# hhcho/sfgwas

Measured on AMD Instinct MI355X. Metric: pca_power_iter_ring_macs_per_s, higher is better.
Workload: dtype u64 ring words, exact integers: int8 digits on the matrix core for the MAC of all five moduli, fp64-held integers in the encode and key-switch kernels

## Files before the change

sfgwas_amd/csrc/ab/ab.hpp:

```cpp
#pragma once
struct MacStrides; struct PanelMap; struct I8Args;
void ab_read_config(SfgConfig &c);
const char *ab_mgpu_solo(int n_local, bool multi_process, bool &solo, int &world, int &rank0);
int ab_set_attrs(sfg_ctx *ctx);
int ab_mac_dma_set_attrs(sfg_ctx *ctx);
int ab_launch_mac_dma_tiles(sfg_ctx *ctx, const double *rotf, size_t rows_per_k, const u64 *pt, u64 *out, int K, int R, int Ncols, int L, int accumulate, const MacStrides &st);
int ab_ntt_set_attrs(sfg_ctx *ctx);
int ab_launch_ntt_half_full(sfg_ctx *ctx, const double *pc, u64 *out_half, size_t nplain, int L, const PanelMap &pm);
int launch_mac(sfg_ctx *ctx, const u64 *rot, const u64 *pt, u64 *out, int K, int R, int Ncols, int L, int accumulate);
int launch_mac_strided(sfg_ctx *ctx, const u64 *rot, const u64 *pt, u64 *out, int K, int R, int Ncols, int L, int accumulate, const MacStrides &st);
void ab_launch_mac_i8_lds(hipStream_t q, const I8Args &a, const ModConst *modc, int nl);
```

sfgwas_amd/csrc/ab/config.hip:

```cpp
#include "../common.hpp"

void ab_read_config(SfgConfig &c) {
    auto env = [](const char *n) { return getenv(n); };
    if (const char *e = env("SFG_MAC_IMPL")) { c.mac_reg = !strcmp(e, "reg"); c.mac_bc = strcmp(e, "dma") != 0 && !c.mac_reg; c.mac_i8 = !strcmp(e, "i8"); }
    if (const char *e = env("SFG_MAC_I8_BIG")) c.mac_i8_big = atoi(e) != 0;
    if (const char *e = env("SFG_MAC_I8_ROT")) { c.mac_i8_nolds = strcmp(e, "lds") != 0; c.mac_i8_ring = !strcmp(e, "ring"); }
    if (env("SFG_MAC_I8_WG")) c.mac_i8_ring = false;
    if (const char *e = env("SFG_MAC_I8_WAVES")) c.mac_i8_waves = atoi(e) == 6 ? 6 : 12;
    if (const char *e = env("SFG_MAC_I8_WG")) c.mac_i8_wg1 = atoi(e) == 1;
    if (const char *e = env("SFG_MAC_WC")) c.mac_wc = atoi(e) == 2 ? 2 : 1;
    if (const char *e = env("SFG_MM_OVERLAP")) c.no_overlap = atoi(e) == 0;
    if (env("SFG_MM_NO_OVERLAP")) c.no_overlap = true;
    if (const char *e = env("SFG_NTT_HALF_IMPL")) c.ntt_half_full = !strcmp(e, "full");
    if (const char *e = env("SFG_NTT_FWD_IMPL")) c.ntt_fwd_full = !strcmp(e, "full");
    if (const char *e = env("SFG_MAC_PT")) c.mac_plain_pt = !strcmp(e, "plain");
    if (const char *e = env("SFG_PT_RIDE")) { c.pt_ride = atoi(e); if (c.pt_ride < 0) c.pt_ride = 0; c.pt_ride = c.pt_ride / 8 * 8; }
    if (const char *e = env("SFG_PT_COMPACT")) c.pt_compact = atoi(e) != 0;
    if (const char *e = env("SFG_PT_KMAJOR")) c.pt_kmajor = atoi(e) != 0;
    if (const char *e = env("SFG_PT_RIDE_DEPTH")) { c.i8_mover_depth_ride = atoi(e); if (c.i8_mover_depth_ride < 1 || c.i8_mover_depth_ride > 3) c.i8_mover_depth_ride = 1; }
    if (const char *e = env("SFG_PT_RIDE_NT")) c.i8_mover_nt_ride = atoi(e) != 0;
    if (env("SFG_ASSOC_TRACE")) c.assoc_trace = true;
}
int ab_set_attrs(sfg_ctx *ctx) { return ab_mac_dma_set_attrs(ctx) || ab_ntt_set_attrs(ctx); }
```

sfgwas_amd/csrc/common.hpp:

```cpp
#pragma once
#include <hip/hip_runtime.h>
#include <cstdint>
#include <cstdio>
#include <cstring>
#include <string>
#include <vector>
#include <map>
#include <set>
#include <unistd.h>
#include "../../include/sfgwas_hip.h"
#include "consts.hpp"

typedef unsigned long long u64;
typedef unsigned __int128 u128;

constexpr unsigned long long SFG_I8_BIG_QMAX = 0x7F7F7F7F7F80ULL;

struct ModConst {
    double q, qinv;
    double ninv, ninv_q;
    u64 qi;
};

struct RotKey {
    u64 *key_dev = nullptr;
    uint16_t *index_dev = nullptr;
};

struct PhaseStat { double ms = 0; int launches = 0; double bytes = 0; };
struct PendingEvent { hipEvent_t e0, e1; std::string name; int launches; double bytes; };

struct sfg_geno {
    const int8_t *dev = nullptr;
    size_t nrow = 0, ncol = 0, ld = 0;
    bool owned = false;
    bool packed = false;
    struct PtcEntry { double *slot; bool transposed; };
    mutable std::map<uint64_t, PtcEntry> ptc;
    mutable size_t ptc_budget = 0, ptc_used = 0;
    mutable double *ptc_arena = nullptr;
    mutable uint32_t *ptc_perm = nullptr;
    mutable const void *ptc_owner = nullptr;
    mutable size_t ptc_hits = 0, ptc_fills = 0;
};

struct SfgConfig {
    int mm_group = 8;
    bool mm_group_auto = true;
    size_t acc_budget = 24ULL << 30;
    size_t assoc_cache_budget = 160ULL << 30;
    size_t ksw_budget = 4ULL << 30;
    int enc_batch = 2048;
    bool upload_blocking = false;
    bool test_hooks = false;
    std::string test_scratch_oom;
    double tie_band = 0x1p-50;
    bool mac_i8_big = true;
    bool mac_reg = false;
    bool mac_bc = true;
    bool mac_i8 = true;
    bool mac_i8_nolds = true;
    bool mac_i8_ring = true;
    int mac_i8_waves = 12;
    bool mac_i8_wg1 = false;
    int mac_wc = 1;
    bool no_overlap = true;
    bool ntt_fwd_full = false;
    bool ntt_half_full = false;
    bool pt_compact = true;
    bool pt_kmajor = true;
    int pt_ride = 192;
    int i8_mover_depth_ride = 1, i8_mover_nt_ride = 1;
    bool mac_plain_pt = false;
    bool assoc_trace = false;
};

struct SfgShared {
    int device = 0;
    int logN = SFG_LOGN, N = SFG_N, nq = 0, np = 0, nmod = 0, beta = 0;
    double scale = 0;
    u64 q[SFG_MAXMOD] = {0}, psi[SFG_MAXMOD] = {0};
    double *tw_fwd = nullptr;
    double *tw_inv = nullptr;
    double2 *pack_fwd = nullptr;
    double2 *pack_inv = nullptr;
    ModConst *modc = nullptr;
    ModConst modc_host[SFG_MAXMOD];
    void *enc_tables = nullptr;
    void *rvec_tables = nullptr;
    void *zeros_dev = nullptr;
    u64 *sk_dev = nullptr;
    u64 *pk_dev = nullptr;
    u64 *skqp_dev = nullptr;
    uint32_t enc_key[8] = {0, 0, 0, 0, 0, 0, 0, 0}; uint32_t *enc_key_dev = nullptr; bool enc_seeded = false;
    u64 enc_next = 0;
    std::map<u64, RotKey> rotkeys;
    SfgConfig cfg;
    int refs = 1;
};

struct sfg_ctx {
    SfgShared *sh = nullptr;
    bool is_fork = false;
    int device = 0;
    int logN = SFG_LOGN, N = SFG_N, nq = 0, np = 0, nmod = 0, beta = 0;
    double scale = 0;
    u64 q[SFG_MAXMOD] = {0}, psi[SFG_MAXMOD] = {0};
    double *tw_fwd = nullptr, *tw_inv = nullptr;
    double2 *pack_fwd = nullptr, *pack_inv = nullptr;
    ModConst *modc = nullptr;
    ModConst modc_host[SFG_MAXMOD];
    SfgConfig cfg;
    unsigned ntt_plain_seq = 0;
    struct I8Slot { const void *src = nullptr; u64 sig[8] = {0, 0, 0, 0, 0, 0, 0, 0}; u64 last_use = 0; };
    static constexpr int I8_SLOTS = 16;
    u64 i8_gen = 1, i8_clock = 0; I8Slot i8_slot[2][I8_SLOTS];
    hipStream_t own_stream = nullptr, stream = nullptr;
    hipStream_t user_stream = nullptr;
    hipStream_t aux_stream = nullptr;
    unsigned char *pin = nullptr; size_t pin_bytes = 0, pin_head = 0;
    hipStream_t coll_stream = nullptr;
    hipEvent_t ev_pipe[4] = {nullptr, nullptr, nullptr, nullptr};
    std::vector<hipEvent_t> ev_pool; size_t ev_next = 0;
    std::map<int, void *> ksw_cache;
    void *ws = nullptr; size_t ws_bytes = 0;
    std::map<std::string, std::pair<void *, size_t>> pool;
    std::map<std::string, std::pair<void *, size_t>> host_pool;
    std::map<std::string, unsigned long long> pool_epoch;
    unsigned long long api_epoch = 0; int api_depth = 0;
    int scratch_oom_seen = 0;
    std::vector<PendingEvent> pending;
    std::string err;
    std::map<std::string, PhaseStat> phases;
    std::set<const sfg_geno *> ptc_genos;
    bool test_hooks = false;
    void *tie_count_dev = nullptr;
    hipStream_t main_stream() const { return user_stream ? user_stream : own_stream; }
    std::map<u64, RotKey> &rotkeys() { return sh->rotkeys; }
    const std::map<u64, RotKey> &rotkeys() const { return sh->rotkeys; }
    void *enc_tables() const { return sh->enc_tables; }
    void *zeros_dev() const { return sh->zeros_dev; }
};

int sfg_sync_all(sfg_ctx *ctx);
int sfg_encoder_check(sfg_ctx *ctx);
void sfg_ptc_detach_all(sfg_ctx *ctx);
void sfg_ptc_invalidate_all(sfg_ctx *ctx);

int encrypt_set_attrs(sfg_ctx *ctx);
int sfg_rows_from_montgomery(sfg_ctx *ctx, unsigned long long *rows_dev, size_t nrows, int nmod);
void sfg_encrypt_destroy(SfgShared *sh);
int enc_take_indices(sfg_ctx *ctx, const char *what, int nct, unsigned long long *first);
int keygen_set_attrs(sfg_ctx *ctx);
void sfg_keygen_destroy(SfgShared *sh);
int sfg_rvec_init(sfg_ctx *ctx);
void sfg_rvec_destroy(SfgShared *sh);

extern thread_local std::string g_create_error;

#define SFG_FAIL(ctx, ...) do { char _b[512]; snprintf(_b, sizeof _b, __VA_ARGS__); (ctx)->err = _b; return 1; } while (0)
#ifdef SFG_AB
#include "ab/ab.hpp"
#endif
#define SFG_HIP(ctx, call) do { hipError_t _e = (call); if (_e != hipSuccess) { char _b[512]; \
    snprintf(_b, sizeof _b, "HIP call failed: %s (%s:%d)", hipGetErrorString(_e), __FILE__, __LINE__); (ctx)->err = _b; return 1; } } while (0)
#define SFG_TRY(expr) do { int _rc = (expr); if (_rc) return _rc; } while (0)

int sfg_ws_reserve(sfg_ctx *ctx, size_t bytes);

static inline u64 h_mulmod(u64 a, u64 b, u64 q) { return (u64)(((u128)a * b) % q); }
static inline u64 h_powmod(u64 a, u64 e, u64 q) { u64 r = 1 % q; a %= q; while (e) { if (e & 1) r = h_mulmod(r, a, q); a = h_mulmod(a, a, q); e >>= 1; } return r; }
static inline u64 h_invmod(u64 a, u64 q) { return h_powmod(a, q - 2, q); }
static inline uint32_t h_brev(uint32_t x, int bits) { uint32_t r = 0; for (int i = 0; i < bits; i++) { r = (r << 1) | (x & 1); x >>= 1; } return r; }

int sfg_upload_small(sfg_ctx *ctx, void *dst_dev, const void *src_host, size_t bytes);
struct ApiScope {
    sfg_ctx *c;
    explicit ApiScope(sfg_ctx *c_) : c(c_) { if (c->api_depth++ == 0) c->api_epoch++; }
    ~ApiScope() { c->api_depth--; }
};
struct AuxScope {
    sfg_ctx *c; hipStream_t saved;
    explicit AuxScope(sfg_ctx *c_, bool on = true) : c(c_), saved(c_->stream) { if (on) c->stream = c->aux_stream; }
    ~AuxScope() { c->stream = saved; }
};
template <class T, hipError_t (*Free)(T)> struct HipOwner {
    T h = T();
    HipOwner() {}
    HipOwner(HipOwner &&o) : h(o.release()) {}
    HipOwner(const HipOwner &) = delete; HipOwner &operator=(const HipOwner &) = delete;
    ~HipOwner() { if (h) (void)Free(h); }
    T release() { T t = h; h = T(); return t; }
};
typedef HipOwner<void *, hipFree> DevMem;
typedef HipOwner<hipEvent_t, hipEventDestroy> EventOwner;
typedef HipOwner<hipStream_t, hipStreamDestroy> StreamOwner;
struct FdOwner {
    int fd;
    explicit FdOwner(int fd_ = -1) : fd(fd_) {}
    FdOwner(FdOwner &&o) : fd(o.fd) { o.fd = -1; }
    FdOwner(const FdOwner &) = delete; FdOwner &operator=(const FdOwner &) = delete;
    ~FdOwner() { reset(); }
    void reset(int fd_ = -1) { if (fd >= 0) close(fd); fd = fd_; }
};
int sfg_stream_after(sfg_ctx *ctx, hipStream_t waiter, hipStream_t signaller);
int sfg_scratch(sfg_ctx *ctx, const char *name, size_t bytes, void **out);
int sfg_host_scratch(sfg_ctx *ctx, const char *name, size_t bytes, void **out);
void sfg_phases_resolve(sfg_ctx *ctx);

struct PhaseTimer {
    sfg_ctx *ctx; const char *name; hipEvent_t e0, e1; bool on;
    PhaseTimer(sfg_ctx *c, const char *n, bool enable = true) : ctx(c), name(n), on(enable) {
        if (on) { (void)hipEventCreate(&e0); (void)hipEventCreate(&e1); (void)hipEventRecord(e0, ctx->stream); }
    }
    void stop(int launches = 1, double bytes = 0) {
        if (!on) return;
        (void)hipEventRecord(e1, ctx->stream);
        ctx->pending.push_back(PendingEvent{e0, e1, name, launches, bytes});
        on = false;
        if (ctx->pending.size() > 4096) sfg_phases_resolve(ctx);
    }
    ~PhaseTimer() { stop(0); }
};

constexpr u64 PACKED_ZERO = 0ULL;
#ifdef __HIPCC__
__device__ __host__ __forceinline__ u64 pack_limbs(u64 w) {
    return (w & 0xFFF) | (((w >> 12) & 0xFFF) << 16) | ((w >> 24) << 32);
}

__device__ __forceinline__ double mulmod_lazy(double x, double w, double wq, double q) {
    double qh = __builtin_rint(x * wq);
    double h = x * w;
    double l = __builtin_fma(x, w, -h);
    double r = __builtin_fma(-qh, q, h);
    return r + l;
}
__device__ __forceinline__ double mulmod_lazy_q(double x, double w, double q, double qinv) {
    double h = x * w;
    double qh = __builtin_rint(h * qinv);
    double l = __builtin_fma(x, w, -h);
    double r = __builtin_fma(-qh, q, h);
    return r + l;
}
__device__ __forceinline__ double canon(double x, double q, double qinv) {
    const double r = __builtin_fma(-__builtin_floor(x * qinv), q, x);
    return r == q ? 0.0 : r;
}
__device__ __forceinline__ double canon_le(double x, double q, double qinv) {
    return __builtin_fma(-__builtin_floor(x * qinv), q, x);
}
__device__ __forceinline__ double pred(double x, double q, double qinv) {
    double qh = __builtin_rint(x * qinv);
    return __builtin_fma(-qh, q, x);
}
__device__ __forceinline__ double u64_to_f64(u64 x) {
    return __longlong_as_double((long long)(x | 0x4330000000000000ULL)) - 4503599627370496.0;
}
__device__ __forceinline__ u64 f64_to_u64(double x) {
    return (u64)__double_as_longlong(x + 4503599627370496.0) & 0x000FFFFFFFFFFFFFULL;
}
__device__ __forceinline__ void bytes_tr4(unsigned w0, unsigned w1, unsigned w2, unsigned w3, unsigned (&o)[4]) {
    const unsigned p0 = __builtin_amdgcn_perm(w1, w0, 0x05010400u), p1 = __builtin_amdgcn_perm(w1, w0, 0x07030602u);
    const unsigned q0 = __builtin_amdgcn_perm(w3, w2, 0x05010400u), q1 = __builtin_amdgcn_perm(w3, w2, 0x07030602u);
    o[0] = __builtin_amdgcn_perm(q0, p0, 0x05040100u); o[1] = __builtin_amdgcn_perm(q0, p0, 0x07060302u);
    o[2] = __builtin_amdgcn_perm(q1, p1, 0x05040100u); o[3] = __builtin_amdgcn_perm(q1, p1, 0x07060302u);
}
__device__ __forceinline__ int sq_sum4_i8(int w) {
    const int sq = __builtin_amdgcn_sdot4(w, w, 0, false);
    if (sq < 128) return sq;
    int s = 0;
#pragma unroll
    for (int k = 0; k < 4; k++) { const int x = (int)(int8_t)(w >> (8 * k)); s += (int)(int8_t)(x * x); }
    return s;
}
__device__ __forceinline__ u64 pack_limbs_f64(double x) {
    const u64 b = (u64)__double_as_longlong(x + 4503599627370496.0);
    const unsigned lo = (unsigned)b, hi = (unsigned)(b >> 32);
    const unsigned x01 = ((lo << 4) & 0x0FFF0000u) | (lo & 0xFFFu);
    const unsigned x2 = __builtin_amdgcn_alignbit(hi, lo, 24) & 0xFFFu;
    return ((u64)x2 << 32) | x01;
}
__device__ __forceinline__ u64 d_mulmod_u64(u64 a, u64 b, u64 q) {
    u64 hi = __umul64hi(a, b), lo = a * b;
    u64 r = hi % q;
    for (int i = 63; i >= 0; i--) { u64 top = r >> 63; r = (r << 1) | ((lo >> i) & 1); if (top || r >= q) r -= q; }
    return r;
}
__device__ __forceinline__ u64 splitmix_at(u64 seed, u64 idx) {
    u64 z = seed + 0x9E3779B97F4A7C15ULL * (idx + 1);
    z = (z ^ (z >> 30)) * 0xBF58476D1CE4E5B9ULL;
    z = (z ^ (z >> 27)) * 0x94D049BB133111EBULL;
    return z ^ (z >> 31);
}
#endif
```

sfgwas_amd/csrc/kernels.hpp:

```cpp
#pragma once
#include "common.hpp"
#include "mm_plan.hpp"
#include "assoc_plan.hpp"

constexpr int SFG_MAXPATTERN = 128;
struct ModPattern { int period; int8_t m[SFG_MAXPATTERN]; };
struct RowMap { int rpg; size_t gstride_in, gstride_out; };
struct PanelMap { int G, g, shift0; unsigned packed_mask = 0; int K = 0; };

int launch_ntt_fwd(sfg_ctx *ctx, const u64 *in, u64 *out, size_t nrows, const ModPattern &pat);
int launch_ntt_inv(sfg_ctx *ctx, const u64 *in, u64 *out, size_t nrows, const ModPattern &pat);
int launch_ntt_plain(sfg_ctx *ctx, const double *pc, u64 *out, size_t nplain, int L);
struct MoveJob;
struct PtRide;
int launch_ntt_plain_half(sfg_ctx *ctx, const double *pc, u64 *out_half, size_t nplain, int L, PanelMap pm, const uint32_t *perm = nullptr, const MoveJob *mv = nullptr);
int launch_expand_half(sfg_ctx *ctx, const u64 *half, u64 *full, size_t nrows);
int launch_ntt_fwd_map(sfg_ctx *ctx, const u64 *in, u64 *out, size_t nrows, const ModPattern &pat, const RowMap &rm);
int launch_ntt_inv_map(sfg_ctx *ctx, const u64 *in, u64 *out, size_t nrows, const ModPattern &pat, const RowMap &rm);
struct MacStrides { size_t rot_k, rot_r, pt_k, pt_n, out_n, out_r; bool pt_half = false; bool pt_packed = false; bool pt_digits = false; bool i8 = false; bool i8_big = false; bool pt_digits_big = false;
                    const int8_t *B_small = nullptr, *B_big = nullptr;
                    int pt_layout = 0, pt_L = 0;
                    int B_mode = 0;
                    const int8_t *A_small = nullptr, *A_big = nullptr; };
int launch_mac_i8_small(sfg_ctx *ctx, const double *rotf, size_t rotf_k_stride, size_t rotf_r_stride, int plane0, const u64 *pt, u64 *out, int K, int R, int r0, int Ncols,
                        int l0, int nl, int accumulate, const MacStrides &st);
int launch_mac_i8_big(sfg_ctx *ctx, const double *rotf, size_t rotf_k_stride, size_t rotf_r_stride, int plane0, const u64 *pt, u64 *out, int K, int R, int r0, int Ncols,
                      int l0, int accumulate, const MacStrides &st);
int launch_skew(sfg_ctx *ctx, const int8_t *blk, size_t ld, int r, int c, int transposed, int square, int8_t *D);
struct PcCache { double *slot = nullptr; int mode = 0; const uint32_t *perm = nullptr; };
int launch_encode_rows(sfg_ctx *ctx, const int8_t *D, int shift0, int nshift, int L, u64 *pt, bool half_rows = false, int G = 0, int g = 0, unsigned packed_mask = 0, const PcCache *pcache = nullptr,
                       PtRide *ride = nullptr);
int encode_rows_launches(const sfg_ctx *ctx, int nshift);
int i8_ride_prepare(sfg_ctx *ctx, const u64 *panel, int K, int Ncols, size_t pt_k, size_t pt_n, int layout, int L, int launches, PtRide &ride);
int i8_ride_finish(sfg_ctx *ctx, PtRide &ride);
int i8_ride_tiles(sfg_ctx *ctx, int K, int L, int8_t **Bs, int8_t **Bb);
struct I8Args;
void launch_i8_pack_pt_digits(hipStream_t q, const I8Args &a, unsigned items, bool big);
void launch_move_alone(hipStream_t q, const MoveJob &j);
int launch_share(sfg_ctx *ctx, const u64 *rows, size_t rows_ct_stride, const u64 *xr, size_t x_ct_stride, u64 *h, int nl, int nct);
int launch_add_rows(sfg_ctx *ctx, const u64 *a, size_t a_ct_stride, const u64 *b, size_t b_ct_stride, u64 *out, size_t out_ct_stride, int nl, int nct);
int encrypt_errors_moddown(sfg_ctx *ctx, const int32_t *e0, const int32_t *e1, int nct, int level, u64 *out);
int launch_geno_unpack(sfg_ctx *ctx, const sfg_geno *g, size_t r0, size_t c0, size_t nr, size_t nc, int8_t *out, size_t ld_out);
int launch_rotate_right(sfg_ctx *ctx, const u64 *in, u64 *out, int nct, int level, const int *nrot_host);
int launch_rotate_right_indexed(sfg_ctx *ctx, const u64 *in, int nin, u64 *out, int nct, int level, const int *nrot_host, const int *in_index);
int launch_rotate_right_indexed_f64(sfg_ctx *ctx, const u64 *in, int nin, double *outf, int nct, int level, const int *nrot_host, const int *in_index, int L,
                                    const size_t *out_slot = nullptr);
int launch_relinearize(sfg_ctx *ctx, const u64 *tmp, int nct, int level, const u64 *mid, u64 *out);
int launch_ct_add(sfg_ctx *ctx, const u64 *a, const u64 *b, u64 *out, size_t nct, int level);
int mac_dma_planes(sfg_ctx *ctx, int L, std::vector<int> &plane_of, std::vector<int> &is_big);
double mac_big_maxterm(u64 q);
int launch_rot_to_f64(sfg_ctx *ctx, const u64 *rot, size_t nrows, int nl_rot, int L, double *rotf);
int launch_mac_dma(sfg_ctx *ctx, const double *rotf, size_t rows_per_k, const u64 *pt, u64 *out, int K, int R, int Ncols, int L, int accumulate, const MacStrides &st,
                   const double *rotsum = nullptr);
int launch_rot_sum(sfg_ctx *ctx, const double *rotf, size_t rows_per_k, int K, int L, double *rotsum);
int launch_pack_pt(sfg_ctx *ctx, const u64 *in, u64 *out, size_t nrows, size_t words_per_row, int L, unsigned packed_mask);
unsigned mac_dma_packed_mask(sfg_ctx *ctx, int L);
bool mac_use_dma(const sfg_ctx *ctx);
int launch_mac_bc(sfg_ctx *ctx, const double *rotf, size_t rows_per_k, const u64 *pt, u64 *out, int K, int R, int Ncols, int L, int accumulate, const MacStrides &st,
                  const double *rotsum);
int rotcache_build_rows_tab(sfg_ctx *ctx, const u64 *A, int s, int in_level, int max_level, int nbr, int b0, int b1, const std::vector<std::vector<uint8_t>> *tabs, double *cache);
int assoc_build_rotcache(sfg_ctx *ctx, const u64 *A_dev, int s, int in_level, int max_level, size_t nr, const std::vector<size_t> &widths, double **out);
struct I8RotPre { int G = 0, nbr = 0, s = 0, L = 0; std::vector<int8_t *> As, Ab; };
int i8_rotpre_build(sfg_ctx *ctx, const u64 *A_dev, int s, int in_level, int max_level, int nbr, const std::vector<std::vector<uint8_t>> *tabs, size_t budget_bytes, const char *prefix, I8RotPre &pre);
void i8_rotpre_free(I8RotPre &pre);
struct I8RotPreScope { I8RotPre pre; ~I8RotPreScope() { i8_rotpre_free(pre); } };
int matmul_resident_range_i8pre(sfg_ctx *ctx, const I8RotPre &pre, int s, int max_level, const sfg_geno *g, unsigned flags, int blk0, int blk1, uint64_t *out);
int matmul_accumulate_i8pre(sfg_ctx *ctx, const I8RotPre &pre, int s, int max_level, const sfg_geno *g, unsigned flags, int j0, int j1, int accumulate, uint64_t *acc,
                            size_t acc_col_words = 0);
int launch_i8_pack_rot_to(sfg_ctx *ctx, const double *rotf, size_t rotf_k_stride, size_t rotf_r_stride, int plane0, int K, int R, int l0, int nl, bool big, int8_t *A_out);
struct AssocRot { double *f64 = nullptr; I8RotPre pre; };
int assoc_build_rot(sfg_ctx *ctx, const u64 *A_dev, int s, int in_level, int max_level, size_t nr, const std::vector<size_t> &widths, AssocRot &out);
void assoc_free_rot(AssocRot &r);
struct AssocRotScope { AssocRot r; ~AssocRotScope() { assoc_free_rot(r); } };
int assoc_product(sfg_ctx *ctx, const AssocRot &r, const uint64_t *A_dev, int s, int in_level, int max_level, const sfg_geno *g, unsigned flags, int nct, uint64_t *out);
int assoc_batch_tail(sfg_ctx *ctx, const u64 *tmp, const sfg_geno *g, int s, size_t nct, size_t ctw, uint64_t *out_dev, size_t out_ct_capacity, size_t out_shift,
                     double *sum_host, double *sqsum_host);

int launch_bed_decode(sfg_ctx *ctx, hipStream_t st, const uint8_t *dbed, size_t bps, size_t num_sample, size_t num_snp, const int32_t *rmap, const int32_t *cmap,
                      int8_t *out, size_t ld);
int launch_bed_decode_lut(sfg_ctx *ctx, hipStream_t st, const uint8_t *dbed, size_t bps, size_t num_sample, size_t num_snp, const int32_t *rmap, const int32_t *cmap,
                          int8_t *out, size_t ld, unsigned lut);
int upload_filter_map(sfg_ctx *ctx, const uint8_t *filt, size_t n, DevMem &map, size_t *kept);

int assoc_stream_part(sfg_ctx *ctx, int fmt, const char *path, size_t num_sample, size_t num_snp, const uint8_t *row_filter, const uint8_t *col_filter,
                      size_t batch_snps, const uint64_t *A_dev, int s, int in_level, int max_level, unsigned flags,
                      uint64_t *out_dev, size_t out_ct_capacity, size_t *out_ct, double *sum_host, double *sqsum_host,
                      int part, int nparts, std::vector<std::pair<size_t, size_t>> *ranges);
```

sfgwas_amd/csrc/ksw.hpp:

```cpp
#pragma once
#include "common.hpp"

constexpr int KSW_MAXA = 4;
constexpr int KSW_MAXDIG = 8;

struct ExtConst {
    int a;
    int src[KSW_MAXA];
    double qhat_inv[KSW_MAXA], qhat_inv_q[KSW_MAXA];
    double qhat_t[SFG_MAXMOD][KSW_MAXA], qhat_t_q[SFG_MAXMOD][KSW_MAXA];
    double D_t[SFG_MAXMOD], D_t_q[SFG_MAXMOD];
};
struct KswConst {
    int level, nl, np, nt, beta, alpha;
    int tmod[SFG_MAXMOD];
    int digit_of[SFG_MAXMOD];
    ExtConst dig[KSW_MAXDIG];
    ExtConst pq;
    double pinv[SFG_MAXMOD], pinv_q[SFG_MAXMOD];
};
int get_ksw(sfg_ctx *ctx, int level, KswConst **dev, KswConst *host);

#ifdef __HIPCC__
__device__ __forceinline__ double mulmod2(double a, double b, double q, double qinv) {
    double h = a * b;
    double l = __builtin_fma(a, b, -h);
    double qh = __builtin_rint(h * qinv);
    double r = __builtin_fma(-qh, q, h);
    return r + l;
}

__device__ __forceinline__ void ext_prepare(const ExtConst &e, const ModConst *modc, const double (&x)[KSW_MAXA], double (&y)[KSW_MAXA], double &v) {
    double vf = 0.0;
#pragma unroll
    for (int m = 0; m < KSW_MAXA; m++) {
        if (m < e.a) {
            const ModConst mc = modc[e.src[m]];
            y[m] = canon(mulmod_lazy(x[m], e.qhat_inv[m], e.qhat_inv_q[m], mc.q), mc.q, mc.qinv);
            vf += y[m] / mc.q;
        }
    }
    v = (double)(u64)vf;
}
__device__ __forceinline__ double ext_target(const ExtConst &e, int tg, double qt, double qtinv, const double (&y)[KSW_MAXA], double v) {
    double acc = -mulmod_lazy(v, e.D_t[tg], e.D_t_q[tg], qt);
#pragma unroll
    for (int m = 0; m < KSW_MAXA; m++) if (m < e.a) acc += mulmod_lazy(y[m], e.qhat_t[tg][m], e.qhat_t_q[tg][m], qt);
    return canon(acc, qt, qtinv);
}
#endif
```

sfgwas_amd/csrc/matmul.hip:

```cpp
#include "common.hpp"
#include "kernels.hpp"
#include "i8_move.hpp"
#include <algorithm>
#include <string>

static inline int ceil_div(size_t a, size_t b) { return (int)((a + b - 1) / b); }

struct Shape {
    size_t nrow, ncol;
    int nbr, m_ct;
    bool transposed;
    const int8_t *dev; size_t ld;
    const sfg_geno *g;
    int rows_of(int bi) const { return (int)(std::min((size_t)(bi + 1) * SFG_SLOTS, nrow) - (size_t)bi * SFG_SLOTS); }
    int cols_of(int bj) const { return (int)(std::min((size_t)(bj + 1) * SFG_SLOTS, ncol) - (size_t)bj * SFG_SLOTS); }
    const int8_t *block(int bi, int bj) const {
        return transposed ? dev + (size_t)bj * SFG_SLOTS * ld + (size_t)bi * SFG_SLOTS
                          : dev + (size_t)bi * SFG_SLOTS * ld + (size_t)bj * SFG_SLOTS;
    }
};
static Shape make_shape(const sfg_geno *g, unsigned flags) {
    Shape sh; sh.transposed = (flags & SFG_TRANSPOSE) != 0;
    sh.nrow = sh.transposed ? g->ncol : g->nrow; sh.ncol = sh.transposed ? g->nrow : g->ncol;
    sh.nbr = ceil_div(sh.nrow, SFG_SLOTS); sh.m_ct = ceil_div(sh.ncol, SFG_SLOTS);
    sh.dev = g->dev; sh.ld = g->ld; sh.g = g; return sh;
}

__global__ void __launch_bounds__(256) k_drop_level(const u64 *in, u64 *out, int nl_in, int nl) {
    const int N = SFG_N; const size_t row = blockIdx.x / (N / 256);
    const size_t ctp = row / nl, m = row % nl;
    const size_t x = (blockIdx.x % (N / 256)) * 256 + threadIdx.x;
    out[row * N + x] = in[(ctp * nl_in + m) * N + x];
}
__global__ void __launch_bounds__(256) k_sum_giants(const u64 *rot, int ngiant, int s, int L, u64 *out, size_t out_i_stride,
                                                    int accumulate, const ModConst *modc) {
    const int N = SFG_N; const size_t row = blockIdx.x / (N / 256);
    const int i = (int)(row / (2 * L)), pl = (int)(row % (2 * L)), l = pl % L;
    const size_t x = (blockIdx.x % (N / 256)) * 256 + threadIdx.x;
    const double q = modc[l].q, qinv = modc[l].qinv;
    double acc = accumulate ? u64_to_f64(out[(size_t)i * out_i_stride + (size_t)pl * N + x]) : 0.0;
    for (int g = 0; g < ngiant; g++) {
        acc += u64_to_f64(rot[(((size_t)g * s + i) * 2 * L + pl) * N + x]);
        if ((g & 31) == 31) acc = pred(acc, q, qinv);
    }
    out[(size_t)i * out_i_stride + (size_t)pl * N + x] = f64_to_u64(canon(acc, q, qinv));
}
__global__ void __launch_bounds__(256) k_reduce_rows(u64 *rows, int L, const ModConst *modc) {
    const int N = SFG_N; const size_t row = blockIdx.x / (N / 256); const int l = (int)(row % L);
    const size_t off = row * N + (blockIdx.x % (N / 256)) * 256 + threadIdx.x;
    rows[off] = rows[off] % modc[l].qi;
}
__global__ void __launch_bounds__(256) k_pt_zero(u64 *pt, size_t pitch_words, size_t seg_words, int L, size_t prow, unsigned packed_mask) {
    const size_t seg = blockIdx.y, x = (size_t)blockIdx.x * 256 + threadIdx.x;
    if (x >= seg_words) return;
    const int l = (int)((x / prow) % L);
    pt[seg * pitch_words + x] = ((packed_mask >> l) & 1u) ? PACKED_ZERO : 0ULL;
}
__global__ void __launch_bounds__(256) k_pt_zero_kmajor(uint8_t *pt, int K, int planes, int n0, int k0, int nk) {
    const size_t blk = ((size_t)(n0 + blockIdx.y) * planes * 64 + blockIdx.x) * (size_t)K * 128 + (size_t)k0 * 128;
    uint4 *p = reinterpret_cast<uint4 *>(pt + blk);
    for (int i = threadIdx.x; i < nk * 8; i += 256) p[i] = make_uint4(0, 0, 0, 0);
}
static int launch_pt_zero_kmajor(sfg_ctx *ctx, u64 *pt, int K, int planes, int n0, int n1, int k0, int k1) {
    if (n1 <= n0 || k1 <= k0) return 0;
    hipLaunchKernelGGL(k_pt_zero_kmajor, dim3((unsigned)(planes * 64), (unsigned)(n1 - n0)), dim3(256), 0, ctx->stream, reinterpret_cast<uint8_t *>(pt), K, planes, n0, k0, k1 - k0);
    SFG_HIP(ctx, hipGetLastError());
    return 0;
}
static int launch_pt_zero(sfg_ctx *ctx, u64 *pt, size_t pitch_words, size_t seg_words, int nseg, int L, size_t prow, unsigned packed_mask) {
    if (!packed_mask) {
        if (nseg == 1) SFG_HIP(ctx, hipMemsetAsync(pt, 0, seg_words * 8, ctx->stream));
        else SFG_HIP(ctx, hipMemset2DAsync(pt, pitch_words * 8, 0, seg_words * 8, nseg, ctx->stream));
        return 0;
    }
    hipLaunchKernelGGL(k_pt_zero, dim3((unsigned)((seg_words + 255) / 256), (unsigned)nseg), dim3(256), 0, ctx->stream, pt, pitch_words, seg_words, L, prow, packed_mask);
    SFG_HIP(ctx, hipGetLastError());
    return 0;
}
constexpr int CS_ROWS = 4096;
__global__ void __launch_bounds__(256) k_colsums(const int8_t *g, size_t nrow, size_t ncol, size_t ld, double *sum, double *sqsum) {
    __shared__ int red[2][16][256 + 1];
    const int tid = threadIdx.x, cg = tid & 15, rl = tid >> 4;
    const size_t col = (size_t)blockIdx.x * 256 + (size_t)cg * 16, r0 = (size_t)blockIdx.y * CS_ROWS, r1 = r0 + CS_ROWS < nrow ? r0 + CS_ROWS : nrow;
    int p1[16], p2[16];
#pragma unroll
    for (int k = 0; k < 16; k++) p1[k] = p2[k] = 0;
    const bool vec = col + 16 <= ncol && ((reinterpret_cast<uintptr_t>(g) | ld) & 15) == 0;
    auto load = [&](size_t i) -> uint4 {
        uint4 v = make_uint4(0, 0, 0, 0);
        if (i >= r1) return v;
        if (vec) v = *reinterpret_cast<const uint4 *>(g + i * ld + col);
        else if (col < ncol) { int8_t b[16]; for (int k = 0; k < 16; k++) b[k] = col + k < ncol ? g[i * ld + col + k] : (int8_t)0; v = *reinterpret_cast<uint4 *>(b); }
        return v;
    };
    for (size_t i = r0 + rl; i < r1; i += 64) {
        const uint4 v0 = load(i), v1 = load(i + 16), v2 = load(i + 32), v3 = load(i + 48);
        const unsigned a0[4] = {v0.x, v0.y, v0.z, v0.w}, a1[4] = {v1.x, v1.y, v1.z, v1.w}, a2[4] = {v2.x, v2.y, v2.z, v2.w}, a3[4] = {v3.x, v3.y, v3.z, v3.w};
#pragma unroll
        for (int q = 0; q < 4; q++) {
            unsigned o[4]; bytes_tr4(a0[q], a1[q], a2[q], a3[q], o);
#pragma unroll
            for (int t = 0; t < 4; t++) {
                unsigned w = o[t];
                const unsigned m = w & 0x80808080u; w &= ~((m << 1) - (m >> 7));
                p1[4 * q + t] = __builtin_amdgcn_sdot4((int)w, 0x01010101, p1[4 * q + t], false);
                p2[4 * q + t] += sq_sum4_i8((int)w);
            }
        }
    }
#pragma unroll
    for (int k = 0; k < 16; k++) { red[0][rl][cg * 16 + k] = p1[k]; red[1][rl][cg * 16 + k] = p2[k]; }
    __syncthreads();
    long long s1 = 0, s2 = 0;
#pragma unroll
    for (int r = 0; r < 16; r++) { s1 += red[0][r][tid]; s2 += red[1][r][tid]; }
    const size_t j = (size_t)blockIdx.x * 256 + tid;
    if (j < ncol) {
        if (sum) atomicAdd(&sum[j], (double)s1);
        if (sqsum) atomicAdd(&sqsum[j], (double)s2);
    }
}

extern "C" int sfg_ct_drop_level_dev(sfg_ctx *ctx, const uint64_t *in, uint64_t *out, int nct, int level_in, int level_out) {
    SFG_HIP(ctx, hipSetDevice(ctx->device));
    if (level_out > level_in) SFG_FAIL(ctx, "DropLevel: requested level %d when input is %d", level_out, level_in);
    if (level_out < 0 || level_in >= ctx->nq || nct < 0) SFG_FAIL(ctx, "DropLevel: level out of range");
    if (!nct) return 0;
    const int nl = level_out + 1, nl_in = level_in + 1;
    if (nl == nl_in) { SFG_HIP(ctx, hipMemcpyAsync(out, in, (size_t)nct * 2 * nl * SFG_N * 8, hipMemcpyDeviceToDevice, ctx->stream)); return 0; }
    hipLaunchKernelGGL(k_drop_level, dim3((unsigned)((size_t)nct * 2 * nl * (SFG_N / 256))), dim3(256), 0, ctx->stream, (const u64 *)in, (u64 *)out, nl_in, nl);
    SFG_HIP(ctx, hipGetLastError());
    return 0;
}
extern "C" int sfg_memcpy_d2d(sfg_ctx *ctx, void *dst, const void *src, size_t bytes) {
    SFG_HIP(ctx, hipSetDevice(ctx->device));
    SFG_HIP(ctx, hipMemcpyAsync(dst, src, bytes, hipMemcpyDeviceToDevice, ctx->stream));
    return 0;
}

extern "C" int sfg_geno_upload(sfg_ctx *ctx, const int8_t *host, size_t nrow, size_t ncol, size_t ld, sfg_geno **out) {
    SFG_HIP(ctx, hipSetDevice(ctx->device));
    if (!nrow || !ncol || ld < ncol) SFG_FAIL(ctx, "sfg_geno_upload: bad dimensions");
    int8_t *d = nullptr;
    SFG_HIP(ctx, hipMalloc(&d, nrow * ncol));
    SFG_HIP(ctx, hipMemcpy2DAsync(d, ncol, host, ld, ncol, nrow, hipMemcpyHostToDevice, ctx->stream));
    SFG_HIP(ctx, hipStreamSynchronize(ctx->stream));
    sfg_geno *g = new sfg_geno(); g->dev = d; g->nrow = nrow; g->ncol = ncol; g->ld = ncol; g->owned = true;
    *out = g; return 0;
}
extern "C" int sfg_geno_create(sfg_ctx *ctx, size_t nrow, size_t ncol, sfg_geno **out) {
    SFG_HIP(ctx, hipSetDevice(ctx->device));
    if (!out) SFG_FAIL(ctx, "sfg_geno_create: null result pointer");
    *out = nullptr;
    if (!nrow || !ncol) SFG_FAIL(ctx, "sfg_geno_create: bad dimensions");
    int8_t *d = nullptr;
    SFG_TRY(sfg_malloc(ctx, (void **)&d, nrow * ncol));
    sfg_geno *g = new sfg_geno(); g->dev = d; g->nrow = nrow; g->ncol = ncol; g->ld = ncol; g->owned = true;
    *out = g; return 0;
}
extern "C" int sfg_geno_write_rows(sfg_ctx *ctx, sfg_geno *g, size_t row0, size_t nrows, const int8_t *rows_host, size_t ld) {
    SFG_HIP(ctx, hipSetDevice(ctx->device));
    if (!g || !g->owned || g->packed) SFG_FAIL(ctx, "sfg_geno_write_rows: not a matrix made by sfg_geno_create");
    if (!nrows) return 0;
    if (!rows_host || ld < g->ncol || row0 > g->nrow || nrows > g->nrow - row0) SFG_FAIL(ctx, "sfg_geno_write_rows: rows [%zu, %zu) of a %zu x %zu matrix, row stride %zu", row0, row0 + nrows, g->nrow, g->ncol, ld);
    if (!g->ptc.empty()) SFG_FAIL(ctx, "sfg_geno_write_rows: the matrix has cached plaintexts (sfg_geno_set_plaintext_cache): it must not change");
    SFG_HIP(ctx, hipMemcpy2DAsync(const_cast<int8_t *>(g->dev) + row0 * g->ld, g->ld, rows_host, ld, g->ncol, nrows, hipMemcpyHostToDevice, ctx->stream));
    SFG_HIP(ctx, hipStreamSynchronize(ctx->stream));
    return 0;
}
__global__ void __launch_bounds__(256) k_geno_compare(const int8_t *chunk, const int8_t *stored, size_t ld, size_t row0, size_t nrows, size_t ncol_l, int transposed, unsigned long long *ndiff) {
    const size_t total = nrows * ncol_l;
    unsigned long long bad = 0;
    for (size_t i = (size_t)blockIdx.x * 256 + threadIdx.x; i < total; i += (size_t)gridDim.x * 256) {
        size_t r, c;
        if (transposed) { r = i % nrows; c = i / nrows; } else { r = i / ncol_l; c = i % ncol_l; }
        const int8_t want = transposed ? stored[c * ld + row0 + r] : stored[(row0 + r) * ld + c];
        bad += chunk[r * ncol_l + c] != want;
    }
    if (bad) atomicAdd(ndiff, bad);
}
extern "C" int sfg_geno_compare_rows(sfg_ctx *ctx, const sfg_geno *g, unsigned flags, size_t row0, size_t nrows, const int8_t *rows_host, size_t ld, uint64_t *ndiff) {
    SFG_HIP(ctx, hipSetDevice(ctx->device));
    if (!g || g->packed || !ndiff) SFG_FAIL(ctx, "sfg_geno_compare_rows: needs an unpacked resident matrix and a result pointer");
    const bool tr = flags & SFG_TRANSPOSE;
    const size_t nrow_l = tr ? g->ncol : g->nrow, ncol_l = tr ? g->nrow : g->ncol;
    if (!nrows) return 0;
    if (!rows_host || ld < ncol_l || row0 > nrow_l || nrows > nrow_l - row0) SFG_FAIL(ctx, "sfg_geno_compare_rows: rows [%zu, %zu) of a %zu x %zu matrix, row stride %zu", row0, row0 + nrows, nrow_l, ncol_l, ld);
    int8_t *chunk = nullptr; unsigned long long *cnt = nullptr;
    SFG_TRY(sfg_scratch(ctx, "geno.cmp", nrows * ncol_l, (void **)&chunk));
    SFG_TRY(sfg_scratch(ctx, "geno.cmpcnt", 8, (void **)&cnt));
    SFG_HIP(ctx, hipMemsetAsync(cnt, 0, 8, ctx->stream));
    SFG_HIP(ctx, hipMemcpy2DAsync(chunk, ncol_l, rows_host, ld, ncol_l, nrows, hipMemcpyHostToDevice, ctx->stream));
    const size_t total = nrows * ncol_l;
    hipLaunchKernelGGL(k_geno_compare, dim3((unsigned)std::min<size_t>((total + 255) / 256, 65536)), dim3(256), 0, ctx->stream, (const int8_t *)chunk, g->dev, g->ld, row0, nrows, ncol_l, tr ? 1 : 0, cnt);
    SFG_HIP(ctx, hipGetLastError());
    unsigned long long h = 0;
    SFG_HIP(ctx, hipMemcpyAsync(&h, cnt, 8, hipMemcpyDeviceToHost, ctx->stream));
    SFG_HIP(ctx, hipStreamSynchronize(ctx->stream));
    *ndiff += h;
    return 0;
}
extern "C" int sfg_pinned_alloc(sfg_ctx *ctx, void **host_ptr, size_t bytes) {
    SFG_HIP(ctx, hipSetDevice(ctx->device));
    if (!host_ptr || !bytes) SFG_FAIL(ctx, "sfg_pinned_alloc: bad arguments");
    SFG_HIP(ctx, hipHostMalloc(host_ptr, bytes, hipHostMallocDefault));
    return 0;
}
extern "C" int sfg_pinned_free(sfg_ctx *ctx, void *host_ptr) {
    SFG_HIP(ctx, hipSetDevice(ctx->device));
    if (host_ptr) SFG_HIP(ctx, hipHostFree(host_ptr));
    return 0;
}
extern "C" int sfg_geno_from_device(sfg_ctx *ctx, const int8_t *dev, size_t nrow, size_t ncol, size_t ld, sfg_geno **out) {
    if (!nrow || !ncol || ld < ncol) SFG_FAIL(ctx, "sfg_geno_from_device: bad dimensions");
    sfg_geno *g = new sfg_geno(); g->dev = dev; g->nrow = nrow; g->ncol = ncol; g->ld = ld; g->owned = false;
    *out = g; return 0;
}
static void ptc_drop(sfg_ctx *ctx, const sfg_geno *g) {
    sfg_ctx *own = g->ptc_owner ? (sfg_ctx *)g->ptc_owner : ctx;
    own->ptc_genos.erase(g);
    if (g->ptc.empty() && !g->ptc_perm) return;
    (void)hipSetDevice(own->device); (void)sfg_sync_all(own);
    if (own != ctx) (void)sfg_sync_all(ctx);
    g->ptc.clear(); g->ptc_used = 0;
    if (g->ptc_arena) { (void)hipFree(g->ptc_arena); g->ptc_arena = nullptr; }
    if (g->ptc_perm) { (void)hipFree(g->ptc_perm); g->ptc_perm = nullptr; }
}
void sfg_ptc_invalidate_all(sfg_ctx *ctx) {
    for (const sfg_geno *g : ctx->ptc_genos) { g->ptc.clear(); g->ptc_used = 0; }
}
void sfg_ptc_detach_all(sfg_ctx *ctx) {
    for (const sfg_geno *g : ctx->ptc_genos) {
        g->ptc.clear(); g->ptc_used = 0; g->ptc_budget = 0;
        if (g->ptc_arena) { (void)hipFree(g->ptc_arena); g->ptc_arena = nullptr; }
        if (g->ptc_perm) { (void)hipFree(g->ptc_perm); g->ptc_perm = nullptr; }
        g->ptc_owner = nullptr;
    }
    ctx->ptc_genos.clear();
}
extern "C" void sfg_geno_free(sfg_ctx *ctx, sfg_geno *g) {
    if (!g) return;
    ptc_drop(ctx, g);
    if (g->owned) { (void)hipSetDevice(ctx->device); (void)sfg_sync_all(ctx); (void)hipFree((void *)g->dev); }
    delete g;
}
extern "C" int sfg_geno_set_plaintext_cache(sfg_ctx *ctx, const sfg_geno *g, size_t max_bytes) {
    SFG_HIP(ctx, hipSetDevice(ctx->device));
    if (!g) SFG_FAIL(ctx, "sfg_geno_set_plaintext_cache: null matrix");
    if (!max_bytes) { ptc_drop(ctx, g); g->ptc_budget = 0; g->ptc_owner = nullptr; return 0; }
    if (g->ptc_owner && g->ptc_owner != (const void *)ctx) SFG_FAIL(ctx, "sfg_geno_set_plaintext_cache: the cache of this matrix belongs to another context (drop it there first)");
    if (!g->ptc_perm) {
        const int n = SFG_SLOTS, d = SFG_D; const unsigned M = 2u * SFG_N;
        std::vector<uint32_t> tab(n);
        std::vector<unsigned> pow5(n); pow5[0] = 1; for (int k = 1; k < n; k++) pow5[k] = (unsigned)(((u64)pow5[k - 1] * 5u) % M);
        for (int t = 0; t < n; t++) {
            const int u = (n - t) % n, k = ((t % d) + d * (u / d)) % n;
            tab[t] = (uint32_t)u | (uint32_t)pow5[k] << 16;
        }
        uint32_t *dv = nullptr;
        SFG_HIP(ctx, hipMalloc((void **)&dv, (size_t)n * 4));
        if (hipMemcpy(dv, tab.data(), (size_t)n * 4, hipMemcpyHostToDevice) != hipSuccess) { (void)hipFree(dv); SFG_FAIL(ctx, "sfg_geno_set_plaintext_cache: table upload failed"); }
        g->ptc_perm = dv;
    }
    const size_t slot_bytes = (size_t)SFG_SLOTS * SFG_SLOTS * 8, want = max_bytes / slot_bytes * slot_bytes;
    if (want != g->ptc_budget || !g->ptc_arena) {
        (void)hipStreamSynchronize(ctx->stream);
        g->ptc.clear(); g->ptc_used = 0;
        if (g->ptc_arena) { (void)hipFree(g->ptc_arena); g->ptc_arena = nullptr; }
        g->ptc_budget = 0;
        if (!want) SFG_FAIL(ctx, "sfg_geno_set_plaintext_cache: max_bytes is less than one block (%zu bytes)", slot_bytes);
        void *a = nullptr;
        if (hipMalloc(&a, want) != hipSuccess) { (void)hipGetLastError(); SFG_FAIL(ctx, "sfg_geno_set_plaintext_cache: cannot allocate %zu bytes", want); }
        g->ptc_arena = (double *)a; g->ptc_budget = want;
    }
    g->ptc_owner = ctx; ctx->ptc_genos.insert(g);
    return 0;
}
extern "C" int sfg_geno_plaintext_cache_stats(sfg_ctx *ctx, const sfg_geno *g, size_t *blocks, size_t *bytes, size_t *hits, size_t *fills) {
    if (!g) SFG_FAIL(ctx, "sfg_geno_plaintext_cache_stats: null matrix");
    if (blocks) *blocks = g->ptc.size();
    if (bytes) *bytes = g->ptc_used;
    if (hits) *hits = g->ptc_hits;
    if (fills) *fills = g->ptc_fills;
    return 0;
}
extern "C" int sfg_geno_colsums(sfg_ctx *ctx, const sfg_geno *g, double *sum_host, double *sqsum_host) {
    SFG_HIP(ctx, hipSetDevice(ctx->device));
    if (g->packed) {
        sfg_geno *u = nullptr; SFG_TRY(sfg_geno_unpack(ctx, g, &u));
        const int rc = sfg_geno_colsums(ctx, u, sum_host, sqsum_host); sfg_geno_free(ctx, u); return rc;
    }
    SFG_TRY(sfg_ws_reserve(ctx, g->ncol * 16));
    double *ds = (double *)ctx->ws, *dq = ds + g->ncol;
    SFG_HIP(ctx, hipMemsetAsync(ds, 0, g->ncol * 16, ctx->stream));
    hipLaunchKernelGGL(k_colsums, dim3((unsigned)((g->ncol + 255) / 256), (unsigned)((g->nrow + CS_ROWS - 1) / CS_ROWS)), dim3(256), 0, ctx->stream, g->dev, g->nrow, g->ncol, g->ld, ds, dq);
    SFG_HIP(ctx, hipGetLastError());
    if (sum_host) SFG_HIP(ctx, hipMemcpyAsync(sum_host, ds, g->ncol * 8, hipMemcpyDeviceToHost, ctx->stream));
    if (sqsum_host) SFG_HIP(ctx, hipMemcpyAsync(sqsum_host, dq, g->ncol * 8, hipMemcpyDeviceToHost, ctx->stream));
    SFG_HIP(ctx, hipStreamSynchronize(ctx->stream));
    return 0;
}
extern "C" int sfg_reduce_rows_dev(sfg_ctx *ctx, uint64_t *rows, size_t nrows_of_L, int L) {
    SFG_HIP(ctx, hipSetDevice(ctx->device));
    const size_t rows_total = nrows_of_L * L;
    if (!rows_total) return 0;
    hipLaunchKernelGGL(k_reduce_rows, dim3((unsigned)(rows_total * (SFG_N / 256))), dim3(256), 0, ctx->stream, (u64 *)rows, L, ctx->modc);
    SFG_HIP(ctx, hipGetLastError());
    return 0;
}

static int build_rot_row_tab(sfg_ctx *ctx, const u64 *A, int s, int nl_in, int nl, int lev, int L, int nbr, int bi, const std::vector<uint8_t> &baby_t,
                             u64 *a_row, u64 *rotc, bool dma, double *rotf_dst);
static int build_rot_row(sfg_ctx *ctx, const u64 *A, int s, int nl_in, int nl, int lev, int L, const Shape &sh, int bi, u64 *a_row, u64 *rotc,
                         bool dma, double *rotf_dst) {
    const int d = SFG_D;
    const int nr = sh.rows_of(bi);
    std::vector<uint8_t> baby_t(d, 0);
    for (int shift = 0; shift < SFG_SLOTS; shift++) {
        if (baby_t[shift % d]) continue;
        bool any = false;
        for (int bj = 0; bj < sh.m_ct && !any; bj++) any = diag_bool(nr, sh.cols_of(bj), SFG_SLOTS, -shift);
        if (any) baby_t[shift % d] = 1;
    }
    return build_rot_row_tab(ctx, A, s, nl_in, nl, lev, L, sh.nbr, bi, baby_t, a_row, rotc, dma, rotf_dst);
}
static int build_rot_row_tab(sfg_ctx *ctx, const u64 *A, int s, int nl_in, int nl, int lev, int L, int nbr, int bi, const std::vector<uint8_t> &baby_t,
                             u64 *a_row, u64 *rotc, bool dma, double *rotf_dst) {
    const int N = SFG_N, d = SFG_D; const size_t ctw = (size_t)2 * nl * N;
    for (int i = 0; i < s; i++) {
        const u64 *src = A + ((size_t)i * nbr + bi) * 2 * nl_in * N;
        if (nl == nl_in) SFG_HIP(ctx, hipMemcpyAsync(a_row + (size_t)i * ctw, src, ctw * 8, hipMemcpyDeviceToDevice, ctx->stream));
        else hipLaunchKernelGGL(k_drop_level, dim3((unsigned)(2 * nl * (N / 256))), dim3(256), 0, ctx->stream, src, a_row + (size_t)i * ctw, nl_in, nl);
    }
    SFG_HIP(ctx, hipGetLastError());
    {
        PhaseTimer t(ctx, "rotate");
        std::vector<int> nrv((size_t)d * s, 0), inv((size_t)d * s, 0);
        for (int baby = 0; baby < d; baby++) for (int i = 0; i < s; i++) { nrv[(size_t)baby * s + i] = baby_t[baby] ? -baby : 0; inv[(size_t)baby * s + i] = i; }
        if (dma) SFG_TRY(launch_rotate_right_indexed_f64(ctx, a_row, s, rotf_dst, d * s, lev, nrv.data(), inv.data(), L));
        else SFG_TRY(launch_rotate_right_indexed(ctx, a_row, s, rotc, d * s, lev, nrv.data(), inv.data()));
        t.stop(1);
    }
    return 0;
}

static MmPlanIn plan_input(sfg_ctx *ctx, int s, int L, int nblockrows, int ncolb, RotSrc rot, int pre_G) {
    const SfgConfig &c = ctx->cfg;
    MmPlanIn in;
    in.mm_group = c.mm_group; in.mm_group_auto = c.mm_group_auto; in.mac_i8 = c.mac_i8; in.mac_i8_big = c.mac_i8_big;
    in.pt_compact = c.pt_compact; in.pt_kmajor = c.pt_kmajor; in.pt_ride = c.pt_ride; in.no_overlap = c.no_overlap;
    in.dma = mac_use_dma(ctx); in.packed_mask = in.dma ? mac_dma_packed_mask(ctx, L) : 0u; in.mods = ModSplit(ctx->q, L);
    in.s = s; in.L = L; in.nblockrows = nblockrows; in.ncolb = ncolb; in.rot = rot; in.pre_G = pre_G;
    if (mm_plan_reads_memory(in)) {
        size_t fr = 0, tot = 0;
        in.mem_failed = hipMemGetInfo(&fr, &tot) != hipSuccess;
        in.mem_search = in.mem_keep = fr;
        for (const auto &kv : ctx->pool) {
            if (kv.first == "mm.pt" || kv.first == "mm.rotf" || kv.first.rfind("mi8.", 0) == 0) in.mem_search += kv.second.second;
            if (kv.first.rfind("mi8.A", 0) == 0) in.mem_keep += kv.second.second;
        }
    }
    return in;
}
struct MmCall {
    sfg_ctx *ctx; const Shape &sh; unsigned flags; const u64 *A; const I8RotPre *pre8;
    int s, L, lev, nl, nl_in; bool dma; unsigned packed_mask; size_t ctw, accw, rowf = 0;
    MmPlan plan;
    u64 *a_row = nullptr, *rotc = nullptr; int8_t *skew = nullptr, *unpacked = nullptr; double *rotf = nullptr, *rotsum = nullptr;
    int8_t *rideBs = nullptr, *rideBb = nullptr;
};
struct MacJob { bool on = false; u64 *ptp = nullptr; int gsn = 0, gi = 0, acc_flag = 0; u64 *accj = nullptr; const double *rotf_grp = nullptr, *rotsum_grp = nullptr; };

static int build_group(const MmCall &c, int bg, int b1, int buf) {
    sfg_ctx *ctx = c.ctx; const int d = SFG_D, s = c.s, ng = std::min(c.plan.G, b1 - bg);
    ctx->i8_gen++;
    double *dst = c.rotf + (size_t)buf * c.plan.grp_slices * s * 2 * c.rowf;
    for (int g = 0; g < ng; g++) SFG_TRY(build_rot_row(ctx, c.A, s, c.nl_in, c.nl, c.lev, c.L, c.sh, bg + g, c.a_row, c.rotc, c.dma, c.dma ? dst + (size_t)g * d * s * 2 * c.rowf : nullptr));
    if (c.dma && (ng * d) % 4)
        SFG_HIP(ctx, hipMemsetAsync(dst + (size_t)ng * d * s * 2 * c.rowf, 0, (size_t)3 * s * 2 * c.rowf * 8, ctx->stream));
    if (c.packed_mask) SFG_TRY(launch_rot_sum(ctx, dst, (size_t)s * 2, ng * d, c.L, c.rotsum + (size_t)buf * s * 2 * c.rowf));
    return 0;
}
static int run_mac(const MmCall &c, const MacJob &m, int B_mode) {
    sfg_ctx *ctx = c.ctx; const MmPlan &p = c.plan; const int N = SFG_N, d = SFG_D;
    PhaseTimer t(ctx, "mac");
    MacStrides st;
    if (c.rideBs) { st.B_small = c.rideBs; st.B_big = c.rideBb; st.B_mode = B_mode; }
    if (c.pre8) { st.A_small = c.pre8->As[m.gi]; st.A_big = c.pre8->Ab[m.gi]; }
    st.rot_k = (size_t)c.s * c.ctw; st.rot_r = (size_t)c.nl * N;
    st.pt_k = p.plw; st.pt_n = (size_t)m.gsn * d * p.plw; st.pt_half = c.dma; st.pt_packed = c.packed_mask != 0; st.pt_digits = st.i8 = p.use_i8; st.i8_big = st.pt_digits_big = p.use_i8_big;
    st.pt_layout = p.pt_layout; st.pt_L = c.L;
    st.out_n = c.accw; st.out_r = (size_t)c.L * N;
    int rc;
    if (c.dma) rc = launch_mac_dma(ctx, c.pre8 ? nullptr : m.rotf_grp, (size_t)c.s * 2, m.ptp, m.accj, m.gsn * d, 2 * c.s, d, c.L, m.acc_flag, st, m.rotsum_grp);
#ifdef SFG_AB
    else rc = launch_mac_strided(ctx, c.rotc, m.ptp, m.accj, d, 2 * c.s, d, c.L, m.acc_flag, st);
#else
    else { rc = 1; ctx->err = "matmul: the register-staged MAC exists in the A/B build only (make ab)"; }
#endif
    t.stop(1);
    return rc;
}
struct PtcSlot {
    static constexpr size_t slot_bytes = (size_t)SFG_SLOTS * SFG_SLOTS * 8;
    PcCache pcc; const sfg_geno *g; uint64_t key = 0; bool fresh = false;
    PtcSlot(const MmCall &c, int bi, int bj) : g(c.sh.g) {
        if (!c.dma || !g->ptc_budget || g->ptc_owner != (const void *)c.ctx) return;
        const uint64_t sr = c.sh.transposed ? bj : bi, sc = c.sh.transposed ? bi : bj;
        key = sr << 33 | sc << 1 | ((c.flags & SFG_SQUARE) ? 1u : 0u);
        auto it = g->ptc.find(key);
        if (it != g->ptc.end()) { pcc.slot = it->second.slot; pcc.mode = it->second.transposed == c.sh.transposed ? 2 : 3; pcc.perm = g->ptc_perm; g->ptc_hits++; }
        else if (g->ptc_used + slot_bytes <= g->ptc_budget) {
            double *slot = g->ptc_arena + g->ptc_used / 8;
            g->ptc[key] = sfg_geno::PtcEntry{slot, c.sh.transposed}; g->ptc_used += slot_bytes; g->ptc_fills++;
            pcc.slot = slot; pcc.mode = 1; fresh = true;
        }
    }
    void undo() {
        if (!fresh) return;
        auto it = g->ptc.find(key);
        if (it != g->ptc.end()) { g->ptc.erase(it); g->ptc_used -= slot_bytes; }
        fresh = false;
    }
};
static int encode_block(const MmCall &c, int bi, int bj, int g, int ng, u64 *pt, PtRide *ride) {
    sfg_ctx *ctx = c.ctx; const Shape &sh = c.sh; const MmPlan &p = c.plan;
    const int d = SFG_D, L = c.L, nr = sh.rows_of(bi), nc = sh.cols_of(bj), tr = sh.transposed ? 1 : 0, sq = (c.flags & SFG_SQUARE) ? 1 : 0;
    const size_t plw = p.plw, nplain = (size_t)d * d;
    PtcSlot ptc(c, bi, bj);
    int rc = 0;
    if (ptc.pcc.mode < 2) {
        PhaseTimer t(ctx, "skew");
        if (sh.g->packed) {
            const size_t sr0 = (size_t)(tr ? bj : bi) * SFG_SLOTS, sc0 = (size_t)(tr ? bi : bj) * SFG_SLOTS;
            rc = launch_geno_unpack(ctx, sh.g, sr0, sc0, tr ? nc : nr, tr ? nr : nc, c.unpacked, SFG_SLOTS);
            if (!rc) rc = launch_skew(ctx, c.unpacked, SFG_SLOTS, nr, nc, tr, sq, c.skew);
        } else rc = launch_skew(ctx, sh.block(bi, bj), sh.ld, nr, nc, tr, sq, c.skew);
        t.stop(1);
    }
    if (rc) { ptc.undo(); return rc; }
    int runs[2][2]; int nruns = 0;
    if (nr + nc > SFG_SLOTS) { runs[0][0] = 0; runs[0][1] = SFG_SLOTS; nruns = 1; }
    else { runs[0][0] = 0; runs[0][1] = nr; runs[1][0] = SFG_SLOTS - nc + 1; runs[1][1] = SFG_SLOTS; nruns = runs[1][0] < runs[1][1] ? 2 : 1; }
    const bool full = nruns == 1 && runs[0][1] - runs[0][0] == SFG_SLOTS;
    if (p.kmajor) {
        const int kb0 = g * d;
        if (full) rc = launch_pt_zero_kmajor(ctx, pt, ng * d, p.pt_planes, d - 1, d, kb0 + (SFG_SLOTS - (d - 1) * d), kb0 + d);
        else rc = launch_pt_zero_kmajor(ctx, pt, ng * d, p.pt_planes, 0, d, kb0, kb0 + d);
    } else if (full) {
        rc = launch_pt_zero(ctx, pt + (((size_t)(d - 1) * ng + g) * d + (SFG_SLOTS - (d - 1) * d)) * plw, 0, (nplain - SFG_SLOTS) * plw, 1, L, p.prow, c.packed_mask);
    } else {
        rc = launch_pt_zero(ctx, pt + (size_t)g * d * plw, (size_t)ng * d * plw, (size_t)d * plw, d, L, p.prow, c.packed_mask);
    }
    if (rc) { ptc.undo(); return rc; }
    PhaseTimer t(ctx, "encode");
    for (int r = 0; r < nruns && !rc; r++) {
        if (c.dma) rc = launch_encode_rows(ctx, c.skew, runs[r][0], runs[r][1] - runs[r][0], L, pt, true, ng, g, p.enc_flags, ptc.pcc.mode ? &ptc.pcc : nullptr, ride);
        else rc = launch_encode_rows(ctx, c.skew, runs[r][0], runs[r][1] - runs[r][0], L, pt + (size_t)runs[r][0] * plw, false);
    }
    t.stop(nruns);
    if (rc) ptc.undo();
    return rc;
}
static int ride_launch_count(const MmCall &c, int bg, int ng, int nc) {
    int launches = 0;
    for (int g = 0; g < ng; g++) {
        const int nr = c.sh.rows_of(bg + g);
        if (nr + nc > SFG_SLOTS) launches += encode_rows_launches(c.ctx, SFG_SLOTS);
        else launches += encode_rows_launches(c.ctx, nr) + (nc > 1 ? encode_rows_launches(c.ctx, nc - 1) : 0);
    }
    return launches;
}

static int matmul_accumulate(sfg_ctx *ctx, const u64 *A, int s, int in_level, int max_level, const Shape &sh, unsigned flags,
                             int b0, int b1, int j0, int j1, int accumulate, u64 *acc, const double *rotf_pre = nullptr, const double *rotsum_pre = nullptr,
                             const I8RotPre *pre8 = nullptr, size_t acc_col_words = 0) {
    const int N = SFG_N, d = SFG_D, L = max_level;
    if (pre8 && (rotf_pre || !mac_use_dma(ctx) || b0 != 0 || b1 != pre8->nbr || sh.nbr != pre8->nbr || s != pre8->s || L != pre8->L))
        SFG_FAIL(ctx, "matmul: internal: the int8 rot tiles were built for another product (block rows %d, s = %d, level %d)", pre8->nbr, pre8->s, pre8->L);
    const int lev = in_level > max_level ? max_level : in_level, nl = lev + 1, nl_in = in_level + 1;
    if (L < 1 || L > ctx->nq) SFG_FAIL(ctx, "matmul: max_level out of range");
    if (nl < L) SFG_FAIL(ctx, "matmul: input level %d has fewer than max_level = %d moduli", in_level, max_level);
    if (b0 < 0 || b1 > sh.nbr || b0 > b1 || j0 < 0 || j1 > sh.m_ct || j0 > j1) SFG_FAIL(ctx, "matmul: block range out of bounds");
    const size_t ctw = (size_t)2 * nl * N, accw = (size_t)s * 2 * L * N;
    const int ncolb = j1 - j0;
    const size_t acc_col = acc_col_words ? acc_col_words : (size_t)d * accw;
    if (acc_col < (size_t)d * accw) SFG_FAIL(ctx, "matmul: internal: accumulator column stride below 91 giant steps");
    if (b0 == b1 || j0 == j1) {
        if (!accumulate) for (int c = 0; c < ncolb; c++) SFG_HIP(ctx, hipMemsetAsync(acc + (size_t)c * acc_col, 0, (size_t)d * accw * 8, ctx->stream));
        return 0;
    }
    const MmPlanIn in = plan_input(ctx, s, L, b1 - b0, ncolb, rotf_pre ? RotSrc::f64_cache : pre8 ? RotSrc::i8_tiles : RotSrc::own, pre8 ? pre8->G : 0);
    if (in.dma && in.mods.too_big) SFG_FAIL(ctx, "sfg_mac: modulus >= 2^47 unsupported by the fp64 limb schedule");
    MmCall c{ctx, sh, flags, A, pre8, s, L, lev, nl, nl_in, in.dma, in.packed_mask, ctw, accw};
    c.plan = mm_plan(in);
    MmPlan &plan = c.plan;
    const int G = plan.G; const bool dma = in.dma, rot_ext = in.rot != RotSrc::own;
    if (rotsum_pre && G < rotsum_group_size(in.mm_group, in.nblockrows)) SFG_FAIL(ctx, "matmul: internal: fewer rot-sum groups than MAC groups");
    u64 *pt = nullptr;
    SFG_TRY(sfg_scratch(ctx, "mm.a_row", (size_t)s * ctw * 8, (void **)&c.a_row));
    SFG_TRY(sfg_scratch(ctx, "mm.rotc", dma ? 8 : (size_t)d * s * ctw * 8, (void **)&c.rotc));
    if (plan.ride_want && sfg_scratch(ctx, "mm.pt", plan.panel_words * 8 * 2 + 65536, (void **)&pt)) { ctx->err.clear(); plan.ride_want = false; }
    if (!plan.ride_want) SFG_TRY(sfg_scratch(ctx, "mm.pt", plan.panel_words * 8 + 65536, (void **)&pt));
    u64 *const pt_base = pt;
    SFG_TRY(sfg_scratch(ctx, "mm.skew", (size_t)SFG_SLOTS * SFG_SLOTS, (void **)&c.skew));
    if (sh.g->packed) SFG_TRY(sfg_scratch(ctx, "mm.unpack", (size_t)SFG_SLOTS * SFG_SLOTS, (void **)&c.unpacked));
    if (dma) {
        c.rowf = (size_t)in.mods.fp64_planes * N;
        if (!rot_ext) SFG_TRY(sfg_scratch(ctx, "mm.rotf", plan.grp_slices * s * 2 * c.rowf * 8 * (plan.pipelined ? 2 : 1), (void **)&c.rotf));
        if (!rot_ext && in.packed_mask) SFG_TRY(sfg_scratch(ctx, "mm.rotsum", (size_t)2 * s * 2 * c.rowf * 8, (void **)&c.rotsum));
    }
    const size_t rot_half = plan.grp_slices * s * 2 * c.rowf, rotsum_half = (size_t)s * 2 * c.rowf;
    hipStream_t main_stream = ctx->stream;
    if (plan.pipelined) {
        SFG_TRY(sfg_stream_after(ctx, ctx->aux_stream, main_stream));
        { AuxScope aux(ctx); SFG_TRY(build_group(c, b0, b1, 0)); }
        SFG_HIP(ctx, hipEventRecord(ctx->ev_pipe[0], ctx->aux_stream));
    }
    int rc = 0, gi = 0, it = 0;
    MacJob held;
    for (int bg = b0; bg < b1; bg += G, gi++) {
        const int ng = std::min(G, b1 - bg);
        if (held.on && !pre8) { SFG_TRY(run_mac(c, held, 2)); held.on = false; }
        const double *rotf_grp = c.rotf, *rotsum_grp = c.rotsum;
        if (rotf_pre) { rotf_grp = rotf_pre + (size_t)(bg - b0) * d * s * 2 * c.rowf; rotsum_grp = rotsum_pre ? rotsum_pre + (size_t)gi * rotsum_half : nullptr; }
        else if (pre8) { rotf_grp = nullptr; rotsum_grp = nullptr; }
        else if (plan.pipelined) {
            if (bg + G < b1) {
                SFG_TRY(sfg_stream_after(ctx, ctx->aux_stream, main_stream));
                { AuxScope aux(ctx); SFG_TRY(build_group(c, bg + G, b1, (gi + 1) & 1)); }
                SFG_HIP(ctx, hipEventRecord(ctx->ev_pipe[(gi + 1) & 1], ctx->aux_stream));
            }
            SFG_HIP(ctx, hipStreamWaitEvent(main_stream, ctx->ev_pipe[gi & 1], 0));
            rotf_grp = c.rotf + (size_t)(gi & 1) * rot_half;
            if (c.rotsum) rotsum_grp = c.rotsum + (size_t)(gi & 1) * rotsum_half;
        } else SFG_TRY(build_group(c, bg, b1, 0));
        for (int bj = j0; bj < j1; bj++, it++) {
            pt = pt_base + (size_t)(plan.ride_want ? (it & 1) : 0) * plan.panel_words;
            PtRide ride;
            if (plan.ride_want && !c.rideBs) SFG_TRY(i8_ride_tiles(ctx, G * d, L, &c.rideBs, &c.rideBb));
            if (held.on && plan.ride_want && c.rideBs) {
                SFG_TRY(i8_ride_prepare(ctx, held.ptp, held.gsn * d, d, plan.plw, (size_t)held.gsn * d * plan.plw, plan.pt_layout, L, ride_launch_count(c, bg, ng, sh.cols_of(bj)), ride));
                if (ride.on && (ride.job.a5.B != c.rideBs || (ride.job.n6 && ride.job.a6.B != c.rideBb))) SFG_FAIL(ctx, "matmul: internal: the riding transposition's tile buffers moved");
            }
            if (held.on && !ride.on) { SFG_TRY(run_mac(c, held, c.rideBs ? 2 : 0)); held.on = false; }
            for (int g = 0; g < ng; g++) SFG_TRY(encode_block(c, bg + g, bj, g, ng, pt, ride.on ? &ride : nullptr));
            if (held.on) { SFG_TRY(i8_ride_finish(ctx, ride)); SFG_TRY(run_mac(c, held, 1)); held.on = false; }
            MacJob m; m.on = true; m.ptp = pt; m.gsn = ng; m.gi = gi;
            m.acc_flag = (accumulate || bg != b0) ? 1 : 0;
            m.accj = acc + (size_t)(bj - j0) * acc_col; m.rotf_grp = rotf_grp; m.rotsum_grp = rotsum_grp;
            if (plan.ride_want && c.rideBs) held = m;
            else SFG_TRY(run_mac(c, m, c.rideBs ? 2 : 0));
        }
    }
    if (held.on) rc = run_mac(c, held, 2);
    return rc;
}

static int matmul_finalize(sfg_ctx *ctx, const u64 *acc, int s, int max_level, int ncolb, int m_ct_out, int jout0, int g0, int g1,
                           const std::vector<uint8_t> *giant_active, int accumulate, u64 *out, int acc_giants = SFG_D, int giant_base = 0) {
    const int N = SFG_N, d = SFG_D, L = max_level;
    const size_t accw = (size_t)s * 2 * L * N, ctw = (size_t)2 * L * N;
    if (g0 < 0 || g1 > acc_giants || g0 > g1 || giant_base < 0) SFG_FAIL(ctx, "finalize: giant range out of bounds");
    u64 *rot = nullptr;
    SFG_TRY(sfg_scratch(ctx, "mm.fin_rot", (size_t)d * accw * 8, (void **)&rot));
    std::vector<int> glist;
    for (int g = g0; g < g1; g++) if (giant_base + g < d && (!giant_active || (*giant_active)[giant_base + g])) glist.push_back(g);
    const int ng = (int)glist.size();
    std::vector<int> nrv((size_t)ng * s), inv((size_t)ng * s);
    for (int k = 0; k < ng; k++) for (int i = 0; i < s; i++) { nrv[(size_t)k * s + i] = -(giant_base + glist[k]) * d; inv[(size_t)k * s + i] = glist[k] * s + i; }
    int rc = 0;
    for (int jb = 0; jb < ncolb && !rc; jb++) {
        const u64 *accj = acc + (size_t)jb * acc_giants * accw;
        u64 *o = out + (size_t)(jout0 + jb) * ctw;
        if (ng) {
            PhaseTimer t(ctx, "rotate");
            rc = launch_rotate_right_indexed(ctx, accj, acc_giants * s, rot, ng * s, L - 1, nrv.data(), inv.data());
            t.stop(1);
            if (rc) break;
        }
        hipLaunchKernelGGL(k_sum_giants, dim3((unsigned)((size_t)s * 2 * L * (N / 256))), dim3(256), 0, ctx->stream, rot, ng, s, L,
                           o, (size_t)m_ct_out * ctw, accumulate, ctx->modc);
        if (hipGetLastError() != hipSuccess) { rc = 1; ctx->err = "finalize: k_sum_giants launch failed"; }
    }
    return rc;
}

static void giant_table(const Shape &sh, std::vector<uint8_t> &giant_t) {
    giant_t.assign(SFG_D, 0);
    for (int bi = 0; bi < sh.nbr; bi++) {
        const int nr = sh.rows_of(bi);
        for (int shift = 0; shift < SFG_SLOTS; shift++) {
            if (giant_t[shift / SFG_D]) { shift = (shift / SFG_D + 1) * SFG_D - 1; continue; }
            bool any = false;
            for (int bj = 0; bj < sh.m_ct && !any; bj++) any = diag_bool(nr, sh.cols_of(bj), SFG_SLOTS, -shift);
            if (any) giant_t[shift / SFG_D] = 1;
        }
    }
}

extern "C" int sfg_matmul_accumulate_dev(sfg_ctx *ctx, const uint64_t *A, int s, int in_level, int max_level, const sfg_geno *g, unsigned flags,
                                         int b0, int b1, int j0, int j1, int accumulate, uint64_t *acc) {
    ApiScope api_scope(ctx);
    SFG_HIP(ctx, hipSetDevice(ctx->device));
    Shape sh = make_shape(g, flags);
    return matmul_accumulate(ctx, (const u64 *)A, s, in_level, max_level, sh, flags, b0, b1, j0, j1, accumulate, (u64 *)acc);
}
extern "C" int sfg_matmul_finalize_dev(sfg_ctx *ctx, const uint64_t *acc, int s, int max_level, int ncolb, int g0, int g1, int accumulate, uint64_t *out) {
    ApiScope api_scope(ctx);
    SFG_HIP(ctx, hipSetDevice(ctx->device));
    return matmul_finalize(ctx, (const u64 *)acc, s, max_level, ncolb, ncolb, 0, g0, g1, nullptr, accumulate, (u64 *)out);
}

extern "C" int sfg_matmul_finalize_slots_dev(sfg_ctx *ctx, const uint64_t *acc, int s, int max_level, int ncolb, int acc_giants, int giant_base,
                                             int g0, int g1, int accumulate, uint64_t *out) {
    ApiScope api_scope(ctx);
    SFG_HIP(ctx, hipSetDevice(ctx->device));
    if (acc_giants < 1) SFG_FAIL(ctx, "finalize: acc_giants must be positive");
    return matmul_finalize(ctx, (const u64 *)acc, s, max_level, ncolb, ncolb, 0, g0, g1, nullptr, accumulate, (u64 *)out, acc_giants, giant_base);
}

static int matmul_resident_range(sfg_ctx *ctx, const uint64_t *A, int s, int in_level, int max_level, const sfg_geno *g, unsigned flags,
                                 int blk0, int blk1, uint64_t *out, const double *rotf_ext, const I8RotPre *pre8 = nullptr) {
    SFG_HIP(ctx, hipSetDevice(ctx->device));
    ctx->phases.clear();
    if (!rotf_ext && !pre8) ctx->i8_gen++;
    Shape sh = make_shape(g, flags);
    const int d = SFG_D, L = max_level, N = SFG_N;
    const size_t accw = (size_t)s * 2 * L * N;
    std::vector<uint8_t> giant_t; giant_table(sh, giant_t);
    int b0 = 0, b1 = sh.nbr, j0 = 0, j1 = sh.m_ct;
    if (sh.transposed) { b0 = blk0; b1 = blk1; } else { j0 = blk0; j1 = blk1; }
    if (b0 < 0 || b1 > sh.nbr || j0 < 0 || j1 > sh.m_ct || b0 > b1 || j0 > j1) SFG_FAIL(ctx, "matmul: SNP-block range out of bounds");
    const int m_out = j1 - j0;
    const size_t budget = ctx->cfg.acc_budget;
    int jg = (int)(budget / ((size_t)d * accw * 8)); if (jg < 1) jg = 1;
    const double *rotf_all = rotf_ext, *rotsum_all = nullptr;
    if (rotf_ext && !mac_use_dma(ctx)) SFG_FAIL(ctx, "matmul: a prebuilt rotation cache needs the LDS-DMA MAC (the A/B build selected the register-staged kernel)");
    if (!rotf_ext && !pre8 && mac_use_dma(ctx) && j1 - j0 > jg && b1 > b0) {
        std::vector<int> plane_of, is_big; const int nplanes = mac_dma_planes(ctx, L, plane_of, is_big);
        if (nplanes < 0) return 1;
        const size_t rowf = (size_t)nplanes * N, per_row = (size_t)d * s * 2 * rowf;
        const int lev = in_level > max_level ? max_level : in_level, nl = lev + 1;
        if (nl >= L && ((size_t)(b1 - b0) * per_row + 3 * (size_t)s * 2 * rowf) * 8 <= (48ULL << 30)) {
            double *buf = nullptr; u64 *a_row = nullptr, *rotc = nullptr;
            const size_t ctw = (size_t)2 * nl * N;
            SFG_TRY(sfg_scratch(ctx, "mm.rotf", ((size_t)(b1 - b0) * per_row + 3 * (size_t)s * 2 * rowf) * 8, (void **)&buf));
            SFG_TRY(sfg_scratch(ctx, "mm.a_row", (size_t)s * ctw * 8, (void **)&a_row));
            SFG_TRY(sfg_scratch(ctx, "mm.rotc", 8, (void **)&rotc));
            for (int bi = b0; bi < b1; bi++) SFG_TRY(build_rot_row(ctx, (const u64 *)A, s, in_level + 1, nl, lev, L, sh, bi, a_row, rotc, true, buf + (size_t)(bi - b0) * per_row));
            SFG_HIP(ctx, hipMemsetAsync(buf + (size_t)(b1 - b0) * per_row, 0, 3 * (size_t)s * 2 * rowf * 8, ctx->stream));
            rotf_all = buf;
            if (mac_dma_packed_mask(ctx, L)) {
                const int G = rotsum_group_size(ctx->cfg.mm_group, b1 - b0), ngrp = (b1 - b0 + G - 1) / G;
                double *rs = nullptr;
                SFG_TRY(sfg_scratch(ctx, "mm.rotsum_all", (size_t)ngrp * s * 2 * rowf * 8, (void **)&rs));
                for (int gi = 0; gi < ngrp; gi++) {
                    const int ng = std::min(G, b1 - b0 - gi * G);
                    SFG_TRY(launch_rot_sum(ctx, buf + (size_t)gi * G * per_row, (size_t)s * 2, ng * d, L, rs + (size_t)gi * s * 2 * rowf));
                }
                rotsum_all = rs;
            }
        }
    }
    const bool overlap = (rotf_all || pre8) && !ctx->cfg.no_overlap;
    if (overlap) { jg = (jg + 1) / 2; }
    hipStream_t main_stream = ctx->stream;
    int k = 0;
    for (int ja = j0; ja < j1; ja += jg, k++) {
        const int jb = std::min(j1, ja + jg);
        u64 *acc = nullptr;
        SFG_TRY(sfg_scratch(ctx, "mm.acc", (size_t)jg * d * accw * 8 * (overlap ? 2 : 1), (void **)&acc));
        if (overlap) {
            acc += (size_t)(k & 1) * jg * d * accw;
            if (k >= 2) SFG_HIP(ctx, hipStreamWaitEvent(main_stream, ctx->ev_pipe[2 + (k & 1)], 0));
        }
        int rc = matmul_accumulate(ctx, (const u64 *)A, s, in_level, max_level, sh, flags, b0, b1, ja, jb, 0, acc, rotf_all, rotsum_all, pre8);
        if (rc) return rc;
        if (overlap) {
            SFG_TRY(sfg_stream_after(ctx, ctx->aux_stream, main_stream));
            { AuxScope aux(ctx); rc = matmul_finalize(ctx, acc, s, max_level, jb - ja, m_out, ja - j0, 0, d, &giant_t, 0, (u64 *)out); }
            if (rc) return rc;
            SFG_HIP(ctx, hipEventRecord(ctx->ev_pipe[2 + (k & 1)], ctx->aux_stream));
        } else {
            rc = matmul_finalize(ctx, acc, s, max_level, jb - ja, m_out, ja - j0, 0, d, &giant_t, 0, (u64 *)out);
            if (rc) return rc;
        }
    }
    if (overlap) SFG_TRY(sfg_stream_after(ctx, main_stream, ctx->aux_stream));
    return 0;
}
extern "C" int sfg_matmul_resident_range_dev(sfg_ctx *ctx, const uint64_t *A, int s, int in_level, int max_level, const sfg_geno *g, unsigned flags,
                                             int blk0, int blk1, uint64_t *out) {
    ApiScope api_scope(ctx);
    return matmul_resident_range(ctx, A, s, in_level, max_level, g, flags, blk0, blk1, out, nullptr);
}

static int rotcache_rowf(sfg_ctx *ctx, int L, size_t &rowf) {
    if (!mac_use_dma(ctx)) SFG_FAIL(ctx, "rotation cache objects need the LDS-DMA MAC (the A/B build selected the register-staged kernel)");
    if (L < 1 || L > ctx->nq) SFG_FAIL(ctx, "rotcache: max_level out of range");
    std::vector<int> plane_of, is_big; const int nplanes = mac_dma_planes(ctx, L, plane_of, is_big);
    if (nplanes < 0) return 1;
    rowf = (size_t)nplanes * SFG_N; return 0;
}
extern "C" int sfg_rotcache_layout(sfg_ctx *ctx, int s, int max_level, size_t *job_doubles, size_t *tail_doubles) {
    size_t rowf = 0; SFG_TRY(rotcache_rowf(ctx, max_level, rowf));
    if (job_doubles) *job_doubles = (size_t)SFG_D * 2 * rowf;
    if (tail_doubles) *tail_doubles = (size_t)3 * s * 2 * rowf;
    return 0;
}
extern "C" int sfg_rotcache_build_jobs_dev(sfg_ctx *ctx, const uint64_t *A, int s, int in_level, int max_level, int nbr, int job0, int job1, double *staged) {
    ApiScope api_scope(ctx);
    SFG_HIP(ctx, hipSetDevice(ctx->device));
    const int N = SFG_N, d = SFG_D, L = max_level;
    size_t rowf = 0; SFG_TRY(rotcache_rowf(ctx, L, rowf));
    const int lev = in_level > max_level ? max_level : in_level, nl = lev + 1, nl_in = in_level + 1;
    if (nl < L || in_level >= ctx->nq) SFG_FAIL(ctx, "rotcache: input level %d unusable with max_level = %d", in_level, max_level);
    if (s < 1 || nbr < 1 || job0 < 0 || job1 > nbr * s || job0 > job1) SFG_FAIL(ctx, "rotcache: job range out of bounds");
    const size_t ctw = (size_t)2 * nl * N;
    constexpr int CH = 64;
    u64 *a_in = nullptr;
    SFG_TRY(sfg_scratch(ctx, "rc.in", (size_t)CH * ctw * 8, (void **)&a_in));
    PhaseTimer t(ctx, "rotate");
    for (int c0 = job0; c0 < job1; c0 += CH) {
        const int nj = std::min(CH, job1 - c0);
        for (int k = 0; k < nj; k++) {
            const int job = c0 + k, bi = job / s, i = job % s;
            const u64 *src = (const u64 *)A + ((size_t)i * nbr + bi) * 2 * nl_in * N;
            if (nl == nl_in) SFG_HIP(ctx, hipMemcpyAsync(a_in + (size_t)k * ctw, src, ctw * 8, hipMemcpyDeviceToDevice, ctx->stream));
            else hipLaunchKernelGGL(k_drop_level, dim3((unsigned)(2 * nl * (N / 256))), dim3(256), 0, ctx->stream, src, a_in + (size_t)k * ctw, nl_in, nl);
        }
        SFG_HIP(ctx, hipGetLastError());
        std::vector<int> nrv((size_t)d * nj), inv((size_t)d * nj); std::vector<size_t> slot((size_t)d * nj);
        for (int baby = 0; baby < d; baby++) for (int k = 0; k < nj; k++) {
            nrv[(size_t)baby * nj + k] = -baby; inv[(size_t)baby * nj + k] = k; slot[(size_t)baby * nj + k] = (size_t)(c0 - job0 + k) * d + baby;
        }
        SFG_TRY(launch_rotate_right_indexed_f64(ctx, a_in, nj, staged, d * nj, lev, nrv.data(), inv.data(), L, slot.data()));
    }
    t.stop(1);
    return 0;
}
extern "C" int sfg_rotcache_scatter_dev(sfg_ctx *ctx, const double *staged, int s, int max_level, int job0, int job1, int row0, int nrows, double *cache) {
    ApiScope api_scope(ctx);
    SFG_HIP(ctx, hipSetDevice(ctx->device));
    ctx->i8_gen++;
    const int d = SFG_D;
    size_t rowf = 0; SFG_TRY(rotcache_rowf(ctx, max_level, rowf));
    if (s < 1 || nrows < 1 || job0 < row0 * s || job1 > (row0 + nrows) * s || job0 > job1) SFG_FAIL(ctx, "rotcache: job range outside the cache rows");
    const size_t jw = (size_t)2 * rowf;
    for (int job = job0; job < job1; job++) {
        const int bi = job / s, i = job % s;
        SFG_HIP(ctx, hipMemcpy2DAsync(cache + (((size_t)(bi - row0) * d) * s + i) * jw, (size_t)s * jw * 8, staged + (size_t)(job - job0) * d * jw, jw * 8, jw * 8, d,
                                      hipMemcpyDeviceToDevice, ctx->stream));
    }
    SFG_HIP(ctx, hipMemsetAsync(cache + (size_t)nrows * d * s * jw, 0, (size_t)3 * s * jw * 8, ctx->stream));
    return 0;
}
int rotcache_build_rows_tab(sfg_ctx *ctx, const u64 *A, int s, int in_level, int max_level, int nbr, int b0, int b1, const std::vector<std::vector<uint8_t>> *tabs, double *cache) {
    ctx->i8_gen++;
    SFG_HIP(ctx, hipSetDevice(ctx->device));
    const int N = SFG_N, d = SFG_D, L = max_level;
    size_t rowf = 0; SFG_TRY(rotcache_rowf(ctx, L, rowf));
    const int lev = in_level > max_level ? max_level : in_level, nl = lev + 1;
    if (nl < L || in_level >= ctx->nq) SFG_FAIL(ctx, "rotcache: input level %d unusable with max_level = %d", in_level, max_level);
    if (s < 1 || b0 < 0 || b1 > nbr || b0 > b1) SFG_FAIL(ctx, "rotcache: block-row range out of bounds");
    const size_t ctw = (size_t)2 * nl * N, per_row = (size_t)d * s * 2 * rowf;
    u64 *a_row = nullptr, *rotc = nullptr;
    SFG_TRY(sfg_scratch(ctx, "mm.a_row", (size_t)s * ctw * 8, (void **)&a_row));
    SFG_TRY(sfg_scratch(ctx, "mm.rotc", 8, (void **)&rotc));
    const std::vector<uint8_t> all(d, 1);
    for (int bi = b0; bi < b1; bi++)
        SFG_TRY(build_rot_row_tab(ctx, A, s, in_level + 1, nl, lev, L, nbr, bi, tabs ? (*tabs)[bi - b0] : all, a_row, rotc, true, cache + (size_t)(bi - b0) * per_row));
    SFG_HIP(ctx, hipMemsetAsync(cache + (size_t)(b1 - b0) * per_row, 0, (size_t)3 * s * 2 * rowf * 8, ctx->stream));
    return 0;
}
extern "C" int sfg_rotcache_build_rows_dev(sfg_ctx *ctx, const uint64_t *A, int s, int in_level, int max_level, int nbr, int b0, int b1, double *cache) {
    ApiScope api_scope(ctx);
    return rotcache_build_rows_tab(ctx, (const u64 *)A, s, in_level, max_level, nbr, b0, b1, nullptr, cache);
}
void i8_rotpre_free(I8RotPre &pre) { pre = I8RotPre(); }
int i8_rotpre_build(sfg_ctx *ctx, const u64 *A, int s, int in_level, int max_level, int nbr, const std::vector<std::vector<uint8_t>> *tabs, size_t budget_bytes, const char *prefix, I8RotPre &pre) {
    pre = I8RotPre();
    const int d = SFG_D, L = max_level;
    const auto &c = ctx->cfg;
    if (!mac_use_dma(ctx) || !c.mac_bc || c.mac_plain_pt || !c.mac_i8 || !c.mac_i8_big || 2 * s > 30 || L < 1 || L > ctx->nq || nbr < 1) return 0;
    if (!mac_dma_packed_mask(ctx, L)) return 0;
    const ModSplit m(ctx->q, L);
    const int l_big = m.l_big, l_s0 = m.l_small0, n_s = m.nsmall; const int *plane_of = m.plane_of;
    const size_t rowf = (size_t)m.fp64_planes * SFG_N;
    size_t have = 0, tot = 0; bool mem_failed = false;
    if (c.mm_group_auto && nbr > c.mm_group) {
        mem_failed = hipMemGetInfo(&have, &tot) != hipSuccess;
        for (const auto &kv : ctx->pool) if (kv.first.rfind(prefix, 0) == 0 || kv.first == "mm.pt" || kv.first == "mm.rotf" || kv.first.rfind("mi8.", 0) == 0) have += kv.second.second;
    }
    int G = i8pre_group_size(m, c.mm_group, c.mm_group_auto, s, nbr, mem_failed, have, budget_bytes);
    if (!G) return 0;
    double *tmp = nullptr;
    auto alloc_all = [&](int Gc) -> bool {
        const int ngc = (nbr + Gc - 1) / Gc;
        pre.As.assign(ngc, nullptr); pre.Ab.assign(ngc, nullptr);
        int arc = sfg_scratch(ctx, "mm.rotf", ((size_t)Gc * d + 3) * s * 2 * rowf * 8, (void **)&tmp);
        for (int gi = 0; gi < ngc && !arc; gi++) {
            const int ng = std::min(Gc, nbr - gi * Gc);
            char nm[48];
            snprintf(nm, sizeof nm, "%s.s%d", prefix, gi);
            arc = sfg_scratch(ctx, nm, mac_i8_rot_tile_bytes(ng * d, n_s, 5), (void **)&pre.As[gi]);
            if (!arc && l_big >= 0) { snprintf(nm, sizeof nm, "%s.b%d", prefix, gi); arc = sfg_scratch(ctx, nm, mac_i8_rot_tile_bytes(ng * d, 1, 6), (void **)&pre.Ab[gi]); }
        }
        if (arc) { ctx->err.clear(); i8_rotpre_free(pre); }
        return !arc;
    };
    if (!alloc_all(G)) {
        const int G0 = std::min(c.mm_group, nbr);
        if (G0 == G) return 0;
        G = G0;
        if (!alloc_all(G)) return 0;
    }
    const int ngrp = (nbr + G - 1) / G;
    for (int gi = 0; gi < ngrp; gi++) {
        const int bg = gi * G, ng = std::min(G, nbr - bg);
        std::vector<std::vector<uint8_t>> sub;
        if (tabs) sub.assign(tabs->begin() + bg, tabs->begin() + bg + ng);
        int rc = rotcache_build_rows_tab(ctx, A, s, in_level, max_level, nbr, bg, bg + ng, tabs ? &sub : nullptr, tmp);
        if (!rc) rc = launch_i8_pack_rot_to(ctx, tmp, (size_t)s * 2 * rowf, rowf, plane_of[l_s0], ng * d, 2 * s, l_s0, n_s, false, pre.As[gi]);
        if (!rc && l_big >= 0) rc = launch_i8_pack_rot_to(ctx, tmp, (size_t)s * 2 * rowf, rowf, plane_of[l_big], ng * d, 2 * s, l_big, 1, true, pre.Ab[gi]);
        if (rc) { i8_rotpre_free(pre); return rc; }
    }
    pre.G = G; pre.nbr = nbr; pre.s = s; pre.L = L;
    return 0;
}
int matmul_resident_range_i8pre(sfg_ctx *ctx, const I8RotPre &pre, int s, int max_level, const sfg_geno *g, unsigned flags, int blk0, int blk1, uint64_t *out) {
    ApiScope api_scope(ctx);
    if (!pre.G) SFG_FAIL(ctx, "matmul: no int8 rot tiles");
    return matmul_resident_range(ctx, nullptr, s, max_level, max_level, g, flags, blk0, blk1, out, nullptr, &pre);
}
int matmul_accumulate_i8pre(sfg_ctx *ctx, const I8RotPre &pre, int s, int max_level, const sfg_geno *g, unsigned flags, int j0, int j1, int accumulate, uint64_t *acc, size_t acc_col_words) {
    ApiScope api_scope(ctx);
    SFG_HIP(ctx, hipSetDevice(ctx->device));
    if (!pre.G) SFG_FAIL(ctx, "matmul: no int8 rot tiles");
    Shape sh = make_shape(g, flags);
    return matmul_accumulate(ctx, nullptr, s, max_level, max_level, sh, flags, 0, pre.nbr, j0, j1, accumulate, (u64 *)acc, nullptr, nullptr, &pre, acc_col_words);
}
extern "C" int sfg_matmul_resident_range_rc_dev(sfg_ctx *ctx, const double *cache, int s, int max_level, const sfg_geno *g, unsigned flags,
                                                int blk0, int blk1, uint64_t *out) {
    ApiScope api_scope(ctx);
    if (!cache) SFG_FAIL(ctx, "matmul: null rotation cache");
    return matmul_resident_range(ctx, nullptr, s, max_level, max_level, g, flags, blk0, blk1, out, cache);
}
extern "C" int sfg_matmul_accumulate_rc_dev(sfg_ctx *ctx, const double *cache, int s, int max_level, const sfg_geno *g, unsigned flags,
                                            int b0, int b1, int j0, int j1, int accumulate, uint64_t *acc) {
    ApiScope api_scope(ctx);
    SFG_HIP(ctx, hipSetDevice(ctx->device));
    if (!cache) SFG_FAIL(ctx, "matmul: null rotation cache");
    if (!mac_use_dma(ctx)) SFG_FAIL(ctx, "matmul: a prebuilt rotation cache needs the LDS-DMA MAC (the A/B build selected the register-staged kernel)");
    Shape sh = make_shape(g, flags);
    return matmul_accumulate(ctx, nullptr, s, max_level, max_level, sh, flags, b0, b1, j0, j1, accumulate, (u64 *)acc, cache, nullptr);
}

extern "C" int sfg_matmul_resident_dev(sfg_ctx *ctx, const uint64_t *A, int s, int in_level, int max_level, const sfg_geno *g, unsigned flags, uint64_t *out) {
    ApiScope api_scope(ctx);
    const size_t nb = (g->ncol + SFG_SLOTS - 1) / SFG_SLOTS;
    return sfg_matmul_resident_range_dev(ctx, A, s, in_level, max_level, g, flags, 0, (int)nb, out);
}

extern "C" int sfg_matmul_stream(sfg_ctx *ctx, const uint64_t *A_host, int s, int in_level, int max_level,
                                 const int8_t *geno_host, size_t nrow, size_t ncol, size_t ld, unsigned flags,
                                 uint64_t *out_host, double *sum_host, double *sqsum_host) {
    ApiScope api_scope(ctx);
    SFG_HIP(ctx, hipSetDevice(ctx->device));
    sfg_geno *g = nullptr;
    SFG_TRY(sfg_geno_upload(ctx, geno_host, nrow, ncol, ld, &g));
    Shape sh = make_shape(g, flags);
    const size_t a_words = (size_t)s * sh.nbr * 2 * (in_level + 1) * SFG_N, o_words = (size_t)s * sh.m_ct * 2 * max_level * SFG_N;
    u64 *dA = nullptr, *dO = nullptr; int rc = 0;
    if (hipMalloc(&dA, a_words * 8) != hipSuccess || hipMalloc(&dO, o_words * 8) != hipSuccess) { rc = 1; ctx->err = "matmul_stream: out of device memory"; }
    if (!rc && hipMemcpy(dA, A_host, a_words * 8, hipMemcpyHostToDevice) != hipSuccess) { rc = 1; ctx->err = "matmul_stream: upload failed"; }
    if (!rc && (sum_host || sqsum_host)) rc = sfg_geno_colsums(ctx, g, sum_host, sqsum_host);
    if (!rc) rc = sfg_matmul_resident_dev(ctx, (const uint64_t *)dA, s, in_level, max_level, g, flags, (uint64_t *)dO);
    if (!rc && (hipMemcpyAsync(out_host, dO, o_words * 8, hipMemcpyDeviceToHost, ctx->stream) != hipSuccess ||
                hipStreamSynchronize(ctx->stream) != hipSuccess)) { rc = 1; ctx->err = "matmul_stream: download failed"; }
    (void)hipStreamSynchronize(ctx->stream);
    (void)hipFree(dA); (void)hipFree(dO); sfg_geno_free(ctx, g);
    if (!rc) rc = sfg_encoder_check(ctx);
    return rc;
}


struct DiagCacheHdr { uint64_t vectorLen, level, n, numModuli, rowSize; double scale; std::vector<uint8_t> baby, giant; long data_pos; };
static int dc_open(sfg_ctx *ctx, const std::string &fn, FILE **fp, DiagCacheHdr &h) {
    FILE *f = fopen(fn.c_str(), "rb");
    if (!f) SFG_FAIL(ctx, "matmul_from_cache: cannot open %s", fn.c_str());
    unsigned char b[48];
    auto le = [&](int k) { uint64_t v = 0; for (int i = 0; i < 8; i++) v |= (uint64_t)b[8 * k + i] << (8 * i); return v; };
    h.baby.assign(SFG_D, 0); h.giant.assign(SFG_D, 0);
    if (fread(b, 1, 48, f) != 48 || fread(h.baby.data(), 1, SFG_D, f) != (size_t)SFG_D || fread(h.giant.data(), 1, SFG_D, f) != (size_t)SFG_D) { fclose(f); SFG_FAIL(ctx, "matmul_from_cache: short header in %s", fn.c_str()); }
    h.vectorLen = le(0); h.level = le(1); uint64_t sb = le(2); memcpy(&h.scale, &sb, 8); h.n = le(3); h.numModuli = le(4); h.rowSize = le(5);
    h.data_pos = ftell(f);
    *fp = f; return 0;
}
__global__ void __launch_bounds__(256) k_cache_to_panel(const u64 *raw, const uint8_t *present, u64 *panel, int jp, int L, unsigned packed_mask,
                                                        const u64 *r64inv, const ModConst *modc, unsigned long long *asym) {
    const int N = SFG_N, n = N / 2;
    const size_t row = blockIdx.x / (n / 256);
    const int l = (int)(row % L); const size_t bj = row / L; const int j = (int)(bj % jp), baby = (int)(bj / jp);
    const int x = (int)(blockIdx.x % (n / 256)) * 256 + threadIdx.x;
    u64 *dst = panel + (((size_t)j * SFG_D + baby) * L + l) * n;
    const bool packed = (packed_mask >> l) & 1u;
    if (!present[bj]) { dst[x] = packed ? PACKED_ZERO : 0ULL; return; }
    const u64 *src = raw + row * N;
    const u64 be = src[x], bm = src[N - 1 - x];
    if (be != bm) atomicAdd(asym, 1ULL);
    const u64 w = __builtin_bswap64(be);
    const u64 v = d_mulmod_u64(w % modc[l].qi, r64inv[l], modc[l].qi);
    dst[x] = packed ? pack_limbs(v) : v;
}

__global__ void __launch_bounds__(256) k_cache_payload(const u64 *pt, u64 *out, int LV, const u64 *r64, const ModConst *modc) {
    const int N = SFG_N; const size_t row = blockIdx.x / (N / 256); const int l = (int)(row % LV);
    const size_t x = row * N + (blockIdx.x % (N / 256)) * 256 + threadIdx.x;
    out[x] = __builtin_bswap64(d_mulmod_u64(pt[x], r64[l], modc[l].qi));
}
extern "C" int sfg_diagcache_write(sfg_ctx *ctx, const sfg_geno *g, unsigned flags, int max_level, const char *prefix, int *files_written) {
    ApiScope api_scope(ctx);
    SFG_HIP(ctx, hipSetDevice(ctx->device));
    if (files_written) *files_written = 0;
    if (!g || !prefix) SFG_FAIL(ctx, "sfg_diagcache_write: null argument");
    if (flags & ~SFG_TRANSPOSE) SFG_FAIL(ctx, "sfg_diagcache_write: only the transpose flag is meaningful here (MatMult4StreamPreprocess neither squares nor sums)");
    const int LV = max_level + 1;
    if (max_level < 1 || LV > ctx->nq) SFG_FAIL(ctx, "sfg_diagcache_write: max_level out of range");
    if (g->packed) {
        sfg_geno *u = nullptr; SFG_TRY(sfg_geno_unpack(ctx, g, &u));
        const int rc = sfg_diagcache_write(ctx, u, flags, max_level, prefix, files_written); sfg_geno_free(ctx, u); return rc;
    }
    const Shape sh = make_shape(g, flags);
    const int N = SFG_N, d = SFG_D, slots = SFG_SLOTS;
    const size_t ptw = (size_t)LV * N;
    const size_t row_size = 4 + (1 + ptw * 8) * (size_t)sh.m_ct;
    u64 r64_h[SFG_MAXMOD];
    for (int l = 0; l < LV; l++) { const unsigned __int128 t = ((unsigned __int128)1 << 64) % ctx->q[l]; r64_h[l] = (u64)t; }
    u64 *r64_d = nullptr; int8_t *skew = nullptr; u64 *half = nullptr, *full = nullptr, *pay_d = nullptr; unsigned char *pay_h = nullptr;
    const int BATCH = 64;
    SFG_TRY(sfg_scratch(ctx, "dcw.r64", SFG_MAXMOD * 8, (void **)&r64_d));
    SFG_TRY(sfg_scratch(ctx, "enc.skew", (size_t)slots * slots, (void **)&skew));
    SFG_TRY(sfg_scratch(ctx, "enc.half", (size_t)BATCH * LV * (N / 2) * 8, (void **)&half));
    SFG_TRY(sfg_scratch(ctx, "dcw.full", (size_t)BATCH * ptw * 8, (void **)&full));
    SFG_TRY(sfg_scratch(ctx, "dcw.pay", (size_t)BATCH * ptw * 8, (void **)&pay_d));
    SFG_HIP(ctx, hipMemcpyAsync(r64_d, r64_h, SFG_MAXMOD * 8, hipMemcpyHostToDevice, ctx->stream));
    SFG_HIP(ctx, hipHostMalloc((void **)&pay_h, (size_t)BATCH * ptw * 8, hipHostMallocDefault));
    int rc = 0, written = 0;
    for (int bi = 0; bi < sh.nbr && !rc; bi++) {
        const std::string fn = std::string(prefix) + "_" + std::to_string(bi) + ".bin";
        if (FILE *t = fopen(fn.c_str(), "rb")) { fclose(t); continue; }
        const int nr = sh.rows_of(bi);
        std::vector<uint8_t> baby_t(d, 0), giant_t(d, 0), shift_t(slots, 0);
        std::vector<std::vector<uint8_t>> has(sh.m_ct, std::vector<uint8_t>(slots, 0));
        for (int shift = 0; shift < slots; shift++) {
            bool any = false;
            for (int bj = 0; bj < sh.m_ct; bj++) { has[bj][shift] = diag_bool(nr, sh.cols_of(bj), slots, -shift) ? 1 : 0; any = any || has[bj][shift]; }
            if (any) { baby_t[shift % d] = 1; giant_t[shift / d] = 1; shift_t[shift] = 1; }
        }
        const std::string tmp = fn + ".part";
        FILE *f = fopen(tmp.c_str(), "wb");
        if (!f) { ctx->err = "sfg_diagcache_write: cannot create " + tmp; rc = 1; break; }
        {
            uint64_t sb; const double sc = ctx->scale; memcpy(&sb, &sc, 8);
            const uint64_t hdr[6] = {(uint64_t)sh.m_ct, (uint64_t)max_level, sb, (uint64_t)N, (uint64_t)LV, (uint64_t)row_size};
            unsigned char hb[48]; for (int k = 0; k < 6; k++) for (int i = 0; i < 8; i++) hb[8 * k + i] = (unsigned char)(hdr[k] >> (8 * i));
            if (fwrite(hb, 1, 48, f) != 48 || fwrite(baby_t.data(), 1, d, f) != (size_t)d || fwrite(giant_t.data(), 1, d, f) != (size_t)d) rc = 1;
        }
        std::vector<long long> rec_pos(slots, -1); long long pos = 48 + 2 * d;
        for (int shift = 0; shift < slots && !rc; shift++) if (shift_t[shift]) {
            size_t len = 4; for (int bj = 0; bj < sh.m_ct; bj++) len += 1 + (has[bj][shift] ? ptw * 8 : 0);
            unsigned char head[12]; for (int i = 0; i < 8; i++) head[i] = (unsigned char)((uint64_t)len >> (8 * i));
            for (int i = 0; i < 4; i++) head[8 + i] = (unsigned char)((uint32_t)shift >> (8 * i));
            if (fseeko(f, pos, SEEK_SET) || fwrite(head, 1, 12, f) != 12) { rc = 1; break; }
            rec_pos[shift] = pos + 12; pos += 8 + (long long)len;
        }
        for (int bj = 0; bj < sh.m_ct && !rc; bj++) {
            const int nc = sh.cols_of(bj);
            rc = launch_skew(ctx, sh.block(bi, bj), sh.ld, nr, nc, sh.transposed ? 1 : 0, 0, skew);
            for (int s0 = 0; s0 < slots && !rc; s0 += BATCH) {
                int lo = -1, hi = -1;
                for (int sft = s0; sft < std::min(slots, s0 + BATCH); sft++) if (has[bj][sft]) { if (lo < 0) lo = sft; hi = sft + 1; }
                if (lo >= 0) {
                    const int nb = hi - lo;
                    rc = launch_encode_rows(ctx, skew, lo, nb, LV, half, true);
                    if (!rc) rc = launch_expand_half(ctx, half, full, (size_t)nb * LV);
                    if (!rc) {
                        hipLaunchKernelGGL(k_cache_payload, dim3((unsigned)((size_t)nb * LV * (N / 256))), dim3(256), 0, ctx->stream, full, pay_d, LV, r64_d, ctx->modc);
                        if (hipGetLastError() != hipSuccess || hipMemcpyAsync(pay_h, pay_d, (size_t)nb * ptw * 8, hipMemcpyDeviceToHost, ctx->stream) != hipSuccess ||
                            hipStreamSynchronize(ctx->stream) != hipSuccess) { ctx->err = "sfg_diagcache_write: device work failed"; rc = 1; }
                    }
                }
                for (int sft = s0; sft < std::min(slots, s0 + BATCH) && !rc; sft++) if (shift_t[sft]) {
                    long long off = rec_pos[sft]; for (int k = 0; k < bj; k++) off += 1 + (has[k][sft] ? (long long)ptw * 8 : 0);
                    const unsigned char flag = has[bj][sft] ? 0 : 1;
                    if (fseeko(f, off, SEEK_SET) || fwrite(&flag, 1, 1, f) != 1) { rc = 1; break; }
                    if (has[bj][sft] && fwrite(pay_h + (size_t)(sft - lo) * ptw * 8, 1, ptw * 8, f) != ptw * 8) { rc = 1; break; }
                }
            }
        }
        if (fclose(f)) rc = 1;
        if (!rc && rename(tmp.c_str(), fn.c_str())) rc = 1;
        if (rc) { remove(tmp.c_str()); if (ctx->err.empty()) ctx->err = "sfg_diagcache_write: I/O error on " + fn; break; }
        written++;
    }
    (void)hipHostFree(pay_h);
    if (files_written) *files_written = written;
    if (!rc) rc = sfg_encoder_check(ctx);
    return rc;
}

extern "C" int sfg_diagcache_header(sfg_ctx *ctx, const char *prefix, int block_row, uint64_t hdr[6]) {
    FILE *f = nullptr; DiagCacheHdr h;
    SFG_TRY(dc_open(ctx, std::string(prefix) + "_" + std::to_string(block_row) + ".bin", &f, h));
    fclose(f);
    uint64_t sb; memcpy(&sb, &h.scale, 8);
    hdr[0] = h.vectorLen; hdr[1] = h.level; hdr[2] = sb; hdr[3] = h.n; hdr[4] = h.numModuli; hdr[5] = h.rowSize;
    return 0;
}

extern "C" int sfg_matmul_from_cache(sfg_ctx *ctx, const uint64_t *A, int s, int in_level, int max_level, const char *prefix, int nbr, uint64_t *out) {
    ApiScope api_scope(ctx);
    SFG_HIP(ctx, hipSetDevice(ctx->device));
    ctx->phases.clear();
    if (!mac_use_dma(ctx)) SFG_FAIL(ctx, "matmul_from_cache needs the LDS-DMA MAC (the A/B build selected the register-staged kernel)");
    const int N = SFG_N, d = SFG_D, L = max_level;
    if (L < 1 || L > ctx->nq) SFG_FAIL(ctx, "matmul_from_cache: max_level out of range");
    const int lev = in_level > max_level ? max_level : in_level, nl = lev + 1, nl_in = in_level + 1;
    if (nl < L) SFG_FAIL(ctx, "matmul_from_cache: input level %d has fewer than max_level = %d moduli", in_level, max_level);
    if (nbr < 1) SFG_FAIL(ctx, "matmul_from_cache: no block rows");
    std::vector<DiagCacheHdr> hdrs(nbr); std::vector<FILE *> files(nbr, nullptr);
    auto close_all = [&]() { for (FILE *f : files) if (f) fclose(f); };
    for (int bi = 0; bi < nbr; bi++) {
        if (dc_open(ctx, std::string(prefix) + "_" + std::to_string(bi) + ".bin", &files[bi], hdrs[bi])) { close_all(); return 1; }
        const DiagCacheHdr &h = hdrs[bi];
        long fsize = -1; { const long here = ftell(files[bi]); if (!fseek(files[bi], 0, SEEK_END)) fsize = ftell(files[bi]); fseek(files[bi], here, SEEK_SET); }
        if (h.n != (uint64_t)N || h.numModuli < (uint64_t)L || h.numModuli > (uint64_t)ctx->nmod || h.vectorLen != hdrs[0].vectorLen || h.vectorLen < 1 ||
            h.vectorLen > (1u << 20) || h.rowSize != 4 + (1 + h.n * h.numModuli * 8) * h.vectorLen || fsize < 0 || h.rowSize > (uint64_t)fsize) {
            close_all(); SFG_FAIL(ctx, "matmul_from_cache: %s_%d.bin does not match this ring (n = %llu, numModuli = %llu, vectorLen = %llu)", prefix, bi,
                                  (unsigned long long)h.n, (unsigned long long)h.numModuli, (unsigned long long)h.vectorLen);
        }
    }
    const int m_ct = (int)hdrs[0].vectorLen;
    std::vector<uint8_t> giant_t(d, 0);
    for (auto &h : hdrs) for (int g = 0; g < d; g++) giant_t[g] |= h.giant[g];
    const size_t accw = (size_t)s * 2 * L * N, ctw = (size_t)2 * nl * N, prow = (size_t)N / 2, plw = (size_t)L * prow;
    std::vector<int> plane_of, is_big; const int nplanes = mac_dma_planes(ctx, L, plane_of, is_big);
    if (nplanes < 0) { close_all(); return 1; }
    const size_t rowf = (size_t)nplanes * N;
    const unsigned packed_mask = mac_dma_packed_mask(ctx, L);
    int jp = (int)(ctx->cfg.acc_budget / ((size_t)d * accw * 8)); if (jp < 1) jp = 1; if (jp > m_ct) jp = m_ct;
    u64 *a_row = nullptr, *rotc = nullptr, *acc = nullptr, *panel = nullptr, *raw_d = nullptr, *inv_d = nullptr; double *rotf = nullptr, *rotsum = nullptr;
    uint8_t *present_d = nullptr; unsigned long long *asym_d = nullptr; u64 *raw_h = nullptr;
    int rc = 0;
    auto bail = [&](int r) { close_all(); if (raw_h) (void)hipHostFree(raw_h); return r; };
    if (sfg_scratch(ctx, "mm.a_row", (size_t)s * ctw * 8, (void **)&a_row) || sfg_scratch(ctx, "mm.rotc", 8, (void **)&rotc) ||
        sfg_scratch(ctx, "mm.rotf", ((size_t)d + 3) * s * 2 * rowf * 8, (void **)&rotf) || sfg_scratch(ctx, "mm.rotsum", (size_t)2 * s * 2 * rowf * 8, (void **)&rotsum) ||
        sfg_scratch(ctx, "mm.acc", (size_t)jp * d * accw * 8, (void **)&acc) || sfg_scratch(ctx, "dc.panel", (size_t)jp * d * plw * 8, (void **)&panel) ||
        sfg_scratch(ctx, "dc.raw", (size_t)d * jp * L * N * 8 + (size_t)d * jp + 64 + 8 * SFG_MAXMOD, (void **)&raw_d)) return bail(1);
    present_d = (uint8_t *)(raw_d + (size_t)d * jp * L * N);
    asym_d = (unsigned long long *)(present_d + (((size_t)d * jp + 63) & ~(size_t)63)); inv_d = (u64 *)(asym_d + 1);
    if (hipHostMalloc((void **)&raw_h, (size_t)d * jp * L * N * 8 + (size_t)d * jp, hipHostMallocDefault) != hipSuccess) { ctx->err = "matmul_from_cache: hipHostMalloc failed"; return bail(1); }
    uint8_t *present_h = (uint8_t *)(raw_h + (size_t)d * jp * L * N);
    {
        u64 inv[SFG_MAXMOD] = {0};
        for (int l = 0; l < L; l++) { const u64 q = ctx->q[l]; inv[l] = h_invmod((u64)((((u128)1) << 64) % q), q); }
        if (hipMemcpyAsync(inv_d, inv, sizeof inv, hipMemcpyHostToDevice, ctx->stream) != hipSuccess || hipMemsetAsync(asym_d, 0, 8, ctx->stream) != hipSuccess ||
            hipStreamSynchronize(ctx->stream) != hipSuccess) { ctx->err = "matmul_from_cache: setup copy failed"; return bail(1); }
    }
    std::vector<unsigned char> rec;
    for (int ja = 0; ja < m_ct && !rc; ja += jp) {
        const int jn = std::min(jp, m_ct - ja);
        if (hipMemsetAsync(acc, 0, (size_t)jn * d * accw * 8, ctx->stream) != hipSuccess) { ctx->err = "matmul_from_cache: memset failed"; rc = 1; break; }
        for (int bi = 0; bi < nbr && !rc; bi++) {
            const DiagCacheHdr &h = hdrs[bi]; FILE *f = files[bi];
            fseek(f, h.data_pos, SEEK_SET);
            try { rec.resize(h.rowSize); } catch (const std::exception &) { ctx->err = "matmul_from_cache: out of host memory for a record"; rc = 1; break; }
            rc = build_rot_row_tab(ctx, (const u64 *)A, s, nl_in, nl, lev, L, nbr, bi, h.baby, a_row, rotc, true, rotf);
            if (!rc && hipMemsetAsync(rotf + (size_t)d * s * 2 * rowf, 0, (size_t)3 * s * 2 * rowf * 8, ctx->stream) != hipSuccess) rc = 1;
            if (!rc && packed_mask) rc = launch_rot_sum(ctx, rotf, (size_t)s * 2, d, L, rotsum);
            int cur_giant = -1; bool any = false;
            auto flush = [&]() -> int {
                if (!any) return 0;
                SFG_HIP(ctx, hipMemcpyAsync(raw_d, raw_h, (size_t)d * jn * L * N * 8, hipMemcpyHostToDevice, ctx->stream));
                SFG_HIP(ctx, hipMemcpyAsync(present_d, present_h, (size_t)d * jn, hipMemcpyHostToDevice, ctx->stream));
                hipLaunchKernelGGL(k_cache_to_panel, dim3((unsigned)((size_t)d * jn * L * (N / 2 / 256))), dim3(256), 0, ctx->stream, raw_d, present_d, panel, jn, L, packed_mask,
                                   inv_d, ctx->modc, asym_d);
                SFG_HIP(ctx, hipGetLastError());
                MacStrides st;
                st.rot_k = (size_t)s * ctw; st.rot_r = (size_t)nl * N;
                st.pt_k = plw; st.pt_n = (size_t)d * plw; st.pt_half = true; st.pt_packed = packed_mask != 0; st.i8 = ctx->cfg.mac_i8 && packed_mask; st.i8_big = st.i8 && ctx->cfg.mac_i8_big;
                st.out_n = (size_t)d * accw; st.out_r = (size_t)L * N;
                PhaseTimer t(ctx, "mac");
                int r2 = launch_mac_dma(ctx, rotf, (size_t)s * 2, panel, acc + (size_t)cur_giant * accw, d, 2 * s, jn, L, 1, st, rotsum);
                t.stop(1);
                SFG_HIP(ctx, hipStreamSynchronize(ctx->stream));
                any = false;
                return r2;
            };
            while (!rc) {
                unsigned char l8[8];
                if (fread(l8, 1, 8, f) != 8) break;
                uint64_t len = 0; for (int i = 0; i < 8; i++) len |= (uint64_t)l8[i] << (8 * i);
                if (len > h.rowSize || len < 4 || fread(rec.data(), 1, len, f) != len) { ctx->err = "matmul_from_cache: truncated record"; rc = 1; break; }
                const int shift = (int)((uint32_t)rec[0] | (uint32_t)rec[1] << 8 | (uint32_t)rec[2] << 16 | (uint32_t)rec[3] << 24);
                if (shift < 0 || shift >= SFG_SLOTS) { ctx->err = "matmul_from_cache: shift out of range"; rc = 1; break; }
                const int giant = shift / d, baby = shift % d;
                if (giant != cur_giant) { rc = flush(); if (rc) break; cur_giant = giant; memset(present_h, 0, (size_t)d * jn); }
                size_t ptr = 4; const size_t plain_bytes = (size_t)h.n * h.numModuli * 8;
                for (uint64_t j = 0; j < h.vectorLen; j++) {
                    if (ptr >= len) { ctx->err = "matmul_from_cache: malformed record"; rc = 1; break; }
                    const bool empty = rec[ptr++] == 1;
                    if (empty) continue;
                    if (ptr + plain_bytes > len) { ctx->err = "matmul_from_cache: malformed record"; rc = 1; break; }
                    if ((int)j >= ja && (int)j < ja + jn) {
                        memcpy(raw_h + ((size_t)baby * jn + (j - ja)) * L * N, rec.data() + ptr, (size_t)L * N * 8);
                        present_h[(size_t)baby * jn + (j - ja)] = 1; any = true;
                    }
                    ptr += plain_bytes;
                }
            }
            if (!rc) rc = flush();
        }
        if (!rc) rc = matmul_finalize(ctx, acc, s, max_level, jn, m_ct, ja, 0, d, &giant_t, 0, (u64 *)out);
        if (!rc && hipStreamSynchronize(ctx->stream) != hipSuccess) rc = 1;
    }
    unsigned long long asym = 0;
    if (!rc && hipMemcpy(&asym, asym_d, 8, hipMemcpyDeviceToHost) != hipSuccess) rc = 1;
    if (!rc && asym) { ctx->err = "matmul_from_cache: cached plaintexts are not mirror-symmetric (not encodings of real slot vectors)"; rc = 1; }
    return bail(rc);
}
```

sfgwas_amd/csrc/ntt.hip:

```cpp
#include "common.hpp"
#include "kernels.hpp"
#include "i8_move.hpp"
#include "ntt_core.hpp"

template <int IN_MODE>
__global__ void __launch_bounds__(512) k_ntt_fwd(const void *in_, u64 *out_, ModPattern pat, RowMap rm, const double *tw_all, const double2 *pack_all, const ModConst *modc) {
    extern __shared__ double lds[];
    const int N = SFG_N, tid = threadIdx.x;
    const size_t row = blockIdx.x;
    const int m = pat.m[row % pat.period];
    const size_t grp = row / rm.rpg, gi = row % rm.rpg;
    if (m == -2) return;
    if (m < 0) {
        const u64 *src = (const u64 *)in_ + grp * rm.gstride_in + gi * N; u64 *dst = out_ + grp * rm.gstride_out + gi * N;
        if (IN_MODE == 0 && src != dst) for (int a = 0; a < 32; a++) dst[a * 512 + tid] = src[a * 512 + tid];
        return;
    }
    const double *tw = tw_all + (size_t)m * N;
    const double2 *pack = pack_all + (size_t)m * (N / 2);
    const double q = modc[m].q, qinv = modc[m].qinv;
    double v[32];
    if (IN_MODE == 0) {
        const u64 *in = (const u64 *)in_ + grp * rm.gstride_in + gi * N;
#pragma unroll
        for (int a = 0; a < 32; a++) v[a] = u64_to_f64(in[a * 512 + tid]);
    } else {
        const double *pc = (const double *)in_ + (row / pat.period) * (size_t)(N / 2);
#pragma unroll
        for (int a = 0; a < 16; a++) v[a] = pred(pc[a * 512 + tid], q, qinv);
#pragma unroll
        for (int a = 16; a < 32; a++) {
            int x = (a - 16) * 512 + tid;
            v[a] = x == 0 ? 0.0 : -pred(pc[N / 2 - x], q, qinv);
        }
    }
    ntt_fwd_phases(v, lds, tw, pack, q, qinv, tid);
    u64 *out = out_ + grp * rm.gstride_out + gi * N;
    {
        const int b = tid >> 4, c = tid & 15;
#pragma unroll
        for (int a = 0; a < 32; a++) out[a * 512 + tid] = f64_to_u64(canon(lds[a * LDS_ROW + c * 33 + b], q, qinv));
    }
}

__global__ void __launch_bounds__(512) k_ntt_inv(const u64 *in_, u64 *out_, ModPattern pat, RowMap rm, const double *tw_all, const double2 *pack_all, const ModConst *modc) {
    extern __shared__ double lds[];
    const int N = SFG_N, tid = threadIdx.x;
    const size_t row = blockIdx.x;
    const int m = pat.m[row % pat.period];
    if (m < 0) return;
    const size_t grp = row / rm.rpg, gi = row % rm.rpg;
    const double *tw = tw_all + (size_t)m * N;
    const double2 *pack = pack_all + (size_t)m * (N / 2);
    const double q = modc[m].q, qinv = modc[m].qinv;
    const u64 *in = in_ + grp * rm.gstride_in + gi * N;
    double v[32];
    {
        const int b = tid >> 4, c = tid & 15;
#pragma unroll
        for (int a = 0; a < 32; a++) lds[a * LDS_ROW + c * 33 + b] = u64_to_f64(in[a * 512 + tid]);
    }
    __syncthreads();
#pragma unroll
    for (int h = 0; h < 2; h++) {
        const int p = tid + 512 * h, a = p >> 5, b = p & 31;
        double w[16];
#pragma unroll
        for (int c = 0; c < 16; c++) w[c] = lds[a * LDS_ROW + c * 33 + b];
        double tl[16];
        {
            const double2 *pk = pack + (size_t)(p >> 6) * 512 + (p & 63);
#pragma unroll
            for (int i = 0; i < 8; i++) { const double2 e = pk[i * 64]; tl[2 * i] = e.x; tl[2 * i + 1] = e.y; }
        }
        gs_stage<16, 1>(w, q, qinv, [&](int g) { return tl[7 + g]; });
        gs_stage<16, 2>(w, q, qinv, [&](int g) { return tl[3 + g]; });
        gs_stage<16, 4>(w, q, qinv, [&](int g) { return tl[1 + g]; });
        gs_stage<16, 8>(w, q, qinv, [&](int g) { return tl[0 + g]; });
#pragma unroll
        for (int c = 0; c < 16; c++) v[h * 16 + c] = pred(w[c], q, qinv);
    }
    __syncthreads();
#pragma unroll
    for (int h = 0; h < 2; h++) {
        const int p = tid + 512 * h, a = p >> 5, b = p & 31;
#pragma unroll
        for (int c = 0; c < 16; c++) lds[a * LDS_ROW + c * 33 + b] = v[h * 16 + c];
    }
    __syncthreads();
    {
        const int a = tid >> 4, c = tid & 15;
#pragma unroll
        for (int b = 0; b < 32; b++) v[b] = lds[a * LDS_ROW + c * 33 + b];
        gs_stage<32, 1>(v, q, qinv, [&](int g) { return tw[512 + a * 16 + g]; });
        gs_stage<32, 2>(v, q, qinv, [&](int g) { return tw[256 + a * 8 + g]; });
        gs_stage<32, 4>(v, q, qinv, [&](int g) { return tw[128 + a * 4 + g]; });
        gs_stage<32, 8>(v, q, qinv, [&](int g) { return tw[64 + a * 2 + g]; });
        gs_stage<32, 16>(v, q, qinv, [&](int g) { return tw[32 + a + g]; });
        __syncthreads();
#pragma unroll
        for (int b = 0; b < 32; b++) lds[a * LDS_ROW + b * 16 + c] = pred(v[b], q, qinv);
    }
    __syncthreads();
#pragma unroll
    for (int a = 0; a < 32; a++) v[a] = lds[a * LDS_ROW + tid];
    gs_stage<32, 1>(v, q, qinv, [&](int g) { return tw[16 + g]; });
    gs_stage<32, 2>(v, q, qinv, [&](int g) { return tw[8 + g]; });
    gs_stage<32, 4>(v, q, qinv, [&](int g) { return tw[4 + g]; });
    gs_stage<32, 8>(v, q, qinv, [&](int g) { return tw[2 + g]; });
    gs_stage<32, 16>(v, q, qinv, [&](int g) { return tw[1 + g]; });
    const double ninv = modc[m].ninv, ninv_q = modc[m].ninv_q;
    u64 *out = out_ + grp * rm.gstride_out + gi * N;
#pragma unroll
    for (int a = 0; a < 32; a++) {
        double x = mulmod_lazy(pred(v[a], q, qinv), ninv, ninv_q, q);
        out[a * 512 + tid] = f64_to_u64(canon(x, q, qinv));
    }
}

constexpr int H3_ROWA = 264;
constexpr int H3_WREG = 4 * 272;
constexpr int H3_DOUBLES = 16 * H3_ROWA > 4 * H3_WREG ? 16 * H3_ROWA : 4 * H3_WREG;
constexpr int H3_LDS_BYTES = H3_DOUBLES * 8;
struct NoFill {};
template <class First, class Store, class Fill = NoFill, bool WIDE = false>
__device__ __forceinline__ void ntt_half3_body(int hs, First first, Store store, double *lds, const double *tw, const double2 *pack, double q, double qinv, int tid, Fill fill = Fill()) {
    double v[32];
    const int a_b = tid >> 4, c_b = tid & 15;
    double w2[2][16];
    if constexpr (std::is_same<Fill, NoFill>::value) {
#pragma unroll
        for (int h = 0; h < 2; h++)
#pragma unroll
            for (int a = 0; a < 16; a++) w2[h][a] = first(a * 512 + tid + 256 * h);
    } else fill(w2);
#pragma unroll
    for (int h = 0; h < 2; h++) {
        double (&w)[16] = w2[h];
        ct_stage<16, 8>(w, q, qinv, [&](int g) { return tw[2 + hs + g]; });
        ct_stage<16, 4>(w, q, qinv, [&](int g) { return tw[4 + 2 * hs + g]; });
        ct_stage<16, 2>(w, q, qinv, [&](int g) { return tw[8 + 4 * hs + g]; });
        ct_stage<16, 1>(w, q, qinv, [&](int g) { return tw[16 + 8 * hs + g]; });
        if (h) __syncthreads();
#pragma unroll
        for (int a = 0; a < 16; a++) lds[a * H3_ROWA + tid] = w[a];
        __syncthreads();
#pragma unroll
        for (int b = 0; b < 16; b++) v[h * 16 + b] = lds[a_b * H3_ROWA + b * 16 + c_b];
    }
    const int ab = 16 * hs + a_b;
    ct_stage<32, 16>(v, q, qinv, [&](int g) { return tw[32 + ab + g]; });
    ct_stage<32, 8>(v, q, qinv, [&](int g) { return tw[64 + ab * 2 + g]; });
    ct_stage<32, 4>(v, q, qinv, [&](int g) { return tw[128 + ab * 4 + g]; });
    ct_stage<32, 2>(v, q, qinv, [&](int g) { return tw[256 + ab * 8 + g]; });
    ct_stage<32, 1>(v, q, qinv, [&](int g) { return tw[512 + ab * 16 + g]; });
    __syncthreads();
    {
        const int wv = tid >> 6, lane = tid & 63, al = lane >> 4, bk = lane & 15;
        double *img = lds + wv * H3_WREG;
        auto sw = [](int idx) { return (idx >> 8) * 272 + ((idx >> 4) & 15) * 17 + (idx & 15); };
#pragma unroll
        for (int r = 0; r < 2; r++) {
            double wc[16];
            __builtin_amdgcn_fence(__ATOMIC_ACQ_REL, "wavefront");
#pragma unroll
            for (int k = 0; k < 16; k++) img[sw(al * 256 + c_b * 16 + k)] = v[16 * r + k];
            __builtin_amdgcn_fence(__ATOMIC_ACQ_REL, "wavefront");
#pragma unroll
            for (int c = 0; c < 16; c++) wc[c] = img[sw(al * 256 + c * 16 + bk)];
            const int p = a_b * 32 + 16 * r + bk;
            double tl[16];
            {
                const double2 *pk = pack + (size_t)((p >> 6) + 8 * hs) * 512 + (p & 63);
#pragma unroll
                for (int i = 0; i < 8; i++) {
                    const double2 e = pk[i * 64];
                    tl[2 * i] = e.x; tl[2 * i + 1] = e.y;
                }
            }
            ct_stage<16, 8>(wc, q, qinv, [&](int g) { return tl[0 + g]; });
            ct_stage<16, 4>(wc, q, qinv, [&](int g) { return tl[1 + g]; });
            ct_stage<16, 2>(wc, q, qinv, [&](int g) { return tl[3 + g]; });
            ct_stage<16, 1>(wc, q, qinv, [&](int g) { return tl[7 + g]; });
            __builtin_amdgcn_fence(__ATOMIC_ACQ_REL, "wavefront");
#pragma unroll
            for (int c = 0; c < 16; c++) img[sw(al * 256 + c * 16 + bk)] = wc[c];
            __builtin_amdgcn_fence(__ATOMIC_ACQ_REL, "wavefront");
#pragma unroll
            for (int ai = 0; ai < 4; ai++) {
                if constexpr (WIDE) {
                    const int x0 = 4 * lane;
                    const int base = ai * 256 + (lane >> 2);
                    store((4 * wv + ai) * 512 + 256 * r + x0, img[sw(base + (4 * (lane & 3) + 0) * 16)], img[sw(base + (4 * (lane & 3) + 1) * 16)],
                          img[sw(base + (4 * (lane & 3) + 2) * 16)], img[sw(base + (4 * (lane & 3) + 3) * 16)]);
                } else {
#pragma unroll
                    for (int qd = 0; qd < 4; qd++) {
                        const int x = qd * 64 + lane;
                        store((4 * wv + ai) * 512 + 256 * r + x, img[sw(ai * 256 + (x & 15) * 16 + (x >> 4))]);
                    }
                }
            }
        }
    }
}
#define NT_ST(p, v) __builtin_nontemporal_store((unsigned)(v), (p))
template <bool PERM, bool DIG>
__device__ __forceinline__ void ntt_half3_wg(size_t vb, double *lds, const double *pc_all, u64 *out_, size_t nplain, int L, PanelMap pm, const double *tw_all, const double2 *pack_all,
                                             const ModConst *modc, const uint32_t *perm) {
    const int N = SFG_N, n = N / 2, tid = threadIdx.x;
    size_t row; int m;
    if (!plain_block_of(vb, nplain, L, row, m)) return;
    const double *tw = tw_all + (size_t)m * N;
    const double2 *pack = pack_all + (size_t)m * (N / 2);
    const double q = modc[m].q, qinv = modc[m].qinv;
    const double *pc = pc_all + (row / L) * (size_t)n;
    unsigned gal = 1;
    if (PERM) { const uint32_t e = perm[pm.shift0 + (int)(row / L)]; pc = pc_all + (size_t)(e & 0xFFFFu) * n; gal = e >> 16; }
    const double W = tw[1], Wq = W * qinv;
    auto first = [&](int j) { const double lo = pc[j], hi = j == 0 ? 0.0 : pc[n - j]; return lo - mulmod_lazy(hi, W, Wq, q); };
    auto fill = [&](double (&w2)[2][16]) {
        double rA[16], rB[16];
#pragma unroll
        for (int k = 0; k < 16; k++) {
            const int i = tid + 256 * k;
            const double lo = pc[i], hi = i == 0 ? 0.0 : pc[n - i];
            const unsigned qd = (((unsigned)i * gal) & (2u * N - 1u)) >> 13;
            const double ca = (qd == 1u || qd == 2u) ? -lo : lo, cb = qd >= 2u ? -hi : hi;
            rA[k] = ca - mulmod_lazy(cb, W, Wq, q);
            rB[k] = cb - mulmod_lazy(ca, W, Wq, q);
        }
#pragma unroll
        for (int h = 0; h < 2; h++) {
#pragma unroll
            for (int k = 0; k < 16; k++) {
                const unsigned raw = ((unsigned)(tid + 256 * k) * gal) & (2u * N - 1u), qd = raw >> 13;
                const int J = qd == 0u ? (int)raw : qd == 1u ? N - (int)raw : qd == 2u ? (int)raw - N : 2 * N - (int)raw, Jb = n - J;
                if (((J >> 8) & 1) == h && J < n) lds[(J >> 9) * H3_ROWA + (J & 255)] = rA[k];
                if (((Jb >> 8) & 1) == h && Jb < n) lds[(Jb >> 9) * H3_ROWA + (Jb & 255)] = rB[k];
            }
            __syncthreads();
#pragma unroll
            for (int a = 0; a < 16; a++) w2[h][a] = lds[a * H3_ROWA + tid];
            __syncthreads();
        }
        if (tid == 0) {
            const double mid = pc[n / 2];
            const double c = ((((unsigned)(n / 2) * gal) & (2u * N - 1u)) >> 13) >= 2u ? -mid : mid;
            w2[0][8] = c - mulmod_lazy(c, W, Wq, q);
        }
    };
    const size_t plain = row / L; const int shift = pm.shift0 + (int)plain;
    const size_t dst = pm.G ? ((size_t)(shift / SFG_D) * pm.G + pm.g) * SFG_D + (size_t)(shift % SFG_D) : plain;
    u64 *out = out_ + (dst * L + m) * (size_t)n;
    size_t dstride = n, cbm = 0;
    if constexpr (DIG) if (pm.packed_mask & PT_COMPACT) {
        const unsigned lm = (1u << L) - 1u, small = pm.packed_mask & lm;
        const int ns_all = __popc(small), ns_below = __popc(small & ((1u << m) - 1u));
        const size_t planes_all = (size_t)ns_all * 5 + (size_t)(L - ns_all) * 6, planes_below = (size_t)ns_below * 5 + (size_t)(m - ns_below) * 6;
        if (pm.packed_mask & PT_KMAJOR) {
            const size_t K = (size_t)pm.K, col = pm.G ? (size_t)(shift / SFG_D) : plain / K, row = pm.G ? (size_t)pm.g * SFG_D + (size_t)(shift % SFG_D) : plain % K;
            out = reinterpret_cast<u64 *>(reinterpret_cast<uint8_t *>(out_) + ((col * planes_all + planes_below) * 64 * K + row) * 128);
            dstride = 64 * K * 128; cbm = K * 128 - 128;
        } else out = reinterpret_cast<u64 *>(reinterpret_cast<uint8_t *>(out_) + dst * (planes_all * n) + planes_below * n);
    }
    if constexpr (DIG) if (!((pm.packed_mask >> m) & 1u) && (pm.packed_mask & PT_DIGITS_BIG)) {
        uint8_t *o8 = reinterpret_cast<uint8_t *>(out);
        auto dig6 = [&](double x, unsigned &lo, unsigned &hi) {
            const u64 b = (u64)__double_as_longlong(canon(x, q, qinv) + (4503599627370496.0 + 141289400074368.0));
            lo = (unsigned)b ^ 0x80808080u; hi = (unsigned)(b >> 32) ^ 0x8080u;
        };
        auto st6 = [&](int j0, double x0, double x1, double x2, double x3) {
            unsigned l0, l1, l2, l3, h0, h1, h2, h3;
            dig6(x0, l0, h0); dig6(x1, l1, h1); dig6(x2, l2, h2); dig6(x3, l3, h3);
            unsigned o[4]; bytes_tr4(l0, l1, l2, l3, o);
            uint8_t *ob = o8 + j0 + (size_t)(j0 >> 7) * cbm;
#pragma unroll
            for (int d = 0; d < 4; d++) NT_ST(reinterpret_cast<unsigned *>(ob + d * dstride), o[d]);
            unsigned p[4]; bytes_tr4(h0, h1, h2, h3, p);
            NT_ST(reinterpret_cast<unsigned *>(ob + 4 * dstride), p[0]);
            NT_ST(reinterpret_cast<unsigned *>(ob + 5 * dstride), p[1]);
        };
        if constexpr (PERM) ntt_half3_body<decltype(first), decltype(st6), decltype(fill), true>(0, first, st6, lds, tw, pack, q, qinv, tid, fill);
        else ntt_half3_body<decltype(first), decltype(st6), NoFill, true>(0, first, st6, lds, tw, pack, q, qinv, tid);
        return;
    }
    if constexpr (DIG) if ((pm.packed_mask >> m) & 1u) {
        uint8_t *o8 = reinterpret_cast<uint8_t *>(out);
        auto dig = [&](double x, unsigned &lo, unsigned &hi) {
            const u64 b = (u64)__double_as_longlong(canon_le(x, q, qinv) + (4503599627370496.0 + 551911719040.0));
            lo = (unsigned)b ^ 0x80808080u; hi = (unsigned)(b >> 32) ^ 0x80u;
        };
        auto st8 = [&](int j0, double x0, double x1, double x2, double x3) {
            unsigned l0, l1, l2, l3, h0, h1, h2, h3;
            dig(x0, l0, h0); dig(x1, l1, h1); dig(x2, l2, h2); dig(x3, l3, h3);
            unsigned o[4]; bytes_tr4(l0, l1, l2, l3, o);
            uint8_t *ob = o8 + j0 + (size_t)(j0 >> 7) * cbm;
#pragma unroll
            for (int d = 0; d < 4; d++) NT_ST(reinterpret_cast<unsigned *>(ob + d * dstride), o[d]);
            NT_ST(reinterpret_cast<unsigned *>(ob + 4 * dstride), (h0 & 255u) | ((h1 & 255u) << 8) | ((h2 & 255u) << 16) | (h3 << 24));
        };
        if constexpr (PERM) ntt_half3_body<decltype(first), decltype(st8), decltype(fill), true>(0, first, st8, lds, tw, pack, q, qinv, tid, fill);
        else ntt_half3_body<decltype(first), decltype(st8), NoFill, true>(0, first, st8, lds, tw, pack, q, qinv, tid);
        return;
    }
    if constexpr (PERM) {
        if (!DIG && ((pm.packed_mask >> m) & 1u)) ntt_half3_body(0, first, [&](int j, double x) { out[j] = pack_limbs_f64(canon_le(x, q, qinv)); }, lds, tw, pack, q, qinv, tid, fill);
        else ntt_half3_body(0, first, [&](int j, double x) { out[j] = f64_to_u64(canon(x, q, qinv)); }, lds, tw, pack, q, qinv, tid, fill);
    } else {
        (void)fill;
        if (!DIG && ((pm.packed_mask >> m) & 1u)) ntt_half3_body(0, first, [&](int j, double x) { out[j] = pack_limbs_f64(canon_le(x, q, qinv)); }, lds, tw, pack, q, qinv, tid);
        else ntt_half3_body(0, first, [&](int j, double x) { out[j] = f64_to_u64(canon(x, q, qinv)); }, lds, tw, pack, q, qinv, tid);
    }
}
template <bool PERM, bool DIG>
__global__ void __launch_bounds__(256, 4) k_ntt_half3(const double *pc_all, u64 *out_, size_t nplain, int L, PanelMap pm, const double *tw_all, const double2 *pack_all, const ModConst *modc,
                                                      const uint32_t *perm) {
    extern __shared__ double lds[];
    ntt_half3_wg<PERM, DIG>(blockIdx.x, lds, pc_all, out_, nplain, L, pm, tw_all, pack_all, modc, perm);
}
template <bool PERM, int DEPTH, bool NT>
__global__ void __launch_bounds__(256, 4) k_ntt_half3_move(const double *pc_all, u64 *out_, size_t nplain, int L, PanelMap pm, const double *tw_all, const double2 *pack_all, const ModConst *modc,
                                                           const uint32_t *perm, MoveJob job) {
    extern __shared__ double lds[];
    if (blockIdx.x < job.nblocks) { i8_move_block<DEPTH, NT>(job, blockIdx.x, reinterpret_cast<unsigned *>(lds), (int)threadIdx.x); return; }
    ntt_half3_wg<PERM, true>((size_t)blockIdx.x - job.nblocks, lds, pc_all, out_, nplain, L, pm, tw_all, pack_all, modc, perm);
}
__global__ void __launch_bounds__(256, 4) k_ntt_fwd_split(const u64 *in_, u64 *out_, size_t nrows, ModPattern pat, RowMap rm, const double *tw_all, const double2 *pack_all, const ModConst *modc) {
    extern __shared__ double lds[];
    const int N = SFG_N, n = N / 2, tid = threadIdx.x;
    const size_t b = blockIdx.x, row = (b / 16) * 8 + b % 8; const int hs = (int)((b / 8) & 1);
    if (row >= nrows) return;
    const int m = pat.m[row % pat.period];
    const size_t grp = row / rm.rpg, gi = row % rm.rpg;
    const u64 *in = in_ + grp * rm.gstride_in + gi * N;
    u64 *out = out_ + grp * rm.gstride_out + gi * N + (size_t)hs * n;
    if (m == -2) return;
    if (m < 0) {
        for (int k = 0; k < 32; k++) out[k * 256 + tid] = in[(size_t)hs * n + k * 256 + tid];
        return;
    }
    const double *tw = tw_all + (size_t)m * N;
    const double2 *pack = pack_all + (size_t)m * (N / 2);
    const double q = modc[m].q, qinv = modc[m].qinv;
    const double W = hs ? -tw[1] : tw[1], Wq = W * qinv;
    auto first = [&](int j) { return u64_to_f64(in[j]) + mulmod_lazy(u64_to_f64(in[n + j]), W, Wq, q); };
    ntt_half3_body(hs, first, [&](int j, double x) { out[j] = f64_to_u64(canon(x, q, qinv)); }, lds, tw, pack, q, qinv, tid);
}
__global__ void __launch_bounds__(256) k_expand_half(const u64 *half, u64 *full) {
    const int N = SFG_N, n = N / 2; const size_t row = blockIdx.x / (n / 256);
    const int i = (int)(blockIdx.x % (n / 256)) * 256 + threadIdx.x;
    const u64 v = half[row * n + i];
    full[row * N + i] = v; full[row * N + (N - 1 - i)] = v;
}

int ntt_set_attrs(sfg_ctx *ctx) {
    hipError_t e = hipFuncSetAttribute((const void *)k_ntt_fwd<0>, hipFuncAttributeMaxDynamicSharedMemorySize, LDS_DOUBLES * 8);
    if (e == hipSuccess) e = hipFuncSetAttribute((const void *)k_ntt_fwd<1>, hipFuncAttributeMaxDynamicSharedMemorySize, LDS_DOUBLES * 8);
    if (e == hipSuccess) e = hipFuncSetAttribute((const void *)k_ntt_inv, hipFuncAttributeMaxDynamicSharedMemorySize, LDS_DOUBLES * 8);
    if (e == hipSuccess) e = hipFuncSetAttribute((const void *)k_ntt_half3<false, false>, hipFuncAttributeMaxDynamicSharedMemorySize, H3_LDS_BYTES);
    if (e == hipSuccess) e = hipFuncSetAttribute((const void *)k_ntt_half3<true, false>, hipFuncAttributeMaxDynamicSharedMemorySize, H3_LDS_BYTES);
    if (e == hipSuccess) e = hipFuncSetAttribute((const void *)k_ntt_half3<false, true>, hipFuncAttributeMaxDynamicSharedMemorySize, H3_LDS_BYTES);
    if (e == hipSuccess) e = hipFuncSetAttribute((const void *)k_ntt_half3<true, true>, hipFuncAttributeMaxDynamicSharedMemorySize, H3_LDS_BYTES);
    if (e == hipSuccess) e = hipFuncSetAttribute((const void *)k_ntt_fwd_split, hipFuncAttributeMaxDynamicSharedMemorySize, H3_LDS_BYTES);
#define SFG_MV_ATTR(P, D, T) if (e == hipSuccess) e = hipFuncSetAttribute((const void *)k_ntt_half3_move<P, D, T>, hipFuncAttributeMaxDynamicSharedMemorySize, H3_LDS_BYTES)
    SFG_MV_ATTR(false, 1, true); SFG_MV_ATTR(true, 1, true);
#ifdef SFG_AB
    SFG_MV_ATTR(false, 1, false); SFG_MV_ATTR(false, 2, false); SFG_MV_ATTR(false, 2, true); SFG_MV_ATTR(false, 3, false); SFG_MV_ATTR(false, 3, true);
    SFG_MV_ATTR(true, 1, false); SFG_MV_ATTR(true, 2, false); SFG_MV_ATTR(true, 2, true); SFG_MV_ATTR(true, 3, false); SFG_MV_ATTR(true, 3, true);
    if (e == hipSuccess && ab_set_attrs(ctx)) return 1;
#endif
#undef SFG_MV_ATTR
    if (e != hipSuccess) SFG_FAIL(ctx, "cannot raise dynamic LDS limit for the NTT kernels");
    return 0;
}

static RowMap dense_map() { RowMap rm; rm.rpg = 1; rm.gstride_in = SFG_N; rm.gstride_out = SFG_N; return rm; }
int launch_ntt_fwd(sfg_ctx *ctx, const u64 *in, u64 *out, size_t nrows, const ModPattern &pat) { return launch_ntt_fwd_map(ctx, in, out, nrows, pat, dense_map()); }
int launch_ntt_inv(sfg_ctx *ctx, const u64 *in, u64 *out, size_t nrows, const ModPattern &pat) { return launch_ntt_inv_map(ctx, in, out, nrows, pat, dense_map()); }
int launch_ntt_fwd_map(sfg_ctx *ctx, const u64 *in, u64 *out, size_t nrows, const ModPattern &pat, const RowMap &rm) {
    if (!nrows) return 0;
    if (in != out && !ctx->cfg.ntt_fwd_full)
        hipLaunchKernelGGL(k_ntt_fwd_split, dim3((unsigned)((nrows + 7) / 8 * 16)), dim3(256), H3_LDS_BYTES, ctx->stream, in, out, nrows, pat, rm, ctx->tw_fwd, ctx->pack_fwd, ctx->modc);
    else
        hipLaunchKernelGGL(k_ntt_fwd<0>, dim3((unsigned)nrows), dim3(512), LDS_DOUBLES * 8, ctx->stream, (const void *)in, out, pat, rm, ctx->tw_fwd, ctx->pack_fwd, ctx->modc);
    SFG_HIP(ctx, hipGetLastError());
    return 0;
}
int launch_ntt_plain(sfg_ctx *ctx, const double *pc, u64 *out, size_t nplain, int L) {
    if (!nplain) return 0;
    ModPattern pat; pat.period = L; for (int l = 0; l < L; l++) pat.m[l] = (int8_t)l;
    hipLaunchKernelGGL(k_ntt_fwd<1>, dim3((unsigned)(nplain * L)), dim3(512), LDS_DOUBLES * 8, ctx->stream, (const void *)pc, out, pat, dense_map(), ctx->tw_fwd, ctx->pack_fwd, ctx->modc);
    SFG_HIP(ctx, hipGetLastError());
    return 0;
}
template <bool PERM>
static int launch_half3_move(sfg_ctx *ctx, dim3 grid, const double *pc, u64 *out_half, size_t nplain, int L, PanelMap pm, const uint32_t *perm, const MoveJob &j) {
#define SFG_MV(D, T) hipLaunchKernelGGL((k_ntt_half3_move<PERM, D, T>), grid, dim3(256), H3_LDS_BYTES, ctx->stream, pc, out_half, nplain, L, pm, ctx->tw_fwd, ctx->pack_fwd, ctx->modc, perm, j)
    if (j.depth == 1 && j.nt) { SFG_MV(1, true); return 0; }
#ifdef SFG_AB
    if (j.depth == 3) { if (j.nt) SFG_MV(3, true); else SFG_MV(3, false); return 0; }
    if (j.depth == 2) { if (j.nt) SFG_MV(2, true); else SFG_MV(2, false); return 0; }
    if (j.depth == 1) { SFG_MV(1, false); return 0; }
#endif
#undef SFG_MV
    SFG_FAIL(ctx, "plaintext NTT: the product build holds the mover with one unit in flight and streaming accesses only (other forms: make ab)");
}
int launch_ntt_plain_half(sfg_ctx *ctx, const double *pc, u64 *out_half, size_t nplain, int L, PanelMap pm, const uint32_t *perm, const MoveJob *mv) {
    if (!nplain) return 0;
    const dim3 grid((unsigned)((nplain + 7) / 8 * 8 * L));
    const bool dig = pm.packed_mask & PT_DIGITS;
    if (mv && mv->count) {
        if (!dig || mv->nblocks % 8 || !mv->nblocks) SFG_FAIL(ctx, "plaintext NTT: mover workgroups need the digit-plane form and a multiple of 8 of them");
        const dim3 g2(grid.x + mv->nblocks);
        if (perm) SFG_TRY(launch_half3_move<true>(ctx, g2, pc, out_half, nplain, L, pm, perm, *mv));
        else SFG_TRY(launch_half3_move<false>(ctx, g2, pc, out_half, nplain, L, pm, (const uint32_t *)nullptr, *mv));
        SFG_HIP(ctx, hipGetLastError());
        return 0;
    }
    if (perm && dig) hipLaunchKernelGGL((k_ntt_half3<true, true>), grid, dim3(256), H3_LDS_BYTES, ctx->stream, pc, out_half, nplain, L, pm, ctx->tw_fwd, ctx->pack_fwd, ctx->modc, perm);
    else if (perm) hipLaunchKernelGGL((k_ntt_half3<true, false>), grid, dim3(256), H3_LDS_BYTES, ctx->stream, pc, out_half, nplain, L, pm, ctx->tw_fwd, ctx->pack_fwd, ctx->modc, perm);
    else if (dig) hipLaunchKernelGGL((k_ntt_half3<false, true>), grid, dim3(256), H3_LDS_BYTES, ctx->stream, pc, out_half, nplain, L, pm, ctx->tw_fwd, ctx->pack_fwd, ctx->modc, (const uint32_t *)nullptr);
#ifdef SFG_AB
    else if (ctx->cfg.ntt_half_full) ab_launch_ntt_half_full(ctx, pc, out_half, nplain, L, pm);
#endif
    else hipLaunchKernelGGL((k_ntt_half3<false, false>), grid, dim3(256), H3_LDS_BYTES, ctx->stream, pc, out_half, nplain, L, pm, ctx->tw_fwd, ctx->pack_fwd, ctx->modc, (const uint32_t *)nullptr);
    SFG_HIP(ctx, hipGetLastError());
    return 0;
}
int launch_expand_half(sfg_ctx *ctx, const u64 *half, u64 *full, size_t nrows) {
    if (!nrows) return 0;
    hipLaunchKernelGGL(k_expand_half, dim3((unsigned)(nrows * (SFG_N / 2 / 256))), dim3(256), 0, ctx->stream, half, full);
    SFG_HIP(ctx, hipGetLastError());
    return 0;
}
int launch_ntt_inv_map(sfg_ctx *ctx, const u64 *in, u64 *out, size_t nrows, const ModPattern &pat, const RowMap &rm) {
    if (!nrows) return 0;
    hipLaunchKernelGGL(k_ntt_inv, dim3((unsigned)nrows), dim3(512), LDS_DOUBLES * 8, ctx->stream, in, out, pat, rm, ctx->tw_inv, ctx->pack_inv, ctx->modc);
    SFG_HIP(ctx, hipGetLastError());
    return 0;
}

static int pattern_from_host(sfg_ctx *ctx, const int *mod_idx, int nrows, ModPattern &pat) {
    for (int period = 1; period <= 64 && period <= nrows; period++) {
        bool ok = true;
        for (int r = 0; r < nrows && ok; r++) ok = mod_idx[r] == mod_idx[r % period];
        if (ok) { pat.period = period; for (int i = 0; i < period; i++) { if (mod_idx[i] < 0 || mod_idx[i] >= ctx->nmod) SFG_FAIL(ctx, "modulus index out of range"); pat.m[i] = (int8_t)mod_idx[i]; } return 0; }
    }
    SFG_FAIL(ctx, "mod_idx must be periodic with period <= 64");
}

extern "C" int sfg_ntt_rows(sfg_ctx *ctx, uint64_t *rows, int nrows, const int *mod_idx) {
    SFG_HIP(ctx, hipSetDevice(ctx->device));
    ModPattern pat; SFG_TRY(pattern_from_host(ctx, mod_idx, nrows, pat));
    return launch_ntt_fwd(ctx, (const u64 *)rows, (u64 *)rows, nrows, pat);
}
extern "C" int sfg_intt_rows(sfg_ctx *ctx, uint64_t *rows, int nrows, const int *mod_idx) {
    SFG_HIP(ctx, hipSetDevice(ctx->device));
    ModPattern pat; SFG_TRY(pattern_from_host(ctx, mod_idx, nrows, pat));
    return launch_ntt_inv(ctx, (const u64 *)rows, (u64 *)rows, nrows, pat);
}
```

sfgwas_amd/csrc/ntt_core.hpp:

```cpp
#pragma once
#include "common.hpp"

constexpr int LDS_ROW = 528;
constexpr int LDS_DOUBLES = 32 * LDS_ROW;

template <int LEN, int H, class TW>
__device__ __forceinline__ void ct_stage(double (&v)[LEN], double q, double qinv, TW tw) {
#pragma unroll
    for (int g = 0; g < LEN / (2 * H); g++) {
        const double w = tw(g);
#pragma unroll
        for (int x = 0; x < H; x++) {
            const int i0 = g * 2 * H + x, i1 = i0 + H;
            double r = mulmod_lazy_q(v[i1], w, q, qinv);
            double U = v[i0];
            v[i0] = U + r; v[i1] = U - r;
        }
    }
}
template <int LEN, int H, class TW>
__device__ __forceinline__ void gs_stage(double (&v)[LEN], double q, double qinv, TW tw) {
#pragma unroll
    for (int g = 0; g < LEN / (2 * H); g++) {
        const double w = tw(g);
#pragma unroll
        for (int x = 0; x < H; x++) {
            const int i0 = g * 2 * H + x, i1 = i0 + H;
            double U = v[i0], V = v[i1];
            v[i0] = U + V;
            v[i1] = mulmod_lazy_q(U - V, w, q, qinv);
        }
    }
}

__device__ __forceinline__ void ntt_fwd_phases(double (&v)[32], double *lds, const double *tw, const double2 *pack, double q, double qinv, int tid) {
    ct_stage<32, 16>(v, q, qinv, [&](int g) { return tw[1 + g]; });
    ct_stage<32, 8>(v, q, qinv, [&](int g) { return tw[2 + g]; });
    ct_stage<32, 4>(v, q, qinv, [&](int g) { return tw[4 + g]; });
    ct_stage<32, 2>(v, q, qinv, [&](int g) { return tw[8 + g]; });
    ct_stage<32, 1>(v, q, qinv, [&](int g) { return tw[16 + g]; });
#pragma unroll
    for (int a = 0; a < 32; a++) lds[a * LDS_ROW + tid] = v[a];
    __syncthreads();
    {
        const int a = tid >> 4, c = tid & 15;
#pragma unroll
        for (int b = 0; b < 32; b++) v[b] = lds[a * LDS_ROW + b * 16 + c];
        ct_stage<32, 16>(v, q, qinv, [&](int g) { return tw[32 + a + g]; });
        ct_stage<32, 8>(v, q, qinv, [&](int g) { return tw[64 + a * 2 + g]; });
        ct_stage<32, 4>(v, q, qinv, [&](int g) { return tw[128 + a * 4 + g]; });
        ct_stage<32, 2>(v, q, qinv, [&](int g) { return tw[256 + a * 8 + g]; });
        ct_stage<32, 1>(v, q, qinv, [&](int g) { return tw[512 + a * 16 + g]; });
        __syncthreads();
#pragma unroll
        for (int b = 0; b < 32; b++) lds[a * LDS_ROW + c * 33 + b] = v[b];
    }
    __syncthreads();
#pragma unroll
    for (int h = 0; h < 2; h++) {
        const int p = tid + 512 * h, a = p >> 5, b = p & 31;
        double w[16];
#pragma unroll
        for (int c = 0; c < 16; c++) w[c] = lds[a * LDS_ROW + c * 33 + b];
        double tl[16];
        {
            const double2 *pk = pack + (size_t)(p >> 6) * 512 + (p & 63);
#pragma unroll
            for (int i = 0; i < 8; i++) { const double2 e = pk[i * 64]; tl[2 * i] = e.x; tl[2 * i + 1] = e.y; }
        }
        ct_stage<16, 8>(w, q, qinv, [&](int g) { return tl[0 + g]; });
        ct_stage<16, 4>(w, q, qinv, [&](int g) { return tl[1 + g]; });
        ct_stage<16, 2>(w, q, qinv, [&](int g) { return tl[3 + g]; });
        ct_stage<16, 1>(w, q, qinv, [&](int g) { return tl[7 + g]; });
#pragma unroll
        for (int c = 0; c < 16; c++) v[h * 16 + c] = w[c];
    }
    __syncthreads();
#pragma unroll
    for (int h = 0; h < 2; h++) {
        const int p = tid + 512 * h, a = p >> 5, b = p & 31;
#pragma unroll
        for (int c = 0; c < 16; c++) lds[a * LDS_ROW + c * 33 + b] = v[h * 16 + c];
    }
    __syncthreads();
}
__device__ __forceinline__ bool plain_block_of(size_t b, size_t nplain, int L, size_t &row, int &m) {
    const size_t per = (size_t)8 * L, plain = (b / per) * 8 + (b % per) % 8;
    m = (int)((b % per) / 8); row = plain * L + m;
    return plain < nplain;
}
__device__ __forceinline__ bool plain_block(size_t nplain, int L, size_t &row, int &m) { return plain_block_of(blockIdx.x, nplain, L, row, m); }
```

sfgwas_amd/csrc/rotate.hip:

```cpp
#include "common.hpp"
#include "kernels.hpp"
#include "ksw.hpp"


static void fill_ext(const sfg_ctx *ctx, ExtConst &e, const std::vector<int> &src) {
    memset(&e, 0, sizeof e);
    e.a = (int)src.size();
    for (int m = 0; m < e.a; m++) e.src[m] = src[m];
    for (int m = 0; m < e.a; m++) {
        u64 qm = ctx->q[src[m]], h = 1;
        for (int k = 0; k < e.a; k++) if (k != m) h = h_mulmod(h, ctx->q[src[k]] % qm, qm);
        u64 hi = h_invmod(h, qm);
        e.qhat_inv[m] = (double)hi; e.qhat_inv_q[m] = (double)hi / (double)qm;
    }
    for (int t = 0; t < ctx->nmod; t++) {
        u64 qt = ctx->q[t], D = 1 % qt;
        for (int m = 0; m < e.a; m++) {
            u64 ht = 1 % qt;
            for (int k = 0; k < e.a; k++) if (k != m) ht = h_mulmod(ht, ctx->q[src[k]] % qt, qt);
            e.qhat_t[t][m] = (double)ht; e.qhat_t_q[t][m] = (double)ht / (double)qt;
            D = h_mulmod(D, ctx->q[src[m]] % qt, qt);
        }
        e.D_t[t] = (double)D; e.D_t_q[t] = (double)D / (double)qt;
    }
}


int get_ksw(sfg_ctx *ctx, int level, KswConst **dev, KswConst *host) {
    KswConst kc; memset(&kc, 0, sizeof kc);
    kc.level = level; kc.nl = level + 1; kc.np = ctx->np; kc.alpha = ctx->np; kc.nt = kc.nl + kc.np;
    kc.beta = (kc.nl + kc.alpha - 1) / kc.alpha;
    if (kc.alpha > KSW_MAXA || kc.beta > KSW_MAXDIG) SFG_FAIL(ctx, "key-switch shape unsupported (alpha > 4 or beta > 8)");
    if (kc.beta * kc.nt > SFG_MAXPATTERN) SFG_FAIL(ctx, "key-switch shape unsupported (beta * (level + 1 + np) = %d rows exceed the modulus pattern table)", kc.beta * kc.nt);
    for (int t = 0; t < kc.nt; t++) { kc.tmod[t] = t < kc.nl ? t : ctx->nq + (t - kc.nl); kc.digit_of[t] = t < kc.nl ? t / kc.alpha : -1; }
    for (int i = 0; i < kc.beta; i++) {
        std::vector<int> src;
        for (int m = i * kc.alpha; m < (i + 1) * kc.alpha && m < kc.nl; m++) src.push_back(m);
        fill_ext(ctx, kc.dig[i], src);
    }
    std::vector<int> ps; for (int p = 0; p < kc.np; p++) ps.push_back(ctx->nq + p);
    fill_ext(ctx, kc.pq, ps);
    for (int t = 0; t < kc.nl; t++) {
        u64 qt = ctx->q[t], P = 1;
        for (int p = 0; p < kc.np; p++) P = h_mulmod(P, ctx->q[ctx->nq + p] % qt, qt);
        u64 pi = h_invmod(P, qt);
        kc.pinv[t] = (double)pi; kc.pinv_q[t] = (double)pi / (double)qt;
    }
    *host = kc;
    auto it = ctx->ksw_cache.find(level);
    if (it == ctx->ksw_cache.end()) {
        KswConst *d = nullptr;
        SFG_HIP(ctx, hipMalloc(&d, sizeof(KswConst)));
        SFG_HIP(ctx, hipMemcpy(d, &kc, sizeof(KswConst), hipMemcpyHostToDevice));
        ctx->ksw_cache[level] = d; *dev = d;
    } else *dev = (KswConst *)it->second;
    return 0;
}


__global__ void __launch_bounds__(256) k_ksw_extend(const u64 *c2, const u64 *ct_in, u64 *ext, const KswConst *kcp, const ModConst *modc) {
    const KswConst &kc = *kcp;
    const int N = SFG_N, x = blockIdx.x * 256 + threadIdx.x, i = blockIdx.y; const size_t b = blockIdx.z;
    const ExtConst &e = kc.dig[i];
    const u64 *c2b = c2 + b * (size_t)kc.nl * N;
    u64 *eb = ext + (b * kc.beta + i) * (size_t)kc.nt * N;
    double xs[KSW_MAXA], y[KSW_MAXA], v = 0.0;
#pragma unroll
    for (int m = 0; m < KSW_MAXA; m++) xs[m] = m < e.a ? u64_to_f64(c2b[(size_t)e.src[m] * N + x]) : 0.0;
    if (e.a > 1) ext_prepare(e, modc, xs, y, v);
    for (int t = 0; t < kc.nt; t++) {
        const int tg = kc.tmod[t];
        u64 outv;
        if (kc.digit_of[t] == i) continue;
        else if (e.a == 1) outv = f64_to_u64(canon(xs[0], modc[tg].q, modc[tg].qinv));
        else outv = f64_to_u64(ext_target(e, tg, modc[tg].q, modc[tg].qinv, y, v));
        eb[(size_t)t * N + x] = outv;
    }
}

__global__ void __launch_bounds__(256) k_ksw_inner(const u64 *ext, const u64 *ct_in, const u64 *const *keys, const int *inidx, u64 *acc, const KswConst *kcp, const ModConst *modc, int nmod) {
    const KswConst &kc = *kcp;
    const int N = SFG_N, x = 2 * (blockIdx.x * 256 + threadIdx.x), t = blockIdx.y; const size_t b = blockIdx.z;
    const int tg = kc.tmod[t];
    const double q = modc[tg].q, qinv = modc[tg].qinv;
    const u64 *key = keys[b];
    const size_t bi = (size_t)inidx[b];
    double a0x = 0.0, a0y = 0.0, a1x = 0.0, a1y = 0.0;
    for (int i = 0; i < kc.beta; i++) {
        const ulonglong2 ev = kc.digit_of[t] == i ? *reinterpret_cast<const ulonglong2 *>(ct_in + (bi * 2 * (size_t)kc.nl + kc.nl + t) * N + x)
                                                  : *reinterpret_cast<const ulonglong2 *>(ext + ((bi * kc.beta + i) * (size_t)kc.nt + t) * N + x);
        const ulonglong2 k0 = *reinterpret_cast<const ulonglong2 *>(key + (((size_t)i * 2 + 0) * nmod + tg) * N + x);
        const ulonglong2 k1 = *reinterpret_cast<const ulonglong2 *>(key + (((size_t)i * 2 + 1) * nmod + tg) * N + x);
        const double ex = u64_to_f64(ev.x), ey = u64_to_f64(ev.y);
        a0x += mulmod2(ex, u64_to_f64(k0.x), q, qinv); a0y += mulmod2(ey, u64_to_f64(k0.y), q, qinv);
        a1x += mulmod2(ex, u64_to_f64(k1.x), q, qinv); a1y += mulmod2(ey, u64_to_f64(k1.y), q, qinv);
    }
    *reinterpret_cast<ulonglong2 *>(acc + ((b * 2 + 0) * (size_t)kc.nt + t) * N + x) = make_ulonglong2(f64_to_u64(canon(a0x, q, qinv)), f64_to_u64(canon(a0y, q, qinv)));
    *reinterpret_cast<ulonglong2 *>(acc + ((b * 2 + 1) * (size_t)kc.nt + t) * N + x) = make_ulonglong2(f64_to_u64(canon(a1x, q, qinv)), f64_to_u64(canon(a1y, q, qinv)));
}

__global__ void __launch_bounds__(256) k_moddown_extend(const u64 *acc, u64 *ext2, const KswConst *kcp, const ModConst *modc) {
    const KswConst &kc = *kcp;
    const int N = SFG_N, x = blockIdx.x * 256 + threadIdx.x, p = blockIdx.y; const size_t b = blockIdx.z;
    const ExtConst &e = kc.pq;
    const u64 *ap = acc + ((b * 2 + p) * (size_t)kc.nt + kc.nl) * N;
    double xs[KSW_MAXA], y[KSW_MAXA], v = 0.0;
#pragma unroll
    for (int m = 0; m < KSW_MAXA; m++) xs[m] = m < e.a ? u64_to_f64(ap[(size_t)m * N + x]) : 0.0;
    if (e.a > 1) ext_prepare(e, modc, xs, y, v);
    for (int t = 0; t < kc.nl; t++) {
        u64 outv = e.a == 1 ? f64_to_u64(canon(xs[0], modc[t].q, modc[t].qinv)) : f64_to_u64(ext_target(e, t, modc[t].q, modc[t].qinv, y, v));
        ext2[((b * 2 + p) * (size_t)kc.nl + t) * N + x] = outv;
    }
}

struct F64Form { int on, L, centre; size_t rowf; int plane_of[SFG_MAXMOD], big[SFG_MAXMOD]; };
__device__ __forceinline__ void store_rot_f64(double *row, const F64Form &ff, int t, int x, double v, double q) {
    const int N = SFG_N;
    double *o = row + (size_t)ff.plane_of[t] * N;
    if (ff.big[t]) {
        const double wc = v > __builtin_floor(q * 0.5) ? v - q : v;
        const double hi = __builtin_floor((wc + 4194304.0) * 0x1p-23), lo = wc - hi * 8388608.0;
        o[2 * x] = lo; o[2 * x + 1] = hi;
    } else o[x] = (ff.centre && v > __builtin_floor(q * 0.5)) ? v - q : v;
}
__global__ void __launch_bounds__(256) k_ksw_finish(const u64 *ct_in, const int *inidx, const u64 *acc, const u64 *ext2, const uint16_t *const *index,
                                                   u64 *const *ct_out, const KswConst *kcp, const ModConst *modc, const u64 *add1, F64Form ff) {
    const KswConst &kc = *kcp;
    const int N = SFG_N, x = blockIdx.x * 256 + threadIdx.x, t = blockIdx.y; const size_t b = blockIdx.z;
    if (ff.on && t >= ff.L) return;
    const double q = modc[t].q, qinv = modc[t].qinv, pinv = kc.pinv[t], pinv_q = kc.pinv_q[t];
    const int src = index[b][x];
#pragma unroll
    for (int p = 0; p < 2; p++) {
        const double a = u64_to_f64(acc[((b * 2 + p) * (size_t)kc.nt + t) * N + src]);
        const double e = u64_to_f64(ext2[((b * 2 + p) * (size_t)kc.nl + t) * N + src]);
        double r = mulmod_lazy(a - e, pinv, pinv_q, q);
        if (p == 0) r += u64_to_f64(ct_in[((size_t)inidx[b] * 2 * (size_t)kc.nl + t) * N + src]);
        else if (add1) r += u64_to_f64(add1[((size_t)inidx[b] * (size_t)kc.nl + t) * N + src]);
        const double v = canon(r, q, qinv);
        if (ff.on) store_rot_f64(reinterpret_cast<double *>(ct_out[b]) + (size_t)p * ff.rowf, ff, t, x, v, q);
        else ct_out[b][((size_t)p * kc.nl + t) * N + x] = f64_to_u64(v);
    }
}

__global__ void __launch_bounds__(256) k_ct_add(const u64 *a, const u64 *b, u64 *out, int nl, const ModConst *modc, size_t total_rows) {
    const int N = SFG_N; const size_t row = blockIdx.x / (N / 256); const int m = (int)(row % nl);
    const u64 q = modc[m].qi;
    const size_t off = row * N + (blockIdx.x % (N / 256)) * 256 + threadIdx.x;
    u64 v = a[off] + b[off]; out[off] = v >= q ? v - q : v;
}

static int launch_keyswitch_jobs(sfg_ctx *ctx, const u64 *in, int nin, int level, const std::vector<int> &job_in, const std::vector<const u64 *> &keyp,
                                 const std::vector<const uint16_t *> &idxp, const std::vector<u64 *> &outp, const u64 *add1, const F64Form *ffp = nullptr) {
    const int N = SFG_N, nl = level + 1;
    F64Form ff; memset(&ff, 0, sizeof ff); if (ffp) ff = *ffp;
    KswConst *kcd; KswConst kc;
    SFG_TRY(get_ksw(ctx, level, &kcd, &kc));
    const size_t ctw = (size_t)2 * nl * N;
    const int nr = (int)job_in.size();
    if (!nr) return 0;
    const size_t in_rows = (size_t)nl + (size_t)kc.beta * kc.nt, job_rows = 2 * (size_t)kc.nt + 2 * (size_t)nl;
    const size_t budget = ctx->cfg.ksw_budget;
    int in_grp = (int)(budget / (in_rows * N * 8)); if (in_grp < 1) in_grp = 1; if (in_grp > nin) in_grp = nin;
    int chunk = (int)(budget / (job_rows * N * 8)); if (chunk < 1) chunk = 1; if (chunk > nr) chunk = nr;
    const size_t ptr_bytes = (size_t)nr * (3 * sizeof(void *) + sizeof(int)) + 256;
    const size_t ext_rows = (size_t)in_grp * kc.beta * kc.nt, ext2_rows = (size_t)chunk * 2 * nl;
    SFG_TRY(sfg_ws_reserve(ctx, (in_rows * in_grp + job_rows * chunk + ext_rows + ext2_rows) * N * 8 + ptr_bytes));
    u64 *c2 = (u64 *)ctx->ws, *ext = c2 + (size_t)in_grp * nl * N;
    u64 *acc = ext + ext_rows * N, *ext2 = acc + (size_t)chunk * 2 * kc.nt * N;
    u64 *extT = ext2 + ext2_rows * N, *ext2T = extT + ext_rows * N;
    const u64 **keys_all = (const u64 **)(ext2T + ext2_rows * N);
    const uint16_t **idx_all = (const uint16_t **)(keys_all + nr);
    u64 **out_all = (u64 **)(idx_all + nr);
    int *inidx_all = (int *)(out_all + nr);
    ModPattern pq; pq.period = nl; for (int m = 0; m < nl; m++) pq.m[m] = (int8_t)m;
    ModPattern pext; pext.period = kc.beta * kc.nt;
    for (int i = 0; i < kc.beta; i++) for (int t = 0; t < kc.nt; t++) pext.m[i * kc.nt + t] = kc.digit_of[t] == i ? (int8_t)-2 : (int8_t)kc.tmod[t];
    ModPattern pp; pp.period = kc.np; for (int p = 0; p < kc.np; p++) pp.m[p] = (int8_t)(ctx->nq + p);
    for (int i0 = 0; i0 < nin; i0 += in_grp) {
        const int ni = nin - i0 < in_grp ? nin - i0 : in_grp;
        std::vector<int> jobs;
        for (int k = 0; k < nr; k++) if (job_in[k] >= i0 && job_in[k] < i0 + ni) jobs.push_back(k);
        if (jobs.empty()) continue;
        const u64 *bin = in + (size_t)i0 * ctw;
        RowMap rm1; rm1.rpg = nl; rm1.gstride_in = ctw; rm1.gstride_out = (size_t)nl * N;
        SFG_TRY(launch_ntt_inv_map(ctx, bin + (size_t)nl * N, c2, (size_t)ni * nl, pq, rm1));
        hipLaunchKernelGGL(k_ksw_extend, dim3(N / 256, kc.beta, ni), dim3(256), 0, ctx->stream, c2, bin, ext, kcd, ctx->modc);
        SFG_HIP(ctx, hipGetLastError());
        SFG_TRY(launch_ntt_fwd(ctx, ext, extT, (size_t)ni * kc.beta * kc.nt, pext));
        {
            const size_t nj = jobs.size();
            std::vector<const u64 *> kp(nj); std::vector<const uint16_t *> ip(nj); std::vector<u64 *> op(nj); std::vector<int> ii(nj);
            for (size_t k = 0; k < nj; k++) { int jb = jobs[k]; kp[k] = keyp[jb]; ip[k] = idxp[jb]; op[k] = outp[jb]; ii[k] = job_in[jb] - i0; }
            SFG_TRY(sfg_upload_small(ctx, keys_all, kp.data(), nj * sizeof(void *)));
            SFG_TRY(sfg_upload_small(ctx, idx_all, ip.data(), nj * sizeof(void *)));
            SFG_TRY(sfg_upload_small(ctx, out_all, op.data(), nj * sizeof(void *)));
            SFG_TRY(sfg_upload_small(ctx, inidx_all, ii.data(), nj * sizeof(int)));
        }
        for (size_t c0 = 0; c0 < jobs.size(); c0 += chunk) {
            const int nb = (int)(jobs.size() - c0 < (size_t)chunk ? jobs.size() - c0 : (size_t)chunk);
            const u64 **keys_d = keys_all + c0; const uint16_t **idx_d = idx_all + c0; u64 **out_d = out_all + c0; int *inidx_d = inidx_all + c0;
            hipLaunchKernelGGL(k_ksw_inner, dim3(N / 512, kc.nt, nb), dim3(256), 0, ctx->stream, extT, bin, keys_d, inidx_d, acc, kcd, ctx->modc, ctx->nmod);
            SFG_HIP(ctx, hipGetLastError());
            RowMap rm4; rm4.rpg = kc.np; rm4.gstride_in = (size_t)kc.nt * N; rm4.gstride_out = (size_t)kc.nt * N;
            SFG_TRY(launch_ntt_inv_map(ctx, acc + (size_t)nl * N, acc + (size_t)nl * N, (size_t)nb * 2 * kc.np, pp, rm4));
            hipLaunchKernelGGL(k_moddown_extend, dim3(N / 256, 2, nb), dim3(256), 0, ctx->stream, acc, ext2, kcd, ctx->modc);
            SFG_HIP(ctx, hipGetLastError());
            SFG_TRY(launch_ntt_fwd(ctx, ext2, ext2T, (size_t)nb * 2 * nl, pq));
            hipLaunchKernelGGL(k_ksw_finish, dim3(N / 256, nl, nb), dim3(256), 0, ctx->stream, bin, inidx_d, acc, ext2T, idx_d, out_d, kcd, ctx->modc,
                               add1 ? add1 + (size_t)i0 * nl * N : nullptr, ff);
            SFG_HIP(ctx, hipGetLastError());
        }
    }
    return 0;
}
int launch_rotate_right_indexed(sfg_ctx *ctx, const u64 *in, int nin, u64 *out, int nct, int level, const int *nrot_host, const int *in_index) {
    const int N = SFG_N, nl = level + 1;
    if (level < 0 || level >= ctx->nq) SFG_FAIL(ctx, "rotate: level out of range");
    const size_t ctw = (size_t)2 * nl * N;
    std::vector<int> job_in; std::vector<const u64 *> keyp; std::vector<const uint16_t *> idxp; std::vector<u64 *> outp;
    for (int j = 0; j < nct; j++) {
        int nrot = nrot_host[j] % SFG_SLOTS; if (nrot < 0) nrot += SFG_SLOTS;
        const int src = in_index ? in_index[j] : j;
        if (src < 0 || src >= nin) SFG_FAIL(ctx, "rotate: input index out of range");
        if (nrot == 0) {
            int run = 1;
            while (j + run < nct && (nrot_host[j + run] % SFG_SLOTS) == 0 && (in_index ? in_index[j + run] : j + run) == src + run && src + run < nin) run++;
            SFG_HIP(ctx, hipMemcpyAsync(out + j * ctw, in + (size_t)src * ctw, (size_t)run * ctw * 8, hipMemcpyDeviceToDevice, ctx->stream));
            j += run - 1;
            continue;
        }
        u64 g = sfg_galois_for_rotation(ctx, SFG_SLOTS - nrot);
        auto it = ctx->rotkeys().find(g);
        if (it == ctx->rotkeys().end()) SFG_FAIL(ctx, "rotate: no rotation key loaded for right-rotation by %d (galois element %llu)", nrot, g);
        job_in.push_back(src); keyp.push_back(it->second.key_dev); idxp.push_back(it->second.index_dev); outp.push_back(out + j * ctw);
    }
    return launch_keyswitch_jobs(ctx, in, nin, level, job_in, keyp, idxp, outp, nullptr);
}
int launch_rotate_right_indexed_f64(sfg_ctx *ctx, const u64 *in, int nin, double *outf, int nct, int level, const int *nrot_host, const int *in_index, int L,
                                    const size_t *out_slot) {
    const int N = SFG_N, nl = level + 1;
    ctx->i8_gen++;
    if (level < 0 || level >= ctx->nq || L > nl) SFG_FAIL(ctx, "rotate: level out of range");
    const size_t ctw = (size_t)2 * nl * N;
    std::vector<int> plane_of, is_big; const int nplanes = mac_dma_planes(ctx, L, plane_of, is_big);
    if (nplanes < 0) return 1;
    F64Form ff; memset(&ff, 0, sizeof ff);
    ff.on = 1; ff.L = L; ff.centre = mac_dma_packed_mask(ctx, L) != 0; ff.rowf = (size_t)nplanes * N;
    for (int l = 0; l < L; l++) { ff.plane_of[l] = plane_of[l]; ff.big[l] = is_big[l]; }
    std::vector<int> job_in; std::vector<const u64 *> keyp; std::vector<const uint16_t *> idxp; std::vector<u64 *> outp;
    for (int j = 0; j < nct; j++) {
        int nrot = nrot_host[j] % SFG_SLOTS; if (nrot < 0) nrot += SFG_SLOTS;
        const int src = in_index ? in_index[j] : j;
        if (src < 0 || src >= nin) SFG_FAIL(ctx, "rotate: input index out of range");
        double *dst = outf + (out_slot ? out_slot[j] : (size_t)j) * 2 * ff.rowf;
        if (nrot == 0) {
            int run = 1;
            while (!out_slot && j + run < nct && (nrot_host[j + run] % SFG_SLOTS) == 0 && (in_index ? in_index[j + run] : j + run) == src + run && src + run < nin) run++;
            SFG_TRY(launch_rot_to_f64(ctx, in + (size_t)src * ctw, (size_t)2 * run, nl, L, dst));
            j += run - 1;
            continue;
        }
        u64 g = sfg_galois_for_rotation(ctx, SFG_SLOTS - nrot);
        auto it = ctx->rotkeys().find(g);
        if (it == ctx->rotkeys().end()) SFG_FAIL(ctx, "rotate: no rotation key loaded for right-rotation by %d (galois element %llu)", nrot, g);
        job_in.push_back(src); keyp.push_back(it->second.key_dev); idxp.push_back(it->second.index_dev); outp.push_back(reinterpret_cast<u64 *>(dst));
    }
    return launch_keyswitch_jobs(ctx, in, nin, level, job_in, keyp, idxp, outp, nullptr, &ff);
}
int launch_relinearize(sfg_ctx *ctx, const u64 *tmp, int nct, int level, const u64 *mid, u64 *out) {
    auto it = ctx->rotkeys().find(1);
    if (it == ctx->rotkeys().end()) SFG_FAIL(ctx, "relinearize: no relinearisation key loaded");
    const size_t ctw = (size_t)2 * (level + 1) * SFG_N;
    std::vector<int> job_in(nct); std::vector<const u64 *> keyp(nct, it->second.key_dev); std::vector<const uint16_t *> idxp(nct, it->second.index_dev); std::vector<u64 *> outp(nct);
    for (int j = 0; j < nct; j++) { job_in[j] = j; outp[j] = out + (size_t)j * ctw; }
    return launch_keyswitch_jobs(ctx, tmp, nct, level, job_in, keyp, idxp, outp, mid);
}
int launch_rotate_right(sfg_ctx *ctx, const u64 *in, u64 *out, int nct, int level, const int *nrot_host) {
    return launch_rotate_right_indexed(ctx, in, nct, out, nct, level, nrot_host, nullptr);
}

extern "C" int sfg_rotate_right_dev(sfg_ctx *ctx, const uint64_t *in, uint64_t *out, int nct, int level, const int *nrot_host) {
    SFG_HIP(ctx, hipSetDevice(ctx->device));
    if (in == out) SFG_FAIL(ctx, "rotate: in and out must not alias");
    PhaseTimer t(ctx, "rotate");
    int rc = launch_rotate_right(ctx, (const u64 *)in, (u64 *)out, nct, level, nrot_host);
    t.stop(1);
    return rc;
}

extern "C" int sfg_ct_galois_dev(sfg_ctx *ctx, const uint64_t *in, uint64_t *out, int nct, int level, uint64_t galois_el) {
    SFG_HIP(ctx, hipSetDevice(ctx->device));
    if (in == out) SFG_FAIL(ctx, "galois: in and out must not alias");
    if (level < 0 || level >= ctx->nq) SFG_FAIL(ctx, "galois: level out of range");
    auto it = ctx->rotkeys().find(galois_el);
    if (it == ctx->rotkeys().end() || galois_el == 1) SFG_FAIL(ctx, "galois: no switching key loaded for galois element %llu", (unsigned long long)galois_el);
    const size_t ctw = (size_t)2 * (level + 1) * SFG_N;
    std::vector<int> job_in(nct); std::vector<const u64 *> keyp(nct, it->second.key_dev); std::vector<const uint16_t *> idxp(nct, it->second.index_dev); std::vector<u64 *> outp(nct);
    for (int j = 0; j < nct; j++) { job_in[j] = j; outp[j] = (u64 *)out + (size_t)j * ctw; }
    PhaseTimer t(ctx, "rotate");
    int rc = launch_keyswitch_jobs(ctx, (const u64 *)in, nct, level, job_in, keyp, idxp, outp, nullptr);
    t.stop(1);
    return rc;
}

int launch_ct_add(sfg_ctx *ctx, const u64 *a, const u64 *b, u64 *out, size_t nct, int level) {
    const int nl = level + 1; const size_t rows = nct * 2 * nl;
    if (!rows) return 0;
    hipLaunchKernelGGL(k_ct_add, dim3((unsigned)(rows * (SFG_N / 256))), dim3(256), 0, ctx->stream, a, b, out, nl, ctx->modc, rows);
    SFG_HIP(ctx, hipGetLastError());
    return 0;
}
extern "C" int sfg_ct_add_dev(sfg_ctx *ctx, const uint64_t *a, const uint64_t *b, uint64_t *out, int nct, int level) {
    SFG_HIP(ctx, hipSetDevice(ctx->device));
    if (level < 0 || level >= ctx->nq) SFG_FAIL(ctx, "evaluator op: level %d out of range", level);
    if (nct < 0) SFG_FAIL(ctx, "evaluator op: negative ciphertext count");
    return launch_ct_add(ctx, (const u64 *)a, (const u64 *)b, (u64 *)out, (size_t)nct, level);
}
```

Baseline: 6151 billion.

## Fuse giant-step rotation with summation in finalize; add optional fused inverse-NTT extend kernel

The finalize step no longer writes every rotated ciphertext to a scratch buffer and then sums them in a separate kernel. The key-switch pipeline now ends in a finish-and-sum kernel that adds the rotated outputs straight into the result, with the unrotated giant supplied as a plain addend. This is on by default and cuts scratch memory traffic and one launch per column block. A separate fused inverse-NTT plus basis-extension kernel is also added but stays disabled by default. The NTT inverse body is moved into a shared helper.

```diff
diff --git a/sfgwas_amd/csrc/ab/ab.hpp b/sfgwas_amd/csrc/ab/ab.hpp
--- a/sfgwas_amd/csrc/ab/ab.hpp
+++ b/sfgwas_amd/csrc/ab/ab.hpp
@@ -6,6 +6,10 @@
 int ab_mac_dma_set_attrs(sfg_ctx *ctx);
 int ab_launch_mac_dma_tiles(sfg_ctx *ctx, const double *rotf, size_t rows_per_k, const u64 *pt, u64 *out, int K, int R, int Ncols, int L, int accumulate, const MacStrides &st);
 int ab_ntt_set_attrs(sfg_ctx *ctx);
+struct KswConst;
+int ab_ntt_inv_ext_set_attrs(sfg_ctx *ctx);
+bool ab_ntt_inv_ext_fits(int alpha);
+int ab_launch_ntt_inv_ext(sfg_ctx *ctx, const u64 *in, u64 *out, size_t ngroups, int a, bool moddown, const KswConst *kcd);
 int ab_launch_ntt_half_full(sfg_ctx *ctx, const double *pc, u64 *out_half, size_t nplain, int L, const PanelMap &pm);
 int launch_mac(sfg_ctx *ctx, const u64 *rot, const u64 *pt, u64 *out, int K, int R, int Ncols, int L, int accumulate);
 int launch_mac_strided(sfg_ctx *ctx, const u64 *rot, const u64 *pt, u64 *out, int K, int R, int Ncols, int L, int accumulate, const MacStrides &st);
diff --git a/sfgwas_amd/csrc/ab/config.hip b/sfgwas_amd/csrc/ab/config.hip
--- a/sfgwas_amd/csrc/ab/config.hip
+++ b/sfgwas_amd/csrc/ab/config.hip
@@ -13,6 +13,8 @@
     if (env("SFG_MM_NO_OVERLAP")) c.no_overlap = true;
     if (const char *e = env("SFG_NTT_HALF_IMPL")) c.ntt_half_full = !strcmp(e, "full");
     if (const char *e = env("SFG_NTT_FWD_IMPL")) c.ntt_fwd_full = !strcmp(e, "full");
+    if (const char *e = env("SFG_KSW_FUSE_EXT")) c.ksw_fuse_ext = atoi(e) != 0;
+    if (const char *e = env("SFG_FIN_FUSE_SUM")) c.fin_fuse_sum = atoi(e) != 0;
     if (const char *e = env("SFG_MAC_PT")) c.mac_plain_pt = !strcmp(e, "plain");
     if (const char *e = env("SFG_PT_RIDE")) { c.pt_ride = atoi(e); if (c.pt_ride < 0) c.pt_ride = 0; c.pt_ride = c.pt_ride / 8 * 8; }
     if (const char *e = env("SFG_PT_COMPACT")) c.pt_compact = atoi(e) != 0;
@@ -21,4 +23,4 @@
     if (const char *e = env("SFG_PT_RIDE_NT")) c.i8_mover_nt_ride = atoi(e) != 0;
     if (env("SFG_ASSOC_TRACE")) c.assoc_trace = true;
 }
-int ab_set_attrs(sfg_ctx *ctx) { return ab_mac_dma_set_attrs(ctx) || ab_ntt_set_attrs(ctx); }
+int ab_set_attrs(sfg_ctx *ctx) { return ab_mac_dma_set_attrs(ctx) || ab_ntt_set_attrs(ctx) || ab_ntt_inv_ext_set_attrs(ctx); }
diff --git a/sfgwas_amd/csrc/ab/ntt_inv_ext.hip b/sfgwas_amd/csrc/ab/ntt_inv_ext.hip
--- /dev/null
+++ b/sfgwas_amd/csrc/ab/ntt_inv_ext.hip
@@ -0,0 +1,87 @@
+#include "../common.hpp"
+#include "../kernels.hpp"
+#include "../ntt_core.hpp"
+#include "../ksw.hpp"
+
+constexpr int KSW_FUSE_MAXA = 2;
+
+template <int A, bool MODDOWN>
+__global__ void __launch_bounds__(512) k_ntt_inv_ext(const u64 *in_, u64 *out_, const KswConst *kcp, const double *tw_all, const double2 *pack_all, const ModConst *modc) {
+    extern __shared__ double lds[];
+    const KswConst &kc = *kcp;
+    const int N = SFG_N, tid = threadIdx.x;
+    const size_t g = blockIdx.x;
+    const int i = MODDOWN ? -1 : (int)(g % kc.beta);
+    const ExtConst &e = MODDOWN ? kc.pq : kc.dig[i];
+    const u64 *in = MODDOWN ? in_ + (g * kc.nt + kc.nl) * N : in_ + ((g / kc.beta) * 2 * kc.nl + kc.nl) * N;
+    const int ntg = MODDOWN ? kc.nl : kc.nt;
+    u64 *out = out_ + g * (size_t)ntg * N;
+    double xs[A][32];
+#pragma unroll
+    for (int m = 0; m < A; m++) {
+        if (m < e.a) {
+            const int sm = e.src[m];
+            const double q = modc[sm].q, qinv = modc[sm].qinv, ninv = modc[sm].ninv, ninv_q = modc[sm].ninv_q;
+            if (m) __syncthreads();
+            ntt_inv_phases(in + (size_t)(MODDOWN ? m : sm) * N, xs[m], lds, tw_all + (size_t)sm * N, pack_all + (size_t)sm * (N / 2), q, qinv, tid);
+#pragma unroll
+            for (int a = 0; a < 32; a++) xs[m][a] = canon(mulmod_lazy(pred(xs[m][a], q, qinv), ninv, ninv_q, q), q, qinv);
+        } else {
+#pragma unroll
+            for (int a = 0; a < 32; a++) xs[m][a] = 0.0;
+        }
+    }
+    const bool single = A == 1 || e.a == 1;
+    double vv[A > 1 ? 32 : 1];
+    if constexpr (A > 1) if (!single) {
+#pragma unroll
+        for (int a = 0; a < 32; a++) {
+            double x[A], y[A];
+#pragma unroll
+            for (int m = 0; m < A; m++) x[m] = xs[m][a];
+            ext_prepare(e, modc, x, y, vv[a]);
+#pragma unroll
+            for (int m = 0; m < A; m++) xs[m][a] = y[m];
+        }
+    }
+    for (int t = 0; t < ntg; t++) {
+        if (!MODDOWN && kc.digit_of[t] == i) continue;
+        const int tg = MODDOWN ? t : kc.tmod[t];
+        const double qt = modc[tg].q, qtinv = modc[tg].qinv;
+        u64 *o = out + (size_t)t * N;
+        if (single) {
+#pragma unroll
+            for (int a = 0; a < 32; a++) o[a * 512 + tid] = f64_to_u64(canon(xs[0][a], qt, qtinv));
+        } else if constexpr (A > 1) {
+#pragma unroll
+            for (int a = 0; a < 32; a++) {
+                double y[A];
+#pragma unroll
+                for (int m = 0; m < A; m++) y[m] = xs[m][a];
+                o[a * 512 + tid] = f64_to_u64(ext_target(e, tg, qt, qtinv, y, vv[a]));
+            }
+        }
+    }
+}
+
+int ab_launch_ntt_inv_ext(sfg_ctx *ctx, const u64 *in, u64 *out, size_t ngroups, int a, bool moddown, const KswConst *kcd) {
+    if (!ngroups) return 0;
+    if (a < 1 || a > KSW_FUSE_MAXA) SFG_FAIL(ctx, "fused inverse NTT: %d source rows per group (at most %d)", a, KSW_FUSE_MAXA);
+    const dim3 grid((unsigned)ngroups), blk(512);
+#define SFG_IE(A, M) hipLaunchKernelGGL((k_ntt_inv_ext<A, M>), grid, blk, LDS_DOUBLES * 8, ctx->stream, in, out, kcd, ctx->tw_inv, ctx->pack_inv, ctx->modc)
+    if (a == 1) { if (moddown) SFG_IE(1, true); else SFG_IE(1, false); }
+    else { if (moddown) SFG_IE(2, true); else SFG_IE(2, false); }
+#undef SFG_IE
+    SFG_HIP(ctx, hipGetLastError());
+    return 0;
+}
+
+int ab_ntt_inv_ext_set_attrs(sfg_ctx *ctx) {
+    hipError_t e = hipFuncSetAttribute((const void *)k_ntt_inv_ext<1, false>, hipFuncAttributeMaxDynamicSharedMemorySize, LDS_DOUBLES * 8);
+    if (e == hipSuccess) e = hipFuncSetAttribute((const void *)k_ntt_inv_ext<1, true>, hipFuncAttributeMaxDynamicSharedMemorySize, LDS_DOUBLES * 8);
+    if (e == hipSuccess) e = hipFuncSetAttribute((const void *)k_ntt_inv_ext<2, false>, hipFuncAttributeMaxDynamicSharedMemorySize, LDS_DOUBLES * 8);
+    if (e == hipSuccess) e = hipFuncSetAttribute((const void *)k_ntt_inv_ext<2, true>, hipFuncAttributeMaxDynamicSharedMemorySize, LDS_DOUBLES * 8);
+    if (e != hipSuccess) SFG_FAIL(ctx, "cannot raise dynamic LDS limit for the fused inverse NTT");
+    return 0;
+}
+bool ab_ntt_inv_ext_fits(int alpha) { return alpha <= KSW_FUSE_MAXA; }
diff --git a/sfgwas_amd/csrc/common.hpp b/sfgwas_amd/csrc/common.hpp
--- a/sfgwas_amd/csrc/common.hpp
+++ b/sfgwas_amd/csrc/common.hpp
@@ -65,6 +65,8 @@
     bool mac_i8_wg1 = false;
     int mac_wc = 1;
     bool no_overlap = true;
+    bool ksw_fuse_ext = false;
+    bool fin_fuse_sum = true;
     bool ntt_fwd_full = false;
     bool ntt_half_full = false;
     bool pt_compact = true;
diff --git a/sfgwas_amd/csrc/kernels.hpp b/sfgwas_amd/csrc/kernels.hpp
--- a/sfgwas_amd/csrc/kernels.hpp
+++ b/sfgwas_amd/csrc/kernels.hpp
@@ -43,6 +43,7 @@
 int launch_geno_unpack(sfg_ctx *ctx, const sfg_geno *g, size_t r0, size_t c0, size_t nr, size_t nc, int8_t *out, size_t ld_out);
 int launch_rotate_right(sfg_ctx *ctx, const u64 *in, u64 *out, int nct, int level, const int *nrot_host);
 int launch_rotate_right_indexed(sfg_ctx *ctx, const u64 *in, int nin, u64 *out, int nct, int level, const int *nrot_host, const int *in_index);
+int launch_rotate_sum(sfg_ctx *ctx, const u64 *in, int nin, int level, const int *nrot_host, const int *in_index, int ngiant, int s, u64 *out, size_t out_i_stride, int accumulate);
 int launch_rotate_right_indexed_f64(sfg_ctx *ctx, const u64 *in, int nin, double *outf, int nct, int level, const int *nrot_host, const int *in_index, int L,
                                     const size_t *out_slot = nullptr);
 int launch_relinearize(sfg_ctx *ctx, const u64 *tmp, int nct, int level, const u64 *mid, u64 *out);
diff --git a/sfgwas_amd/csrc/ksw.hpp b/sfgwas_amd/csrc/ksw.hpp
--- a/sfgwas_amd/csrc/ksw.hpp
+++ b/sfgwas_amd/csrc/ksw.hpp
@@ -30,10 +30,11 @@
     return r + l;
 }
 
-__device__ __forceinline__ void ext_prepare(const ExtConst &e, const ModConst *modc, const double (&x)[KSW_MAXA], double (&y)[KSW_MAXA], double &v) {
+template <int MA>
+__device__ __forceinline__ void ext_prepare(const ExtConst &e, const ModConst *modc, const double (&x)[MA], double (&y)[MA], double &v) {
     double vf = 0.0;
 #pragma unroll
-    for (int m = 0; m < KSW_MAXA; m++) {
+    for (int m = 0; m < MA; m++) {
         if (m < e.a) {
             const ModConst mc = modc[e.src[m]];
             y[m] = canon(mulmod_lazy(x[m], e.qhat_inv[m], e.qhat_inv_q[m], mc.q), mc.q, mc.qinv);
@@ -42,10 +43,11 @@
     }
     v = (double)(u64)vf;
 }
-__device__ __forceinline__ double ext_target(const ExtConst &e, int tg, double qt, double qtinv, const double (&y)[KSW_MAXA], double v) {
+template <int MA>
+__device__ __forceinline__ double ext_target(const ExtConst &e, int tg, double qt, double qtinv, const double (&y)[MA], double v) {
     double acc = -mulmod_lazy(v, e.D_t[tg], e.D_t_q[tg], qt);
 #pragma unroll
-    for (int m = 0; m < KSW_MAXA; m++) if (m < e.a) acc += mulmod_lazy(y[m], e.qhat_t[tg][m], e.qhat_t_q[tg][m], qt);
+    for (int m = 0; m < MA; m++) if (m < e.a) acc += mulmod_lazy(y[m], e.qhat_t[tg][m], e.qhat_t_q[tg][m], qt);
     return canon(acc, qt, qtinv);
 }
 #endif
diff --git a/sfgwas_amd/csrc/matmul.hip b/sfgwas_amd/csrc/matmul.hip
--- a/sfgwas_amd/csrc/matmul.hip
+++ b/sfgwas_amd/csrc/matmul.hip
@@ -32,6 +32,7 @@
     const size_t x = (blockIdx.x % (N / 256)) * 256 + threadIdx.x;
     out[row * N + x] = in[(ctp * nl_in + m) * N + x];
 }
+#ifdef SFG_AB
 __global__ void __launch_bounds__(256) k_sum_giants(const u64 *rot, int ngiant, int s, int L, u64 *out, size_t out_i_stride,
                                                     int accumulate, const ModConst *modc) {
     const int N = SFG_N; const size_t row = blockIdx.x / (N / 256);
@@ -45,6 +46,7 @@
     }
     out[(size_t)i * out_i_stride + (size_t)pl * N + x] = f64_to_u64(canon(acc, q, qinv));
 }
+#endif
 __global__ void __launch_bounds__(256) k_reduce_rows(u64 *rows, int L, const ModConst *modc) {
     const int N = SFG_N; const size_t row = blockIdx.x / (N / 256); const int l = (int)(row % L);
     const size_t off = row * N + (blockIdx.x % (N / 256)) * 256 + threadIdx.x;
@@ -562,26 +564,36 @@
     const int N = SFG_N, d = SFG_D, L = max_level;
     const size_t accw = (size_t)s * 2 * L * N, ctw = (size_t)2 * L * N;
     if (g0 < 0 || g1 > acc_giants || g0 > g1 || giant_base < 0) SFG_FAIL(ctx, "finalize: giant range out of bounds");
-    u64 *rot = nullptr;
-    SFG_TRY(sfg_scratch(ctx, "mm.fin_rot", (size_t)d * accw * 8, (void **)&rot));
     std::vector<int> glist;
     for (int g = g0; g < g1; g++) if (giant_base + g < d && (!giant_active || (*giant_active)[giant_base + g])) glist.push_back(g);
     const int ng = (int)glist.size();
     std::vector<int> nrv((size_t)ng * s), inv((size_t)ng * s);
     for (int k = 0; k < ng; k++) for (int i = 0; i < s; i++) { nrv[(size_t)k * s + i] = -(giant_base + glist[k]) * d; inv[(size_t)k * s + i] = glist[k] * s + i; }
     int rc = 0;
+#ifdef SFG_AB
+    u64 *rot = nullptr;
+    if (!ctx->cfg.fin_fuse_sum) SFG_TRY(sfg_scratch(ctx, "mm.fin_rot", (size_t)d * accw * 8, (void **)&rot));
+#endif
     for (int jb = 0; jb < ncolb && !rc; jb++) {
         const u64 *accj = acc + (size_t)jb * acc_giants * accw;
         u64 *o = out + (size_t)(jout0 + jb) * ctw;
-        if (ng) {
-            PhaseTimer t(ctx, "rotate");
-            rc = launch_rotate_right_indexed(ctx, accj, acc_giants * s, rot, ng * s, L - 1, nrv.data(), inv.data());
-            t.stop(1);
-            if (rc) break;
-        }
-        hipLaunchKernelGGL(k_sum_giants, dim3((unsigned)((size_t)s * 2 * L * (N / 256))), dim3(256), 0, ctx->stream, rot, ng, s, L,
-                           o, (size_t)m_ct_out * ctw, accumulate, ctx->modc);
-        if (hipGetLastError() != hipSuccess) { rc = 1; ctx->err = "finalize: k_sum_giants launch failed"; }
+#ifdef SFG_AB
+        if (!ctx->cfg.fin_fuse_sum) {
+            if (ng) {
+                PhaseTimer t(ctx, "rotate");
+                rc = launch_rotate_right_indexed(ctx, accj, acc_giants * s, rot, ng * s, L - 1, nrv.data(), inv.data());
+                t.stop(1);
+                if (rc) break;
+            }
+            hipLaunchKernelGGL(k_sum_giants, dim3((unsigned)((size_t)s * 2 * L * (N / 256))), dim3(256), 0, ctx->stream, rot, ng, s, L,
+                               o, (size_t)m_ct_out * ctw, accumulate, ctx->modc);
+            if (hipGetLastError() != hipSuccess) { rc = 1; ctx->err = "finalize: k_sum_giants launch failed"; }
+            continue;
+        }
+#endif
+        PhaseTimer t(ctx, "rotate");
+        rc = launch_rotate_sum(ctx, accj, acc_giants * s, L - 1, nrv.data(), inv.data(), ng, s, o, (size_t)m_ct_out * ctw, accumulate);
+        t.stop(1);
     }
     return rc;
 }
diff --git a/sfgwas_amd/csrc/ntt.hip b/sfgwas_amd/csrc/ntt.hip
--- a/sfgwas_amd/csrc/ntt.hip
+++ b/sfgwas_amd/csrc/ntt.hip
@@ -55,60 +55,7 @@
     const double q = modc[m].q, qinv = modc[m].qinv;
     const u64 *in = in_ + grp * rm.gstride_in + gi * N;
     double v[32];
-    {
-        const int b = tid >> 4, c = tid & 15;
-#pragma unroll
-        for (int a = 0; a < 32; a++) lds[a * LDS_ROW + c * 33 + b] = u64_to_f64(in[a * 512 + tid]);
-    }
-    __syncthreads();
-#pragma unroll
-    for (int h = 0; h < 2; h++) {
-        const int p = tid + 512 * h, a = p >> 5, b = p & 31;
-        double w[16];
-#pragma unroll
-        for (int c = 0; c < 16; c++) w[c] = lds[a * LDS_ROW + c * 33 + b];
-        double tl[16];
-        {
-            const double2 *pk = pack + (size_t)(p >> 6) * 512 + (p & 63);
-#pragma unroll
-            for (int i = 0; i < 8; i++) { const double2 e = pk[i * 64]; tl[2 * i] = e.x; tl[2 * i + 1] = e.y; }
-        }
-        gs_stage<16, 1>(w, q, qinv, [&](int g) { return tl[7 + g]; });
-        gs_stage<16, 2>(w, q, qinv, [&](int g) { return tl[3 + g]; });
-        gs_stage<16, 4>(w, q, qinv, [&](int g) { return tl[1 + g]; });
-        gs_stage<16, 8>(w, q, qinv, [&](int g) { return tl[0 + g]; });
-#pragma unroll
-        for (int c = 0; c < 16; c++) v[h * 16 + c] = pred(w[c], q, qinv);
-    }
-    __syncthreads();
-#pragma unroll
-    for (int h = 0; h < 2; h++) {
-        const int p = tid + 512 * h, a = p >> 5, b = p & 31;
-#pragma unroll
-        for (int c = 0; c < 16; c++) lds[a * LDS_ROW + c * 33 + b] = v[h * 16 + c];
-    }
-    __syncthreads();
-    {
-        const int a = tid >> 4, c = tid & 15;
-#pragma unroll
-        for (int b = 0; b < 32; b++) v[b] = lds[a * LDS_ROW + c * 33 + b];
-        gs_stage<32, 1>(v, q, qinv, [&](int g) { return tw[512 + a * 16 + g]; });
-        gs_stage<32, 2>(v, q, qinv, [&](int g) { return tw[256 + a * 8 + g]; });
-        gs_stage<32, 4>(v, q, qinv, [&](int g) { return tw[128 + a * 4 + g]; });
-        gs_stage<32, 8>(v, q, qinv, [&](int g) { return tw[64 + a * 2 + g]; });
-        gs_stage<32, 16>(v, q, qinv, [&](int g) { return tw[32 + a + g]; });
-        __syncthreads();
-#pragma unroll
-        for (int b = 0; b < 32; b++) lds[a * LDS_ROW + b * 16 + c] = pred(v[b], q, qinv);
-    }
-    __syncthreads();
-#pragma unroll
-    for (int a = 0; a < 32; a++) v[a] = lds[a * LDS_ROW + tid];
-    gs_stage<32, 1>(v, q, qinv, [&](int g) { return tw[16 + g]; });
-    gs_stage<32, 2>(v, q, qinv, [&](int g) { return tw[8 + g]; });
-    gs_stage<32, 4>(v, q, qinv, [&](int g) { return tw[4 + g]; });
-    gs_stage<32, 8>(v, q, qinv, [&](int g) { return tw[2 + g]; });
-    gs_stage<32, 16>(v, q, qinv, [&](int g) { return tw[1 + g]; });
+    ntt_inv_phases(in, v, lds, tw, pack, q, qinv, tid);
     const double ninv = modc[m].ninv, ninv_q = modc[m].ninv_q;
     u64 *out = out_ + grp * rm.gstride_out + gi * N;
 #pragma unroll
@@ -440,7 +387,6 @@
     SFG_HIP(ctx, hipGetLastError());
     return 0;
 }
-
 static int pattern_from_host(sfg_ctx *ctx, const int *mod_idx, int nrows, ModPattern &pat) {
     for (int period = 1; period <= 64 && period <= nrows; period++) {
         bool ok = true;
diff --git a/sfgwas_amd/csrc/ntt_core.hpp b/sfgwas_amd/csrc/ntt_core.hpp
--- a/sfgwas_amd/csrc/ntt_core.hpp
+++ b/sfgwas_amd/csrc/ntt_core.hpp
@@ -84,6 +84,62 @@
     }
     __syncthreads();
 }
+__device__ __forceinline__ void ntt_inv_phases(const u64 *in, double (&v)[32], double *lds, const double *tw, const double2 *pack, double q, double qinv, int tid) {
+    {
+        const int b = tid >> 4, c = tid & 15;
+#pragma unroll
+        for (int a = 0; a < 32; a++) lds[a * LDS_ROW + c * 33 + b] = u64_to_f64(in[a * 512 + tid]);
+    }
+    __syncthreads();
+#pragma unroll
+    for (int h = 0; h < 2; h++) {
+        const int p = tid + 512 * h, a = p >> 5, b = p & 31;
+        double w[16];
+#pragma unroll
+        for (int c = 0; c < 16; c++) w[c] = lds[a * LDS_ROW + c * 33 + b];
+        double tl[16];
+        {
+            const double2 *pk = pack + (size_t)(p >> 6) * 512 + (p & 63);
+#pragma unroll
+            for (int i = 0; i < 8; i++) { const double2 e = pk[i * 64]; tl[2 * i] = e.x; tl[2 * i + 1] = e.y; }
+        }
+        gs_stage<16, 1>(w, q, qinv, [&](int g) { return tl[7 + g]; });
+        gs_stage<16, 2>(w, q, qinv, [&](int g) { return tl[3 + g]; });
+        gs_stage<16, 4>(w, q, qinv, [&](int g) { return tl[1 + g]; });
+        gs_stage<16, 8>(w, q, qinv, [&](int g) { return tl[0 + g]; });
+#pragma unroll
+        for (int c = 0; c < 16; c++) v[h * 16 + c] = pred(w[c], q, qinv);
+    }
+    __syncthreads();
+#pragma unroll
+    for (int h = 0; h < 2; h++) {
+        const int p = tid + 512 * h, a = p >> 5, b = p & 31;
+#pragma unroll
+        for (int c = 0; c < 16; c++) lds[a * LDS_ROW + c * 33 + b] = v[h * 16 + c];
+    }
+    __syncthreads();
+    {
+        const int a = tid >> 4, c = tid & 15;
+#pragma unroll
+        for (int b = 0; b < 32; b++) v[b] = lds[a * LDS_ROW + c * 33 + b];
+        gs_stage<32, 1>(v, q, qinv, [&](int g) { return tw[512 + a * 16 + g]; });
+        gs_stage<32, 2>(v, q, qinv, [&](int g) { return tw[256 + a * 8 + g]; });
+        gs_stage<32, 4>(v, q, qinv, [&](int g) { return tw[128 + a * 4 + g]; });
+        gs_stage<32, 8>(v, q, qinv, [&](int g) { return tw[64 + a * 2 + g]; });
+        gs_stage<32, 16>(v, q, qinv, [&](int g) { return tw[32 + a + g]; });
+        __syncthreads();
+#pragma unroll
+        for (int b = 0; b < 32; b++) lds[a * LDS_ROW + b * 16 + c] = pred(v[b], q, qinv);
+    }
+    __syncthreads();
+#pragma unroll
+    for (int a = 0; a < 32; a++) v[a] = lds[a * LDS_ROW + tid];
+    gs_stage<32, 1>(v, q, qinv, [&](int g) { return tw[16 + g]; });
+    gs_stage<32, 2>(v, q, qinv, [&](int g) { return tw[8 + g]; });
+    gs_stage<32, 4>(v, q, qinv, [&](int g) { return tw[4 + g]; });
+    gs_stage<32, 8>(v, q, qinv, [&](int g) { return tw[2 + g]; });
+    gs_stage<32, 16>(v, q, qinv, [&](int g) { return tw[1 + g]; });
+}
 __device__ __forceinline__ bool plain_block_of(size_t b, size_t nplain, int L, size_t &row, int &m) {
     const size_t per = (size_t)8 * L, plain = (b / per) * 8 + (b % per) % 8;
     m = (int)((b % per) / 8); row = plain * L + m;
diff --git a/sfgwas_amd/csrc/rotate.hip b/sfgwas_amd/csrc/rotate.hip
--- a/sfgwas_amd/csrc/rotate.hip
+++ b/sfgwas_amd/csrc/rotate.hip
@@ -144,6 +144,34 @@
     }
 }
 
+__global__ void __launch_bounds__(256) k_ksw_finish_sum(const u64 *__restrict__ ct_in, const int *__restrict__ inidx, const u64 *__restrict__ acc, const u64 *__restrict__ ext2,
+                                                       const uint16_t *const *__restrict__ index, int j0, int nb, int s, const u64 *__restrict__ plain, u64 *out,
+                                                       size_t out_i_stride, int accumulate, const KswConst *kcp, const ModConst *modc) {
+    const KswConst &kc = *kcp;
+    const int N = SFG_N, x = blockIdx.x * 256 + threadIdx.x, t = blockIdx.y, i = blockIdx.z, nl = kc.nl;
+    const double q = modc[t].q, qinv = modc[t].qinv, pinv = kc.pinv[t], pinv_q = kc.pinv_q[t];
+    u64 *o0 = out + (size_t)i * out_i_stride + (size_t)t * N + x, *o1 = o0 + (size_t)nl * N;
+    double s0 = 0.0, s1 = 0.0;
+    if (accumulate) { s0 = u64_to_f64(*o0); s1 = u64_to_f64(*o1); }
+    if (plain) {
+        s0 += u64_to_f64(plain[(((size_t)i * 2 + 0) * nl + t) * N + x]);
+        s1 += u64_to_f64(plain[(((size_t)i * 2 + 1) * nl + t) * N + x]);
+    }
+    int n = 0;
+    for (int b = ((i - j0) % s + s) % s; b < nb; b += s) {
+        const int src = index[b][x];
+        const size_t ro = (size_t)t * N + src;
+        const double a0 = u64_to_f64(acc[((size_t)b * 2 + 0) * (size_t)kc.nt * N + ro]), e0 = u64_to_f64(ext2[((size_t)b * 2 + 0) * (size_t)nl * N + ro]);
+        const double a1 = u64_to_f64(acc[((size_t)b * 2 + 1) * (size_t)kc.nt * N + ro]), e1 = u64_to_f64(ext2[((size_t)b * 2 + 1) * (size_t)nl * N + ro]);
+        const double c0 = u64_to_f64(ct_in[(size_t)inidx[b] * 2 * (size_t)nl * N + ro]);
+        s0 += mulmod_lazy(a0 - e0, pinv, pinv_q, q) + c0;
+        s1 += mulmod_lazy(a1 - e1, pinv, pinv_q, q);
+        if (++n == 4) { s0 = pred(s0, q, qinv); s1 = pred(s1, q, qinv); n = 0; }
+    }
+    *o0 = f64_to_u64(canon(s0, q, qinv));
+    *o1 = f64_to_u64(canon(s1, q, qinv));
+}
+
 __global__ void __launch_bounds__(256) k_ct_add(const u64 *a, const u64 *b, u64 *out, int nl, const ModConst *modc, size_t total_rows) {
     const int N = SFG_N; const size_t row = blockIdx.x / (N / 256); const int m = (int)(row % nl);
     const u64 q = modc[m].qi;
@@ -151,23 +179,40 @@
     u64 v = a[off] + b[off]; out[off] = v >= q ? v - q : v;
 }
 
+struct SumForm { int s; u64 *out; size_t out_i_stride; int accumulate; const u64 *plain; };
 static int launch_keyswitch_jobs(sfg_ctx *ctx, const u64 *in, int nin, int level, const std::vector<int> &job_in, const std::vector<const u64 *> &keyp,
-                                 const std::vector<const uint16_t *> &idxp, const std::vector<u64 *> &outp, const u64 *add1, const F64Form *ffp = nullptr) {
+                                 const std::vector<const uint16_t *> &idxp, const std::vector<u64 *> &outp, const u64 *add1, const F64Form *ffp = nullptr,
+                                 const SumForm *sum = nullptr) {
     const int N = SFG_N, nl = level + 1;
     F64Form ff; memset(&ff, 0, sizeof ff); if (ffp) ff = *ffp;
     KswConst *kcd; KswConst kc;
     SFG_TRY(get_ksw(ctx, level, &kcd, &kc));
     const size_t ctw = (size_t)2 * nl * N;
     const int nr = (int)job_in.size();
-    if (!nr) return 0;
-    const size_t in_rows = (size_t)nl + (size_t)kc.beta * kc.nt, job_rows = 2 * (size_t)kc.nt + 2 * (size_t)nl;
+    int sum_acc = sum ? sum->accumulate : 0; const u64 *sum_plain = sum ? sum->plain : nullptr;
+    auto finish_sum = [&](const u64 *bin, const int *inidx_d, const u64 *acc, const u64 *ext2T, const uint16_t *const *idx_d, int j0, int nb) {
+        hipLaunchKernelGGL(k_ksw_finish_sum, dim3(N / 256, nl, sum->s), dim3(256), 0, ctx->stream, bin, inidx_d, acc, ext2T, idx_d, j0, nb, sum->s, sum_plain, sum->out,
+                           sum->out_i_stride, sum_acc, kcd, ctx->modc);
+        sum_acc = 1; sum_plain = nullptr;
+    };
+    if (!nr) {
+        if (sum) { finish_sum(nullptr, nullptr, nullptr, nullptr, nullptr, 0, 0); SFG_HIP(ctx, hipGetLastError()); }
+        return 0;
+    }
+#ifdef SFG_AB
+    const bool fuse = ctx->cfg.ksw_fuse_ext && ab_ntt_inv_ext_fits(kc.alpha);
+#else
+    const bool fuse = false;
+#endif
+    const size_t c2_rows = fuse ? 0 : (size_t)nl;
+    const size_t in_rows = c2_rows + (size_t)kc.beta * kc.nt, job_rows = 2 * (size_t)kc.nt + 2 * (size_t)nl;
     const size_t budget = ctx->cfg.ksw_budget;
     int in_grp = (int)(budget / (in_rows * N * 8)); if (in_grp < 1) in_grp = 1; if (in_grp > nin) in_grp = nin;
     int chunk = (int)(budget / (job_rows * N * 8)); if (chunk < 1) chunk = 1; if (chunk > nr) chunk = nr;
     const size_t ptr_bytes = (size_t)nr * (3 * sizeof(void *) + sizeof(int)) + 256;
     const size_t ext_rows = (size_t)in_grp * kc.beta * kc.nt, ext2_rows = (size_t)chunk * 2 * nl;
     SFG_TRY(sfg_ws_reserve(ctx, (in_rows * in_grp + job_rows * chunk + ext_rows + ext2_rows) * N * 8 + ptr_bytes));
-    u64 *c2 = (u64 *)ctx->ws, *ext = c2 + (size_t)in_grp * nl * N;
+    u64 *c2 = (u64 *)ctx->ws, *ext = c2 + (size_t)in_grp * c2_rows * N;
     u64 *acc = ext + ext_rows * N, *ext2 = acc + (size_t)chunk * 2 * kc.nt * N;
     u64 *extT = ext2 + ext2_rows * N, *ext2T = extT + ext_rows * N;
     const u64 **keys_all = (const u64 **)(ext2T + ext2_rows * N);
@@ -183,11 +228,17 @@
         std::vector<int> jobs;
         for (int k = 0; k < nr; k++) if (job_in[k] >= i0 && job_in[k] < i0 + ni) jobs.push_back(k);
         if (jobs.empty()) continue;
+        if (sum) for (size_t k = 1; k < jobs.size(); k++) if (jobs[k] != jobs[0] + (int)k) SFG_FAIL(ctx, "rotate-and-sum: the jobs of an input group are not one run of the job list");
         const u64 *bin = in + (size_t)i0 * ctw;
-        RowMap rm1; rm1.rpg = nl; rm1.gstride_in = ctw; rm1.gstride_out = (size_t)nl * N;
-        SFG_TRY(launch_ntt_inv_map(ctx, bin + (size_t)nl * N, c2, (size_t)ni * nl, pq, rm1));
-        hipLaunchKernelGGL(k_ksw_extend, dim3(N / 256, kc.beta, ni), dim3(256), 0, ctx->stream, c2, bin, ext, kcd, ctx->modc);
-        SFG_HIP(ctx, hipGetLastError());
+#ifdef SFG_AB
+        if (fuse) SFG_TRY(ab_launch_ntt_inv_ext(ctx, bin, ext, (size_t)ni * kc.beta, kc.alpha, false, kcd));
+#endif
+        if (!fuse) {
+            RowMap rm1; rm1.rpg = nl; rm1.gstride_in = ctw; rm1.gstride_out = (size_t)nl * N;
+            SFG_TRY(launch_ntt_inv_map(ctx, bin + (size_t)nl * N, c2, (size_t)ni * nl, pq, rm1));
+            hipLaunchKernelGGL(k_ksw_extend, dim3(N / 256, kc.beta, ni), dim3(256), 0, ctx->stream, c2, bin, ext, kcd, ctx->modc);
+            SFG_HIP(ctx, hipGetLastError());
+        }
         SFG_TRY(launch_ntt_fwd(ctx, ext, extT, (size_t)ni * kc.beta * kc.nt, pext));
         {
             const size_t nj = jobs.size();
@@ -203,13 +254,19 @@
             const u64 **keys_d = keys_all + c0; const uint16_t **idx_d = idx_all + c0; u64 **out_d = out_all + c0; int *inidx_d = inidx_all + c0;
             hipLaunchKernelGGL(k_ksw_inner, dim3(N / 512, kc.nt, nb), dim3(256), 0, ctx->stream, extT, bin, keys_d, inidx_d, acc, kcd, ctx->modc, ctx->nmod);
             SFG_HIP(ctx, hipGetLastError());
-            RowMap rm4; rm4.rpg = kc.np; rm4.gstride_in = (size_t)kc.nt * N; rm4.gstride_out = (size_t)kc.nt * N;
-            SFG_TRY(launch_ntt_inv_map(ctx, acc + (size_t)nl * N, acc + (size_t)nl * N, (size_t)nb * 2 * kc.np, pp, rm4));
-            hipLaunchKernelGGL(k_moddown_extend, dim3(N / 256, 2, nb), dim3(256), 0, ctx->stream, acc, ext2, kcd, ctx->modc);
-            SFG_HIP(ctx, hipGetLastError());
+#ifdef SFG_AB
+            if (fuse) SFG_TRY(ab_launch_ntt_inv_ext(ctx, acc, ext2, (size_t)nb * 2, kc.np, true, kcd));
+#endif
+            if (!fuse) {
+                RowMap rm4; rm4.rpg = kc.np; rm4.gstride_in = (size_t)kc.nt * N; rm4.gstride_out = (size_t)kc.nt * N;
+                SFG_TRY(launch_ntt_inv_map(ctx, acc + (size_t)nl * N, acc + (size_t)nl * N, (size_t)nb * 2 * kc.np, pp, rm4));
+                hipLaunchKernelGGL(k_moddown_extend, dim3(N / 256, 2, nb), dim3(256), 0, ctx->stream, acc, ext2, kcd, ctx->modc);
+                SFG_HIP(ctx, hipGetLastError());
+            }
             SFG_TRY(launch_ntt_fwd(ctx, ext2, ext2T, (size_t)nb * 2 * nl, pq));
-            hipLaunchKernelGGL(k_ksw_finish, dim3(N / 256, nl, nb), dim3(256), 0, ctx->stream, bin, inidx_d, acc, ext2T, idx_d, out_d, kcd, ctx->modc,
-                               add1 ? add1 + (size_t)i0 * nl * N : nullptr, ff);
+            if (sum) finish_sum(bin, inidx_d, acc, ext2T, idx_d, jobs[c0], nb);
+            else hipLaunchKernelGGL(k_ksw_finish, dim3(N / 256, nl, nb), dim3(256), 0, ctx->stream, bin, inidx_d, acc, ext2T, idx_d, out_d, kcd, ctx->modc,
+                                    add1 ? add1 + (size_t)i0 * nl * N : nullptr, ff);
             SFG_HIP(ctx, hipGetLastError());
         }
     }
@@ -237,6 +294,33 @@
         job_in.push_back(src); keyp.push_back(it->second.key_dev); idxp.push_back(it->second.index_dev); outp.push_back(out + j * ctw);
     }
     return launch_keyswitch_jobs(ctx, in, nin, level, job_in, keyp, idxp, outp, nullptr);
+}
+int launch_rotate_sum(sfg_ctx *ctx, const u64 *in, int nin, int level, const int *nrot_host, const int *in_index, int ngiant, int s, u64 *out, size_t out_i_stride, int accumulate) {
+    const int N = SFG_N, nl = level + 1;
+    if (level < 0 || level >= ctx->nq) SFG_FAIL(ctx, "rotate: level out of range");
+    if (s < 1 || s > 65535) SFG_FAIL(ctx, "rotate-and-sum: output count out of range");
+    const size_t ctw = (size_t)2 * nl * N;
+    SumForm sum; sum.s = s; sum.out = out; sum.out_i_stride = out_i_stride; sum.accumulate = accumulate; sum.plain = nullptr;
+    std::vector<int> job_in; std::vector<const u64 *> keyp; std::vector<const uint16_t *> idxp; std::vector<u64 *> outp;
+    for (int k = 0; k < ngiant; k++) {
+        int nrot = nrot_host[(size_t)k * s] % SFG_SLOTS; if (nrot < 0) nrot += SFG_SLOTS;
+        for (int i = 0; i < s; i++) {
+            const int src = in_index[(size_t)k * s + i];
+            if (src < 0 || src >= nin) SFG_FAIL(ctx, "rotate: input index out of range");
+            if ((nrot_host[(size_t)k * s + i] - nrot_host[(size_t)k * s]) % SFG_SLOTS) SFG_FAIL(ctx, "rotate-and-sum: the outputs of a giant step must share its rotation");
+            if (nrot == 0 && src != in_index[(size_t)k * s] + i) SFG_FAIL(ctx, "rotate-and-sum: the unrotated giant's inputs must be consecutive");
+        }
+        if (nrot == 0) {
+            if (sum.plain) SFG_FAIL(ctx, "rotate-and-sum: more than one unrotated giant");
+            sum.plain = in + (size_t)in_index[(size_t)k * s] * ctw;
+            continue;
+        }
+        u64 g = sfg_galois_for_rotation(ctx, SFG_SLOTS - nrot);
+        auto it = ctx->rotkeys().find(g);
+        if (it == ctx->rotkeys().end()) SFG_FAIL(ctx, "rotate: no rotation key loaded for right-rotation by %d (galois element %llu)", nrot, g);
+        for (int i = 0; i < s; i++) { job_in.push_back(in_index[(size_t)k * s + i]); keyp.push_back(it->second.key_dev); idxp.push_back(it->second.index_dev); outp.push_back(nullptr); }
+    }
+    return launch_keyswitch_jobs(ctx, in, nin, level, job_in, keyp, idxp, outp, nullptr, nullptr, &sum);
 }
 int launch_rotate_right_indexed_f64(sfg_ctx *ctx, const u64 *in, int nin, double *outf, int nct, int level, const int *nrot_host, const int *in_index, int L,
                                     const size_t *out_slot) {
```

Result: no change. 6209 billion (median of 6 runs) (+0.9%).
